# deepqmc/deepqmc

Hardware: NVIDIA H100
Metric: walker.local-energies/sec (higher is better)
Workload: dtype f32

## Files before the change

deepqmc_b200/_lib.py:

```python
from __future__ import annotations

import ctypes as C
import os

MAX_NUC, MAX_T, MAX_L = 32, 4, 4
LIB_NAME = 'libdqmc_b200.so'
LIB_PATH = os.path.join(os.path.dirname(os.path.abspath(__file__)), LIB_NAME)

SYMBOLS = [
    'dqmc_create', 'dqmc_destroy', 'dqmc_last_error', 'dqmc_version', 'dqmc_param_count',
    'dqmc_param_entry', 'dqmc_param_total', 'dqmc_set_params', 'dqmc_workspace_bytes',
    'dqmc_wf_forward', 'dqmc_local_energy', 'dqmc_mcmc_sweep', 'dqmc_launch_count',
    'dqmc_profile_begin', 'dqmc_profile_end', 'dqmc_debug_gemm', 'dqmc_wf_vjp_params', 'dqmc_langevin_sweep',
    'dqmc_set_pseudo_hamiltonian', 'dqmc_wf_orbitals', 'dqmc_mcmc_sweep_exchange',
    'dqmc_workspace_bytes_min', 'dqmc_debug_plan', 'dqmc_stats_pack', 'dqmc_debug_mlp_block', 'dqmc_debug_trunk',
    'dqmc_profile_end_classes', 'dqmc_debug_trunk_phases', 'dqmc_debug_attention', 'dqmc_debug_mlp',
    'dqmc_debug_slater', 'dqmc_debug_det_sum', 'dqmc_spin', 'dqmc_ecp_forward_count', 'dqmc_wf_grad_positions',
    'dqmc_force_terms', 'dqmc_ecp_force', 'dqmc_debug_wgrad', 'dqmc_zv_force',
    'dqmc_debug_attention_bwd',
]


class DqmcConfig(C.Structure):
    _fields_ = [
        ('kind', C.c_int32), ('dtype', C.c_int32), ('gemm_backend', C.c_int32),
        ('n_up', C.c_int32), ('n_down', C.c_int32), ('n_nuc', C.c_int32),
        ('embedding_dim', C.c_int32), ('n_layers', C.c_int32), ('n_heads', C.c_int32),
        ('n_determinants', C.c_int32), ('edge_dim', C.c_int32),
        ('cusp_kind', C.c_int32), ('cusp_same_scale', C.c_double), ('cusp_anti_scale', C.c_double),
        ('z_valence', C.c_double * MAX_NUC), ('ecp_mask', C.c_int32 * MAX_NUC),
        ('ecp_loc_terms', C.c_int32), ('ecp_loc', C.c_double * (MAX_NUC * 3 * 2 * MAX_T)),
        ('ecp_nl_lmax_p1', C.c_int32), ('ecp_nl_terms', C.c_int32),
        ('ecp_nl', C.c_double * (MAX_NUC * MAX_L * 2 * MAX_T)),
        ('n_env_per_nuc', C.c_int32), ('n_nuc_tokens', C.c_int32),
        ('factorized_det', C.c_int32), ('conf_linear', C.c_int32), ('mult_act', C.c_int32),
        ('n_elec_types', C.c_int32), ('jastrow_n', C.c_int32), ('jastrow_dims', C.c_int32 * 8),
        ('backflow_n', C.c_int32), ('backflow_dims', C.c_int32 * 8),
        ('gnn_features', C.c_int32), ('gnn_concat', C.c_int32), ('gnn_conv_ne', C.c_int32), ('gnn_sub_n', C.c_int32),
        ('gnn_deep_edges', C.c_int32), ('gnn_res_norm', C.c_int32), ('gnn_g_bias', C.c_int32), ('gnn_w_bias', C.c_int32),
        ('gnn_w_dims', C.c_int32 * 32), ('gnn_h_dims', C.c_int32 * 32), ('gnn_u_dims', C.c_int32 * 32),
        ('nuc_cusp_kind', C.c_int32), ('z_nuclear', C.c_double * MAX_NUC), ('backflow_add', C.c_int32),
    ]


_cache = {}


def load(path: str | None = None) -> C.CDLL:
    path = path or LIB_PATH
    if path in _cache:
        return _cache[path]
    if not os.path.exists(path):
        raise ImportError(
            f'{path} not found: the CUDA engine is not built. Run `python -c "import __graft_entry__ as g; '
            'g.build()"` (nvcc, sm_90a). There is no CPU fallback.'
        )
    lib = C.CDLL(path)
    for s in SYMBOLS:
        if not hasattr(lib, s):
            raise ImportError(f'{path} does not export {s}')
    vp, i32, i64, u64 = C.c_void_p, C.c_int32, C.c_int64, C.c_uint64
    lib.dqmc_create.argtypes = [C.POINTER(DqmcConfig), C.c_int, C.POINTER(vp)]
    lib.dqmc_destroy.argtypes = [vp]
    lib.dqmc_last_error.argtypes = [vp]
    lib.dqmc_last_error.restype = C.c_char_p
    lib.dqmc_version.restype = C.c_char_p
    lib.dqmc_param_count.argtypes = [vp]
    lib.dqmc_param_entry.argtypes = [vp, C.c_int, C.c_char_p, C.c_int, C.POINTER(i64), C.POINTER(i32), C.POINTER(i32)]
    lib.dqmc_param_total.argtypes = [vp]
    lib.dqmc_param_total.restype = i64
    lib.dqmc_set_params.argtypes = [vp, C.POINTER(C.c_double), i64, vp]
    lib.dqmc_workspace_bytes.argtypes = [vp, i32, i32]
    lib.dqmc_workspace_bytes.restype = i64
    lib.dqmc_workspace_bytes_min.argtypes = [vp, i32, i32]
    lib.dqmc_workspace_bytes_min.restype = i64
    lib.dqmc_debug_plan.argtypes = [vp, i32, i32, i64, C.POINTER(i64), C.POINTER(i64)]
    lib.dqmc_stats_pack.argtypes = [vp, vp, vp, i32, vp, vp]
    lib.dqmc_debug_mlp_block.argtypes = [vp, i32, vp, vp, vp, i32, vp]
    lib.dqmc_debug_trunk.argtypes = [vp, vp, vp, i32, vp]
    lib.dqmc_debug_trunk_phases.argtypes = [vp, C.POINTER(u64), i32]
    lib.dqmc_debug_attention.argtypes = [vp, i32, vp, vp, i32, i32, C.POINTER(i32), vp]
    lib.dqmc_debug_mlp.argtypes = [vp, i32, i32, vp, vp, vp, vp, i32, C.POINTER(i32), vp]
    lib.dqmc_debug_slater.argtypes = [vp, vp, vp, vp, i32, i32, vp, vp, vp, vp, C.POINTER(i32), vp]
    lib.dqmc_debug_det_sum.argtypes = [vp, vp, vp, vp, vp, vp, vp, i32, i32, vp, vp, vp, vp, vp]
    lib.dqmc_debug_wgrad.argtypes = [vp, vp, vp, i32, i32, i32, i32, i32, vp, vp, vp]
    lib.dqmc_debug_attention_bwd.argtypes = [vp, i32, vp, vp, vp, vp, vp, i32, vp]
    lib.dqmc_wf_forward.argtypes = [vp, vp, vp, i32, i32, vp, vp, vp, i64, vp]
    lib.dqmc_wf_orbitals.argtypes = [vp, vp, vp, i32, i32, vp, vp, i64, vp]
    lib.dqmc_local_energy.argtypes = [vp, vp, vp, i32, i32, u64, vp, vp, vp, vp, vp, vp, vp, i64, vp]
    lib.dqmc_mcmc_sweep.argtypes = [vp, vp, vp, vp, vp, vp, vp, i32, i32, i32, C.c_double, i32, u64, u64, u64,
                                    vp, vp, vp, vp, i64, vp]
    lib.dqmc_mcmc_sweep_exchange.argtypes = [vp, vp, vp, vp, vp, vp, vp, i32, i32, i32, C.c_double, i32, u64, u64, u64,
                                             vp, vp, C.c_double, C.POINTER(i32), vp, vp, vp, i64, vp]
    lib.dqmc_langevin_sweep.argtypes = [vp, vp, vp, vp, vp, vp, vp, vp, i32, i32, i32, C.c_double, i32, u64, u64, u64,
                                        vp, vp, vp, vp, i64, vp]
    lib.dqmc_wf_vjp_params.argtypes = [vp, vp, vp, i32, i32, vp, vp, vp, vp, vp, i64, vp]
    lib.dqmc_spin.argtypes = [vp, vp, vp, i32, i32, vp, vp, i32, vp, vp, vp, i64, vp]
    lib.dqmc_wf_grad_positions.argtypes = [vp, vp, vp, i32, i32, vp, vp, vp, vp, vp, i64, vp]
    lib.dqmc_force_terms.argtypes = [vp, vp, vp, i32, i32, vp, vp, vp, vp, vp]
    lib.dqmc_ecp_force.argtypes = [vp, vp, vp, i32, i32, u64, vp, vp, vp, vp, i64, vp]
    lib.dqmc_zv_force.argtypes = [vp, vp, vp, i32, i32, vp, vp, vp, i64, vp]
    lib.dqmc_set_pseudo_hamiltonian.argtypes = [vp, i32, i32, C.c_double, C.POINTER(C.c_double), C.POINTER(i32)]
    lib.dqmc_launch_count.argtypes = [vp]
    lib.dqmc_launch_count.restype = i64
    lib.dqmc_ecp_forward_count.argtypes = [vp]
    lib.dqmc_ecp_forward_count.restype = i64
    lib.dqmc_profile_begin.argtypes = [vp]
    lib.dqmc_debug_gemm.argtypes = [vp, C.c_char_p, C.c_char_p, vp, vp, vp, i32, i32, i32, i32, vp]
    lib.dqmc_profile_end.argtypes = [vp, C.POINTER(C.c_double), C.POINTER(C.c_double), C.POINTER(i64)]
    lib.dqmc_profile_end_classes.argtypes = [vp, C.POINTER(C.c_double), C.POINTER(C.c_double), C.POINTER(i64)]
    _cache[path] = lib
    return lib
```

deepqmc_b200/csrc/engine.cu:

```cuda
#include <algorithm>
#include <array>
#include <cstdio>
#include <cstdlib>
#include <cstring>
#include <limits>
#include <map>
#include <mutex>
#include <optional>
#include <string>
#include <type_traits>
#include <vector>

#include "dqmc_b200.h"
#include "kernels_mcmc.cuh"
#include "kernels_slater.cuh"
#include "kernels_trunk.cuh"
#include "kernels_gnn.cuh"
#include "kernels_bwd.cuh"
#include "kernels_zv.cuh"
#include "attn_mma.cuh"
#if !defined(DQMC_NO_TCGEN05)
#include "gemm_wgmma.cuh"
#include "fused_tc.cuh"
#include "trunk_tc.cuh"
#endif

namespace dq {

struct ParamEntry {
  std::string name;
  int64_t offset;
  int rows, cols;
};

static inline size_t align_up(size_t x, size_t a = 256) { return (x + a - 1) / a * a; }

template <class W>
static double last_above(W w, double lo, double eps) {
  double hi = lo > 0.0 ? 2 * lo : 1.0;
  while (w(hi) >= eps) { lo = hi; hi *= 2; }
  for (;;) {
    const double mid = lo + 0.5 * (hi - lo);
    if (mid <= lo || mid >= hi) break;
    (w(mid) >= eps ? lo : hi) = mid;
  }
  return lo;
}

template <class T>
static double ecp_cutoff_rc2(const T* nl, int L, int Tn, bool on) {
  const double inf = std::numeric_limits<double>::infinity(), eps = std::ldexp(1.0, -100);
  if (!on) return inf;
  for (int l = 0; l < L; ++l)
    for (int t = 0; t < Tn; ++t)
      if ((double)nl[(l * 2 + 1) * Tn + t] != 0.0 && !((double)nl[(l * 2) * Tn + t] > 0.0)) return inf;
  auto w = [&](double d2) {
    double s = 0.0;
    for (int l = 0; l < L; ++l)
      for (int t = 0; t < Tn; ++t)
        s += (2 * l + 1) * std::fabs((double)nl[(l * 2 + 1) * Tn + t]) * std::exp(-(double)nl[(l * 2) * Tn + t] * d2);
    return s;
  };
  if (w(0.0) < eps) return -inf;
  return last_above(w, 0.0, eps);
}

template <class T>
static double ecp_force_cutoff_rc2(const T* nl, int L, int Tn, bool on) {
  const double rc2 = ecp_cutoff_rc2(nl, L, Tn, on), eps = std::ldexp(1.0, -100);
  if (rc2 == std::numeric_limits<double>::infinity()) return rc2;
  double peak = 0.0;
  for (int l = 0; l < L; ++l)
    for (int t = 0; t < Tn; ++t)
      if ((double)nl[(l * 2 + 1) * Tn + t] != 0.0) peak = std::max(peak, 0.5 / (double)nl[(l * 2) * Tn + t]);
  auto wd = [&](double d2) {
    double s = 0.0;
    for (int l = 0; l < L; ++l)
      for (int t = 0; t < Tn; ++t) {
        const double a = (double)nl[(l * 2) * Tn + t];
        s += (2 * l + 1) * 2 * a * std::fabs((double)nl[(l * 2 + 1) * Tn + t]) * std::sqrt(d2) * std::exp(-a * d2);
      }
    return s;
  };
  return std::max(rc2, wd(peak) >= eps ? last_above(wd, peak, eps) : peak);
}

struct Switches {
  bool tc_trunk = true;
  bool tc_f16 = true;
  std::optional<bool> attn_fl_mma;
  std::optional<int> attn_tb, attn_nt;
  bool attn_generic = false;
  bool no_fuse_tanh = false;
  bool slater_generic = false;
  bool slater_fwd1 = false;
  bool ecp_cutoff = true;
  bool ecp_env_table = true;
  bool ecp_emb_table = true;
  int nsms = 0;
  bool trunk_phases = false;
};

inline Switches read_switches() {
  auto env = [](const char* name) { return std::getenv(name); };
  auto num = [&](const char* name) { const char* ev = env(name); return ev ? std::optional<int>(std::atoi(ev)) : std::nullopt; };
  Switches s;
  s.tc_trunk = num("DQMC_TC_TRUNK").value_or(1) != 0;
  s.tc_f16 = num("DQMC_TC_F16").value_or(1) != 0;
  if (auto v = num("DQMC_ATTN_FL_MMA")) s.attn_fl_mma = *v != 0;
  s.attn_tb = num("DQMC_ATTN_TB");
  s.attn_nt = num("DQMC_ATTN_NT");
  s.attn_generic = env("DQMC_ATTN_GENERIC");
  s.no_fuse_tanh = env("DQMC_NO_FUSE_TANH");
  s.slater_generic = env("DQMC_SLATER_GENERIC");
  s.slater_fwd1 = env("DQMC_SLATER_FWD1");
  s.ecp_cutoff = num("DQMC_ECP_CUTOFF").value_or(1) != 0;
  s.ecp_env_table = !env("DQMC_ECP_ENV_TABLE_OFF");
  s.ecp_emb_table = !env("DQMC_ECP_EMB_TABLE_OFF");
  s.nsms = num("DQMC_NSMS").value_or(0);
  s.trunk_phases = num("DQMC_TRUNK_PHASES").value_or(0) != 0;
  return s;
}

struct EngineBase {
  dqmc_config cfg;
  int device = 0;
  std::string err;
  int64_t launches = 0;
  int64_t ecp_forwards = 0;
  std::vector<ParamEntry> entries;
  int64_t total = 0;
  bool dry = false;
  bool plan_only = false;
  mutable const char* dry_hwm = nullptr;
  void note_hwm(const void* q) const { if (dry && (const char*)q > dry_hwm) dry_hwm = (const char*)q; }
  mutable std::vector<unsigned char*> emu_guards;
  bool prof = false;
  double prof_flops = 0;
  int64_t prof_n = 0;
  double prof_cls_flops[3] = {0, 0, 0};
  int64_t prof_cls_n[3] = {0, 0, 0};
  std::vector<int> prof_cls;
#ifndef DQMC_EMU
  std::vector<cudaEvent_t> prof_ev;
  void prof_note(cudaEvent_t e0, cudaEvent_t e1, double flops, int cls) {
    prof_ev.push_back(e0); prof_ev.push_back(e1);
    prof_cls.push_back(cls);
    prof_flops += flops; prof_cls_flops[cls] += flops;
    ++prof_n; ++prof_cls_n[cls];
  }
#endif
  virtual ~EngineBase() {}
  virtual int set_params(const double* host, int64_t n, cudaStream_t st) = 0;
  virtual int64_t ws_bytes(int B, int mode) = 0;
  virtual int64_t ws_bytes_min(int B, int mode) = 0;
  virtual int debug_plan(int B, int mode, int64_t wsb, int64_t* planned, int64_t* carved) = 0;
  virtual int stats_pack(const void* E, const void* stats, int B, double* out, cudaStream_t st) = 0;
  virtual int debug_mlp_block(int layer, const void* O, const void* X, void* Out, int rows, cudaStream_t st) = 0;
  virtual int debug_trunk(const void* X0, void* Out, int rows, cudaStream_t st) = 0;
  virtual int debug_attention(int layer, const void* QKV, void* O, int rows, int S, int32_t* kernel, cudaStream_t st) = 0;
  virtual int debug_mlp(int layer, int S, const void* O, const void* X, void* Out, void* scratch, int rows, int32_t* path,
                        cudaStream_t st) = 0;
  virtual int debug_trunk_phases(uint64_t* out, int n) = 0;
  virtual int debug_slater(const void* r, const void* R, const void* BF, int rows, int S, void* dsign, void* dlog, void* dgrad,
                           void* dlap, int32_t* kernel, cudaStream_t st) = 0;
  virtual int debug_det_sum(const void* r, const void* R, const void* dsign, const void* dlog, const void* dgrad,
                            const void* dlap, int B, int S, void* sign, void* logp, void* grad, void* stats,
                            cudaStream_t st) = 0;
  virtual int debug_wgrad(const void* A, const void* dY, int rows, int Kc, int Nc, int lo, int hi, void* dW, void* db,
                          cudaStream_t st) = 0;
  virtual int debug_attention_bwd(int layer, const void* QKV, const void* dO, void* dQKV, void* dKn, void* dVn, int rows,
                                  cudaStream_t st) = 0;
  virtual int forward(const void* r, const void* R, int Rb, int B, void* sign, void* logp, void* ws, int64_t wsb,
                      cudaStream_t st) = 0;
  virtual int local_energy(const void* r, const void* R, int Rb, int B, uint64_t seed, const void* twist, void* E,
                           void* stats, void* sign, void* logp, void* grad, void* ws, int64_t wsb,
                           cudaStream_t st) = 0;
  virtual int langevin(void* r, void* sign, void* logp, void* force, int32_t* age, void* tau, const void* R, int Rb, int B,
                       int n_sub, double target, int max_age, uint64_t seed, uint64_t step0, uint64_t woff, const void* nn,
                       const void* nu, void* stats, void* ws, int64_t wsb, cudaStream_t st) = 0;
  virtual int vjp_params(const void* r, const void* R, int Rb, int B, const void* weights, void* sign, void* logp,
                         void* grad_params, void* ws, int64_t wsb, cudaStream_t st) = 0;
  virtual int spin(const void* r, const void* R, int Rb, int B, const void* sign, const void* logp, int down_idx, void* s2,
                   void* ratio, void* ws, int64_t wsb, cudaStream_t st) = 0;
  virtual int grad_positions(const void* r, const void* R, int Rb, int B, void* sign, void* logp, void* grad_r, void* grad_R,
                             void* ws, int64_t wsb, cudaStream_t st) = 0;
  virtual int force_terms(const void* r, const void* R, int Rb, int B, const void* grad_r, void* bare, void* zvq, void* Q,
                          cudaStream_t st) = 0;
  virtual int ecp_force(const void* r, const void* R, int Rb, int B, uint64_t seed, const void* twist, void* bare, void* nl,
                        void* ws, int64_t wsb, cudaStream_t st) = 0;
  virtual int zv_force(const void* r, const void* R, int Rb, int B, void* zv, void* grad_R, void* ws, int64_t wsb,
                       cudaStream_t st) = 0;
  virtual int orbitals(const void* r, const void* R, int Rb, int B, void* out, void* ws, int64_t wsb, cudaStream_t st) = 0;
  virtual int set_ph(int n_tab, int n_grid, double r_max, const double* tables, const int32_t* tab_of_nuc) = 0;
  virtual int debug_gemm(const char* wname, const char* bname, const void* A, const void* Res, void* C, int Mr, int S,
                         int sliced, int backend, cudaStream_t st) = 0;
  virtual int mcmc(void* r, void* sign, void* logp, int32_t* age, void* tau, const void* R, int Rb, int B, int n_sub,
                   double target, int max_age, uint64_t seed, uint64_t step0, uint64_t woff, const void* nn,
                   const void* nu, void* stats, void* ws, int64_t wsb, cudaStream_t st, double p_exchange = 0.0,
                   const int32_t* ex_flags = nullptr, const int32_t* ex_idx = nullptr) = 0;

  void add(const std::string& n, int rows, int cols) {
    entries.push_back({n, total, rows, cols});
    total += (int64_t)rows * cols;
  }
  void build_layout() {
    const int N = cfg.n_up + cfg.n_down, M = cfg.n_nuc, d = cfg.embedding_dim, K = cfg.n_determinants;
    const int rep = cfg.n_env_per_nuc > 1 ? cfg.n_env_per_nuc : 1;
    if (cfg.kind == DQMC_PSIFORMER || cfg.kind == DQMC_TRANSPSIFORMER) {
      add("emb.w", 4 * M + 1, d);
      for (int l = 0; l < cfg.n_layers; ++l) {
        std::string p = "L" + std::to_string(l) + ".";
        add(p + "wqkv", d, 3 * d);
        add(p + "wo", d, d);
        add(p + "w1", d, d);
        add(p + "b1", 1, d);
        add(p + "w2", d, d);
        add(p + "b2", 1, d);
        if (cfg.kind == DQMC_TRANSPSIFORMER && cfg.n_nuc_tokens > 0) {
          add(p + "kn", cfg.n_nuc_tokens, d);
          add(p + "vn", cfg.n_nuc_tokens, d);
        }
      }
    }
    int bf_in = d;
    if (cfg.kind == DQMC_PAULINET) {
      const int e = cfg.edge_dim, nl = cfg.gnn_sub_n > 0 ? cfg.gnn_sub_n : 1;
      if (!cfg.gnn_features) add("emb.table", cfg.n_elec_types > 0 ? cfg.n_elec_types : 1, d);
      int dcur = cfg.gnn_features ? 4 * M : d, ecur = 4;
      const int nt = cfg.gnn_conv_ne ? 3 : 2;
      const char* tn[3] = {"same", "anti", "ne"};
      for (int l = 0; l < cfg.n_layers; ++l) {
        std::string p = "G" + std::to_string(l) + ".";
        for (int t = 0; t < nt; ++t) {
          int din = ecur;
          for (int i = 0; i < nl; ++i) {
            const std::string q = p + "w_" + tn[t] + "." + std::to_string(i);
            add(q + ".w", din, cfg.gnn_w_dims[l][i]);
            if (cfg.gnn_w_bias) add(q + ".b", 1, cfg.gnn_w_dims[l][i]);
            din = cfg.gnn_w_dims[l][i];
          }
          if (t < 2) {
            din = dcur;
            for (int i = 0; i < nl; ++i) {
              const std::string q = p + "h_" + tn[t] + "." + std::to_string(i);
              add(q + ".w", din, cfg.gnn_h_dims[l][i]); add(q + ".b", 1, cfg.gnn_h_dims[l][i]);
              din = cfg.gnn_h_dims[l][i];
            }
          } else {
            add(p + "hne", M, e);
          }
          if (!cfg.gnn_concat) { add(p + "g_" + tn[t] + ".w", e, d); add(p + "g_" + tn[t] + ".b", 1, d); }
        }
        if (cfg.gnn_concat) {
          add(p + "g.w", 3 * dcur + nt * e, d);
          if (cfg.gnn_g_bias) add(p + "g.b", 1, d);
        }
        if (cfg.gnn_deep_edges && l < cfg.n_layers - 1) {
          int din = ecur;
          for (int i = 0; i < nl; ++i) {
            const std::string q = p + "u." + std::to_string(i);
            add(q + ".w", din, cfg.gnn_u_dims[l][i]); add(q + ".b", 1, cfg.gnn_u_dims[l][i]);
            din = cfg.gnn_u_dims[l][i];
          }
          ecur = e;
        }
        dcur = d;
      }
      int din = d;
      for (int i = 0; i < cfg.jastrow_n; ++i) {
        add("J" + std::to_string(i) + ".w", din, cfg.jastrow_dims[i]);
        if (i < cfg.jastrow_n - 1) add("J" + std::to_string(i) + ".b", 1, cfg.jastrow_dims[i]);
        din = cfg.jastrow_dims[i];
      }
      din = d;
      for (int i = 0; i < cfg.backflow_n; ++i) {
        const std::string q = std::to_string(i);
        add("bfh" + q + ".up", din, cfg.backflow_dims[i]); add("bfh" + q + ".dn", din, cfg.backflow_dims[i]);
        add("bfb" + q + ".up", 1, cfg.backflow_dims[i]); add("bfb" + q + ".dn", 1, cfg.backflow_dims[i]);
        din = cfg.backflow_dims[i];
      }
      bf_in = din;
      add("bfb.up", 1, K * N); add("bfb.dn", 1, K * N);
      if (cfg.conf_linear) add("conf.w", 1, K);
    }
    if (cfg.kind == DQMC_FERMINET) {
      const int de = cfg.edge_dim;
      int din = 4 * M, ein = 4;
      for (int l = 0; l < cfg.n_layers; ++l) {
        std::string p = "F" + std::to_string(l) + ".";
        add(p + "wg", 3 * din + 2 * ein, d);
        add(p + "bg", 1, d);
        if (l < cfg.n_layers - 1) {
          add(p + "wu", ein, de);
          add(p + "bu", 1, de);
        }
        din = d; ein = de;
      }
    }
    add("bf.up", bf_in, K * N * (cfg.backflow_add == 2 ? 2 : 1));
    add("bf.dn", bf_in, K * N * (cfg.backflow_add == 2 ? 2 : 1));
    add("env.pi_up", K * N, M * rep);
    add("env.pi_dn", K * N, M * rep);
    add("env.zeta_up", K * N, M * rep);
    add("env.zeta_dn", K * N, M * rep);
    add("cusp.alpha", 1, 2);
    if (cfg.nuc_cusp_kind) add("cusp.nuc", 1, 1 + M);
  }
  int64_t off(const std::string& n) const {
    for (auto& e : entries)
      if (e.name == n) return e.offset;
    return -1;
  }
};

struct Arena {
  const EngineBase* e;
  char* base;
  char* top;
  int64_t cap;
  Arena(const EngineBase* e_, void* base_, int64_t cap_ = INT64_MAX) : e(e_), base((char*)base_), top((char*)base_), cap(cap_) {}
  template <class U>
  U* take(size_t n) {
    U* q = (U*)top;
    top += align_up(sizeof(U) * n);
#ifdef DQMC_EMU
    if (!e->dry) { std::memset(top, 0xC3, 256); e->emu_guards.push_back((unsigned char*)top); }
    top += 256;
#endif
    e->note_hwm(top);
    return q;
  }
  int64_t left() const { return cap - (top - base); }
};

static char* plan_base() { return (char*)(uintptr_t)0x100000; }
struct DryPass {
  EngineBase* e;
  bool was;
  const char* hw;
  explicit DryPass(const EngineBase* e_) : e(const_cast<EngineBase*>(e_)), was(e->dry), hw(e->dry_hwm) {
    e->dry = true;
    e->dry_hwm = plan_base();
  }
  ~DryPass() { e->dry = was; e->dry_hwm = hw; }
  int64_t bytes() const { return e->dry_hwm - plan_base(); }
};

template <class F>
static int64_t largest_fit(int64_t hi, int64_t wsb, F bytes) {
  if (hi < 1 || bytes(1) > wsb) return 0;
  if (bytes(hi) <= wsb) return hi;
  int64_t lo = 1;
  while (hi - lo > 1) {
    const int64_t mid = (lo + hi) / 2;
    (bytes(mid) <= wsb ? lo : hi) = mid;
  }
  return lo;
}

static constexpr int64_t kRowCap = 2000000000;

template <class T>
__global__ void convert_kernel(const double* __restrict__ src, T* __restrict__ dst, int64_t n) {
  int64_t i = (int64_t)blockIdx.x * blockDim.x + threadIdx.x;
  if (i < n) dst[i] = (T)src[i];
}

__global__ void split_transpose_kernel(const float* __restrict__ W, int K, int N, float* __restrict__ hi,
                                       float* __restrict__ lo) {
  int idx = blockIdx.x * blockDim.x + threadIdx.x;
  if (idx >= K * N) return;
  int n = idx / K, k = idx % K;
  float w = W[(size_t)k * N + n];
#if !defined(DQMC_NO_TCGEN05)
  float h = tc::tf32_rna(w);
  hi[idx] = h;
  lo[idx] = tc::tf32_rna(w - h);
#else
  float h = __uint_as_float(__float_as_uint(w) & 0xFFFFE000u);
  hi[idx] = h;
  lo[idx] = w - h;
#endif
}

#if !defined(DQMC_NO_TCGEN05)
__global__ void split_transpose_f16_kernel(const float* __restrict__ W, int K, int N, float scale, uint16_t* __restrict__ hi,
                                           uint16_t* __restrict__ lo) {
  int idx = blockIdx.x * blockDim.x + threadIdx.x;
  if (idx >= K * N) return;
  int n = idx / K, k = idx % K;
  const float w = W[(size_t)k * N + n] * scale;
  const uint32_t h = tc::pack_half2_rn(w, 0.f) & 0xFFFFu;
  const uint32_t l = tc::pack_half2_rn(w - tc::half_bits_to_float(h), 0.f) & 0xFFFFu;
  hi[idx] = (uint16_t)h;
  lo[idx] = (uint16_t)l;
}
#endif

#define DQ_CHECK(call)                                                             \
  do {                                                                             \
    if (dry) break;                              \
    cudaError_t e_ = (call);                                                       \
    if (e_ != cudaSuccess) {                                                       \
      err = std::string(#call) + ": " + cudaGetErrorString(e_);                    \
      return 1;                                                                    \
    }                                                                              \
  } while (0)

template <class F>
inline cudaError_t raise_dyn_smem(F fn, int bytes) {
  static std::mutex mu;
  static std::map<std::pair<int, const void*>, int> high;
  int dev = 0;
  cudaError_t e = cudaGetDevice(&dev);
  if (e != cudaSuccess) return e;
  std::lock_guard<std::mutex> lock(mu);
  int& h = high[std::make_pair(dev, (const void*)fn)];
  if (bytes > h) h = bytes;
  return cudaFuncSetAttribute(fn, cudaFuncAttributeMaxDynamicSharedMemorySize, h);
}

#define DQ_LAUNCH(kern, grid, block, smem, stream, ...)          \
  do {                                                           \
    if (dry) break;                           \
    auto kfn_ = kern;                                            \
    DQMC_LAUNCH(kfn_, grid, block, smem, stream, __VA_ARGS__);   \
    ++launches;                                                  \
  } while (0)

template <class T>
struct Engine : EngineBase {
  T* d_params = nullptr;
  T* d_params_t = nullptr;
  double* d_stage = nullptr;
  T* d_zval = nullptr;
  T* d_znuc = nullptr;
  int* d_ecp_mask = nullptr;
  T* d_ecp_loc = nullptr;
  T* d_nl_params = nullptr;
  int* d_nl_nuc = nullptr;
  double* d_nl_rc2 = nullptr;
  double* d_nl_rc2f = nullptr;
  int J = 0;
  T* d_ph_tabs = nullptr;
  int* d_ph_nuc = nullptr;
  int ph_G = 0;
  double ph_rmax = 0;
  int check_guards() {
#ifdef DQMC_EMU
    for (unsigned char* g : emu_guards)
      for (int i = 0; i < 256; ++i)
        if (g[i] != 0xC3) { emu_guards.clear(); err = "emulator: a workspace buffer was overrun (guard zone modified)"; return 4; }
    emu_guards.clear();
#endif
    return 0;
  }
  bool ph_on = false;
  int attn_tb = 1, attn_tb1 = 1;
  bool attn_gen_mma = false;
  bool attn_fl_mma = false;
  int attn_fl_threads = 128;
  bool attn_f32 = false;
  bool embed_fwd_ok = false;
  bool attn_mma_ok = false;
  bool slater_fwd2_ok = false;
  int N, M, d, K, KN, H, dh, T3;
  int BFW = 0;
  int add_off = 0;
  bool gnn = false;
  int bf_in = 0;
  bool trans = false;
  int Mn = 0, env_rep = 1;
  size_t max_smem = 0;
  int n_sms = 132;
  Switches sw;
  struct FwdIn {
    const T* env = nullptr;
    const T* emb = nullptr;
    const int* pairs = nullptr;
    int vper = 0;
    int layout = kVirtEcp;
    T* mos = nullptr;
    bool ph = false;
  };
#if !defined(DQMC_NO_TCGEN05)
  struct TcWeight {
    float* hi = nullptr; float* lo = nullptr; CUtensorMap mh, ml; int N = 0, K = 0;
    uint16_t* h16 = nullptr; CUtensorMap m16h, m16l, m16h_all, m16l_all; float wscale = 1.f; bool f16 = false, f16_all = false;
    CUtensorMap m16h_256, m16l_256; bool f16_256 = false;
  };
  CUtensorMap* d_trunk_maps = nullptr;
  unsigned char* d_trunk_scratch = nullptr;
  unsigned long long* d_trunk_phase = nullptr;
  static constexpr float kActScale = 16.f;
  std::map<std::string, TcWeight> tcw;
  bool use_tc() const { return std::is_same<T, float>::value && cfg.gemm_backend == DQMC_GEMM_TCGEN05; }
  int prepare_tc_weight(const std::string& name, const float* W, int Kc, int Nc, cudaStream_t st, double wmax) {
    TcWeight& w = tcw[name];
    if (!w.hi) {
      DQ_CHECK(cudaMalloc((void**)&w.hi, sizeof(float) * (size_t)Kc * Nc));
      DQ_CHECK(cudaMalloc((void**)&w.lo, sizeof(float) * (size_t)Kc * Nc));
      w.N = Nc; w.K = Kc;
      if (tc::make_weight_map(&w.mh, w.hi, Nc, Kc, tc::kBN) || tc::make_weight_map(&w.ml, w.lo, Nc, Kc, tc::kBN)) {
        err = "cuTensorMapEncodeTiled failed for " + name;
        return 4;
      }
      if (Kc % 64 == 0) {
        DQ_CHECK(cudaMalloc((void**)&w.h16, sizeof(uint16_t) * 2 * (size_t)Kc * Nc));
        const uint16_t* lo16 = w.h16 + (size_t)Kc * Nc;
        if (tc::make_kmajor_map(&w.m16h, w.h16, 2, Nc, Kc, 64, tc::kBN) || tc::make_kmajor_map(&w.m16l, lo16, 2, Nc, Kc, 64, tc::kBN)) {
          err = "cuTensorMapEncodeTiled (half planes) failed for " + name;
          return 4;
        }
        w.f16 = true;
        if (Nc <= 256 && Nc % 16 == 0) {
          if (tc::make_kmajor_map(&w.m16h_all, w.h16, 2, Nc, Kc, 32, Nc) || tc::make_kmajor_map(&w.m16l_all, lo16, 2, Nc, Kc, 32, Nc)) {
            err = "cuTensorMapEncodeTiled (whole-N half planes) failed for " + name;
            return 4;
          }
          w.f16_all = true;
        }
        if (Kc == 256 && Nc % 256 == 0 &&
            !tc::make_kmajor_map(&w.m16h_256, w.h16, 2, Nc, Kc, 32, 256) && !tc::make_kmajor_map(&w.m16l_256, lo16, 2, Nc, Kc, 32, 256))
          w.f16_256 = true;
      }
    }
    DQ_LAUNCH(split_transpose_kernel, dim3((Kc * Nc + 255) / 256), dim3(256), 0, st, W, Kc, Nc, w.hi, w.lo);
    if (w.f16) {
      int e = 0;
      if (wmax > 0) { std::frexp(wmax, &e); e = 10 - e; }
      e = e > 24 ? 24 : (e < -24 ? -24 : e);
      w.wscale = std::ldexp(1.f, e);
      DQ_LAUNCH(split_transpose_f16_kernel, dim3((Kc * Nc + 255) / 256), dim3(256), 0, st, W, Kc, Nc, w.wscale, w.h16,
                w.h16 + (size_t)Kc * Nc);
    }
    return 0;
  }
#else
  bool use_tc() const { return false; }
#endif

  int init() {
    sw = read_switches();
    N = cfg.n_up + cfg.n_down; M = cfg.n_nuc; d = cfg.embedding_dim; K = cfg.n_determinants;
    KN = K * N; H = cfg.n_heads; dh = d / H; T3 = 3 * N;
    BFW = KN * (cfg.backflow_add == 2 ? 2 : 1);
    add_off = cfg.backflow_add == 2 ? KN : 0;
    if (cfg.backflow_add && cfg.kind == DQMC_PAULINET) { err = "additive backflow: linear-head ansatz kinds only"; return 2; }
    if (cfg.kind != DQMC_PSIFORMER && cfg.kind != DQMC_FERMINET && cfg.kind != DQMC_TRANSPSIFORMER &&
        cfg.kind != DQMC_PAULINET) {
      err = "unknown ansatz kind"; return 2;
    }
    trans = cfg.kind == DQMC_TRANSPSIFORMER;
    Mn = trans ? cfg.n_nuc_tokens : 0;
    env_rep = cfg.n_env_per_nuc > 1 ? cfg.n_env_per_nuc : 1;
    if (M * env_rep > 4 * DQMC_MAX_NUC || Mn < 0 || Mn > DQMC_MAX_NUC) { err = "bad config (envelope terms / nuclear tokens)"; return 2; }
    if (H < 1) H = 1;
    if (cfg.kind == DQMC_FERMINET || cfg.kind == DQMC_PAULINET) { H = 1; dh = d; }
    gnn = cfg.kind == DQMC_PAULINET;
    if (gnn && (cfg.jastrow_n > 8 || cfg.backflow_n > 8 || cfg.jastrow_n < 0 || cfg.backflow_n < 0)) { err = "bad MLP depth"; return 2; }
    bf_in = d;
    if (gnn && cfg.backflow_n > 0) bf_in = cfg.backflow_dims[cfg.backflow_n - 1];
    if (M > DQMC_MAX_NUC || d % H != 0 || N < 2) { err = "bad config"; return 2; }
    build_layout();
    DQ_CHECK(cudaSetDevice(device));
    DQ_CHECK(cudaMalloc((void**)&d_params, sizeof(T) * total));
    DQ_CHECK(cudaMalloc((void**)&d_params_t, sizeof(T) * total));
    DQ_CHECK(cudaMalloc((void**)&d_stage, sizeof(double) * total));
    std::vector<T> z(M);
    for (int m = 0; m < M; ++m) z[m] = (T)cfg.z_valence[m];
    DQ_CHECK(cudaMalloc((void**)&d_zval, sizeof(T) * M));
    DQ_CHECK(cudaMemcpy(d_zval, z.data(), sizeof(T) * M, cudaMemcpyHostToDevice));
    {
      std::vector<T> zn(M);
      for (int m = 0; m < M; ++m) zn[m] = (T)cfg.z_nuclear[m];
      DQ_CHECK(cudaMalloc((void**)&d_znuc, sizeof(T) * M));
      DQ_CHECK(cudaMemcpy(d_znuc, zn.data(), sizeof(T) * M, cudaMemcpyHostToDevice));
    }
    DQ_CHECK(cudaMalloc((void**)&d_ecp_mask, sizeof(int) * M));
    DQ_CHECK(cudaMemcpy(d_ecp_mask, cfg.ecp_mask, sizeof(int) * M, cudaMemcpyHostToDevice));
    const int Tm = cfg.ecp_loc_terms;
    if (Tm > 0) {
      std::vector<T> lp((size_t)M * 6 * Tm);
      for (int m = 0; m < M; ++m)
        for (int n = 0; n < 3; ++n)
          for (int ab = 0; ab < 2; ++ab)
            for (int t = 0; t < Tm; ++t) lp[(((size_t)m * 3 + n) * 2 + ab) * Tm + t] = (T)cfg.ecp_loc[m][n][ab][t];
      DQ_CHECK(cudaMalloc((void**)&d_ecp_loc, sizeof(T) * lp.size()));
      DQ_CHECK(cudaMemcpy(d_ecp_loc, lp.data(), sizeof(T) * lp.size(), cudaMemcpyHostToDevice));
    }
    const int L = cfg.ecp_nl_lmax_p1, Tn = cfg.ecp_nl_terms;
    if (L > 0 && Tn > 0) {
      std::vector<T> np((size_t)M * L * 2 * Tn);
      std::vector<int> nuc;
      for (int m = 0; m < M; ++m) {
        bool any = false;
        for (int l = 0; l < L; ++l)
          for (int ab = 0; ab < 2; ++ab)
            for (int t = 0; t < Tn; ++t) {
              double v = cfg.ecp_nl[m][l][ab][t];
              np[(((size_t)m * L + l) * 2 + ab) * Tn + t] = (T)v;
              any = any || v != 0.0;
            }
        if (any) nuc.push_back(m);
      }
      J = (int)nuc.size();
      if (J > 0) {
        DQ_CHECK(cudaMalloc((void**)&d_nl_params, sizeof(T) * np.size()));
        DQ_CHECK(cudaMemcpy(d_nl_params, np.data(), sizeof(T) * np.size(), cudaMemcpyHostToDevice));
        DQ_CHECK(cudaMalloc((void**)&d_nl_nuc, sizeof(int) * J));
        DQ_CHECK(cudaMemcpy(d_nl_nuc, nuc.data(), sizeof(int) * J, cudaMemcpyHostToDevice));
        std::vector<double> rc2(J), rc2f(J);
        for (int j = 0; j < J; ++j) {
          rc2[j] = ecp_cutoff_rc2(np.data() + (size_t)nuc[j] * L * 2 * Tn, L, Tn, sw.ecp_cutoff);
          rc2f[j] = ecp_force_cutoff_rc2(np.data() + (size_t)nuc[j] * L * 2 * Tn, L, Tn, sw.ecp_cutoff);
        }
        DQ_CHECK(cudaMalloc((void**)&d_nl_rc2, sizeof(double) * J));
        DQ_CHECK(cudaMemcpy(d_nl_rc2, rc2.data(), sizeof(double) * J, cudaMemcpyHostToDevice));
        DQ_CHECK(cudaMalloc((void**)&d_nl_rc2f, sizeof(double) * J));
        DQ_CHECK(cudaMemcpy(d_nl_rc2f, rc2f.data(), sizeof(double) * J, cudaMemcpyHostToDevice));
      }
    }
#ifndef DQMC_EMU
    {
      int v = 0;
      DQ_CHECK(cudaDeviceGetAttribute(&v, cudaDevAttrMultiProcessorCount, device));
      if (v > 0) n_sms = v;
    }
#endif
    if (sw.nsms >= 1) n_sms = sw.nsms;
    const bool psif = cfg.kind == DQMC_PSIFORMER || trans;
    attn_f32 = psif && !trans && std::is_same<T, float>::value && dh % 16 == 0 && !sw.attn_generic;
    if (sw.attn_tb && *sw.attn_tb >= 1 && *sw.attn_tb <= T3) attn_tb = *sw.attn_tb;
    else attn_tb = attn_f32 ? attn_f32_pick_tb(N, dh, T3, 32 * 1024) : attn_pick_tb<T>(N, dh, T3, 100 * 1024, Mn);
    size_t s_attn = !psif ? 0 : attn_f32 ? attn_f32_smem_bytes(N, dh, attn_tb) : attn_smem_bytes<T>(N, dh, attn_tb, Mn);
    if (!sw.attn_nt) attn_fl_threads = s_attn > 110 * 1024 ? 512 : (s_attn > 56 * 1024 ? 256 : 128);
    else if (*sw.attn_nt >= 32 && *sw.attn_nt <= 1024 && *sw.attn_nt % 32 == 0) attn_fl_threads = *sw.attn_nt;
    attn_fl_mma = attn_f32 && N <= 32 && dh % 16 == 0 && sw.attn_fl_mma.value_or(N >= 20);
    if (attn_fl_mma && !sw.attn_tb) {
      attn_tb = attn_f32_pick_tb(N, dh, T3, 110 * 1024);
      s_attn = attn_f32_smem_bytes(N, dh, attn_tb);
    }
    attn_gen_mma = psif && !attn_f32 && std::is_same<T, float>::value && dh % 16 == 0 &&
                   sw.attn_fl_mma.value_or(N >= 20 && !sw.attn_generic);
    if (attn_gen_mma) {
      if (!sw.attn_tb) attn_tb = attn_pick_tb<T>(N, dh, T3, 110 * 1024, Mn, 4);
      s_attn = attn_smem_bytes<T>(N, dh, attn_tb, Mn, 4);
    }
    size_t s_sl = slater_smem_bytes<T>(N);
    max_smem = s_attn > s_sl ? s_attn : s_sl;
    if (max_smem > 227 * 1024) { err = "system too large for the shared-memory tiling (N)"; return 2; }
    if (attn_f32) {
      if (launch_attn_f32(nullptr, nullptr, 0, 0, 0, 0.f, 0, (int)s_attn, nullptr, true)) return 1;
    } else if (psif) {
      DQ_CHECK(raise_dyn_smem(attn_fl_kernel<T>, (int)s_attn));
      if constexpr (std::is_same<T, float>::value) DQ_CHECK(raise_dyn_smem((attn_fl_kernel<T, true>), (int)s_attn));
    }
    DQ_CHECK(raise_dyn_smem(slater_kernel<T>, (int)s_sl));
    slater_fwd2_ok = N <= 32 && slater_fwd2_smem_bytes<T>(N, M, K) <= 110 * 1024 && !sw.slater_generic && !sw.slater_fwd1;
    if (slater_fwd2_ok) {
      DQ_CHECK(raise_dyn_smem(slater_fwd2_kernel<T, 14>, (int)slater_fwd2_smem_bytes<T>(N, M, K)));
      DQ_CHECK(raise_dyn_smem(slater_fwd2_kernel<T, 16>, (int)slater_fwd2_smem_bytes<T>(N, M, K)));
      DQ_CHECK(raise_dyn_smem(slater_fwd2_kernel<T, 28>, (int)slater_fwd2_smem_bytes<T>(N, M, K)));
      DQ_CHECK(raise_dyn_smem(slater_fwd2_kernel<T, 30>, (int)slater_fwd2_smem_bytes<T>(N, M, K)));
      DQ_CHECK(raise_dyn_smem(slater_fwd2_kernel<T, 32>, (int)slater_fwd2_smem_bytes<T>(N, M, K)));
    }
    attn_mma_ok = psif && std::is_same<T, float>::value && dh == 64 && N + Mn <= 48 && d % 4 == 0 && !sw.attn_generic;
    embed_fwd_ok = psif && d % 4 == 0 && embed_fwd_smem_bytes<T>(M, d) <= 200 * 1024;
    if (embed_fwd_ok)
      DQ_CHECK(raise_dyn_smem(embed_fwd_kernel<T>, (int)embed_fwd_smem_bytes<T>(M, d)));
    if (cfg.gemm_backend == DQMC_GEMM_TCGEN05) {
#if !defined(DQMC_NO_TCGEN05)
      if (!std::is_same<T, float>::value) { err = "DQMC_GEMM_TCGEN05 needs dtype DQMC_F32"; return 2; }
      if (d % 32 != 0) { err = "DQMC_GEMM_TCGEN05 needs embedding_dim % 32 == 0"; return 2; }
      DQ_CHECK(raise_dyn_smem(tc::gemm3x_kernel<false>, tc::SmemLayout::total()));
      DQ_CHECK(raise_dyn_smem(tc::gemm3x_kernel<true>, tc::SmemLayout::total()));
      DQ_CHECK(raise_dyn_smem(tc::mlp_block_f16_kernel<128>, tc::MlpSmem::total()));
      DQ_CHECK(raise_dyn_smem(tc::mlp_block_f16_kernel<256>, tc::MlpSmem::total()));
      DQ_CHECK(raise_dyn_smem(tc::trunk_f16_kernel<1>, tc::TrSmem::total()));
      DQ_CHECK(raise_dyn_smem(tc::trunk_f16_kernel<2>, tc::TrSmem::total()));
      DQ_CHECK(raise_dyn_smem(tc::trunk_f16_kernel<4>, tc::TrSmem::total()));
      DQ_CHECK(raise_dyn_smem(tc::trunk_f16_kernel<8>, tc::TrSmem::total()));
      DQ_CHECK(raise_dyn_smem(tc::trunk_f16_kernel<16>, tc::TrSmem::total()));
      DQ_CHECK(raise_dyn_smem(tc::trunk_f16_kernel<32>, tc::TrSmem::total()));
      if (psif && !trans && d == 256 && H == 4 && N <= 32 && cfg.n_layers <= tc::kTrMaxLayers) {
        DQ_CHECK(cudaMalloc((void**)&d_trunk_maps, sizeof(CUtensorMap) * 8 * cfg.n_layers));
        DQ_CHECK(cudaMalloc((void**)&d_trunk_scratch, (size_t)n_sms * tc::kTrScratchPerCta));
        if (sw.trunk_phases) {
          DQ_CHECK(cudaMalloc((void**)&d_trunk_phase, sizeof(unsigned long long) * tc::kPhases));
          DQ_CHECK(cudaMemset(d_trunk_phase, 0, sizeof(unsigned long long) * tc::kPhases));
        }
      }
#else
      err = "this build has no tensor-core backend"; return 2;
#endif
    }
    return 0;
  }
  ~Engine() override {
    if (plan_only) return;
    cudaFree(d_params); cudaFree(d_params_t); cudaFree(d_stage); cudaFree(d_znuc); cudaFree(d_zval); cudaFree(d_ecp_mask);
    if (d_ecp_loc) cudaFree(d_ecp_loc);
    if (d_nl_params) cudaFree(d_nl_params);
    if (d_nl_nuc) cudaFree(d_nl_nuc);
    if (d_nl_rc2) cudaFree(d_nl_rc2);
    if (d_nl_rc2f) cudaFree(d_nl_rc2f);
    if (d_ph_tabs) cudaFree(d_ph_tabs);
    if (d_ph_nuc) cudaFree(d_ph_nuc);
#if !defined(DQMC_NO_TCGEN05)
    for (auto& kv : tcw) {
      if (kv.second.hi) cudaFree(kv.second.hi);
      if (kv.second.lo) cudaFree(kv.second.lo);
      if (kv.second.h16) cudaFree(kv.second.h16);
    }
    if (d_trunk_maps) cudaFree(d_trunk_maps);
    if (d_trunk_scratch) cudaFree(d_trunk_scratch);
    if (d_trunk_phase) cudaFree(d_trunk_phase);
#endif
  }
  const T* P(const std::string& n) const { return d_params + off(n); }

  int set_ph(int n_tab, int n_grid, double r_max, const double* tables, const int32_t* tab_of_nuc) override {
    if (J > 0 || cfg.ecp_loc_terms > 0) { err = "pseudo-Hamiltonian and Gaussian-type ECP are mutually exclusive"; return 2; }
    if (n_tab < 1 || n_grid < 2 || !(r_max > 0) || !tables || !tab_of_nuc) { err = "bad pseudo-Hamiltonian tables"; return 2; }
    for (int m = 0; m < M; ++m)
      if (tab_of_nuc[m] >= n_tab) { err = "pseudo-Hamiltonian table index out of range"; return 2; }
    std::vector<T> h((size_t)n_tab * 2 * n_grid);
    for (size_t i = 0; i < h.size(); ++i) h[i] = (T)tables[i];
    if (d_ph_tabs) cudaFree(d_ph_tabs);
    if (d_ph_nuc) cudaFree(d_ph_nuc);
    DQ_CHECK(cudaMalloc((void**)&d_ph_tabs, sizeof(T) * h.size()));
    DQ_CHECK(cudaMemcpy(d_ph_tabs, h.data(), sizeof(T) * h.size(), cudaMemcpyHostToDevice));
    DQ_CHECK(cudaMalloc((void**)&d_ph_nuc, sizeof(int) * M));
    DQ_CHECK(cudaMemcpy(d_ph_nuc, tab_of_nuc, sizeof(int) * M, cudaMemcpyHostToDevice));
    ph_G = n_grid; ph_rmax = r_max; ph_on = true;
    return 0;
  }
  PhArgs<T> ph_args(const T* QA) const {
    PhArgs<T> a;
    a.QA = QA; a.tabs = d_ph_tabs; a.tab_of_nuc = d_ph_nuc; a.G = ph_G; a.rmax = (T)ph_rmax;
    return a;
  }

  int set_params(const double* host, int64_t n, cudaStream_t st) override {
    if (n != total) { err = "parameter count mismatch"; return 2; }
    DQ_CHECK(cudaMemcpyAsync(d_stage, host, sizeof(double) * n, cudaMemcpyHostToDevice, st));
    DQ_LAUNCH(convert_kernel<T>, dim3((unsigned)((n + 255) / 256)), dim3(256), 0, st, (const double*)d_stage, d_params, n);
    for (auto& e : entries)
      if (e.rows >= 1 && e.cols >= 1)
        DQ_LAUNCH(transpose_kernel<T>, dim3((e.rows * e.cols + 255) / 256), dim3(256), 0, st, (const T*)(d_params + e.offset),
                  e.rows, e.cols, d_params_t + e.offset);
#if !defined(DQMC_NO_TCGEN05)
    if (use_tc()) {
      std::map<std::string, double> wmax;
      auto group = [](const std::string& n) {
        const size_t k = n.size();
        return (k > 3 && (n.compare(k - 3, 3, ".up") == 0 || n.compare(k - 3, 3, ".dn") == 0)) ? n.substr(0, k - 3) : n;
      };
      for (auto& e : entries) {
        double m = 0;
        for (int64_t i = 0; i < (int64_t)e.rows * e.cols; ++i) m = std::max(m, std::fabs(host[e.offset + i]));
        double& g = wmax[group(e.name)];
        g = std::max(g, m);
      }
      for (auto& e : entries) {
        bool is_w = e.name.find(".w") != std::string::npos || e.name.rfind("bf.", 0) == 0;
        if (!is_w || e.name == "emb.w" || e.rows % 32 != 0 || e.cols < 64) continue;
        int rc = prepare_tc_weight(e.name, (const float*)(d_params + e.offset), e.rows, e.cols, st, wmax[group(e.name)]);
        if (rc) return rc;
      }
      if (d_trunk_maps && trunk_weights_ok()) {
        std::vector<CUtensorMap> hm((size_t)8 * cfg.n_layers);
        for (int l = 0; l < cfg.n_layers; ++l) {
          const std::string pfx = "L" + std::to_string(l) + ".";
          int g = 0;
          for (const char* n : {"wqkv", "wo", "w1", "w2"}) {
            const TcWeight& w = tcw.at(pfx + n);
            hm[(size_t)8 * l + 2 * g] = w.m16h_256;
            hm[(size_t)8 * l + 2 * g + 1] = w.m16l_256;
            ++g;
          }
        }
        DQ_CHECK(cudaMemcpy(d_trunk_maps, hm.data(), sizeof(CUtensorMap) * hm.size(), cudaMemcpyHostToDevice));
      }
    }
#endif
    DQ_CHECK(cudaGetLastError());
    return 0;
  }

  struct Ws {
    T *X, *O, *A, *M1, *QKV, *BF, *dsign, *dlog, *dlap, *dgrad;
    T* QA = nullptr;
    T* Gadd = nullptr;
    T *G0 = nullptr, *G1 = nullptr, *G2 = nullptr, *Hs = nullptr, *Ha = nullptr, *C = nullptr, *Fc = nullptr, *HT = nullptr,
      *E0 = nullptr, *E1 = nullptr, *ET0 = nullptr, *ET1 = nullptr, *W3 = nullptr,
      *Y0 = nullptr, *Y1 = nullptr, *Jb = nullptr;
  };
  int gnn_hmax() const {
    int h = 1;
    for (int i = 0; i < cfg.backflow_n; ++i) h = cfg.backflow_dims[i] > h ? cfg.backflow_dims[i] : h;
    return h;
  }
  size_t fermi_dmax() const { return (size_t)(4 * M > d ? 4 * M : d); }
  size_t fermi_emax() const { return (size_t)(cfg.edge_dim > 4 ? cfg.edge_dim : 4); }
  int gnn_dmax() const { return cfg.gnn_features && 4 * M > d ? 4 * M : d; }
  int gnn_emax() const {
    int m = cfg.edge_dim > 4 ? cfg.edge_dim : 4;
    for (int l = 0; l < cfg.n_layers && l < 8; ++l)
      for (int i = 0; i < cfg.gnn_sub_n && i < 4; ++i) {
        m = cfg.gnn_w_dims[l][i] > m ? cfg.gnn_w_dims[l][i] : m;
        m = cfg.gnn_u_dims[l][i] > m ? cfg.gnn_u_dims[l][i] : m;
      }
    return m;
  }
  int gnn_hnode_max() const {
    int m = cfg.edge_dim;
    for (int l = 0; l < cfg.n_layers && l < 8; ++l)
      for (int i = 0; i < cfg.gnn_sub_n && i < 4; ++i) m = cfg.gnn_h_dims[l][i] > m ? cfg.gnn_h_dims[l][i] : m;
    return m;
  }
  int gnn_jsum() const {
    int j = d;
    for (int i = 0; i < cfg.jastrow_n; ++i) j += cfg.jastrow_dims[i];
    return j;
  }
  int64_t chunk_bytes(int Bc, int S) const {
    DryPass dp(this);
    carve(plan_base(), Bc, S);
    return dp.bytes();
  }
  Ws carve(void* base, int Bc, int S) const {
    Ws w;
    size_t rows = (size_t)Bc * N * S;
    Arena a(this, base);
    if (gnn) {
      const size_t e = cfg.edge_dim, hm = gnn_hmax(), dm = gnn_dmax(), em = gnn_emax(), hn = gnn_hnode_max();
      const size_t pairs8 = (size_t)Bc * N * (N + (cfg.gnn_conv_ne ? M : 0)) * 8;
      w.X = a.take<T>(rows * dm); w.O = a.take<T>(rows * dm); w.G0 = a.take<T>(rows * d); w.G1 = a.take<T>(rows * d);
      w.G2 = a.take<T>(rows * d); w.Fc = a.take<T>(rows * (3 * dm + 3 * e)); w.Hs = a.take<T>(rows * e);
      w.Ha = a.take<T>(rows * e); w.HT = a.take<T>(rows * hn); w.C = a.take<T>(rows * 3 * e);
      w.E0 = a.take<T>(pairs8 * em); w.E1 = a.take<T>(pairs8 * em); w.ET0 = a.take<T>(pairs8 * em); w.ET1 = a.take<T>(pairs8 * em);
      w.W3 = a.take<T>(pairs8 * 3 * e);
      w.Y0 = a.take<T>(rows * hm); w.Y1 = a.take<T>(rows * hm); w.Jb = a.take<T>((size_t)Bc * S * gnn_jsum());
      w.A = w.M1 = w.QKV = nullptr;
      w.BF = a.take<T>(rows * KN);
    } else if (cfg.kind == DQMC_FERMINET) {
      const size_t dm = fermi_dmax(), em = fermi_emax(), fin = 3 * dm + 2 * em;
      w.X = a.take<T>(rows * dm); w.O = a.take<T>(rows * dm); w.QKV = a.take<T>(rows * fin);
      w.A = a.take<T>(rows * N * em); w.M1 = a.take<T>(rows * N * em);
      w.BF = a.take<T>(rows * BFW);
    } else {
      w.X = a.take<T>(rows * d); w.O = a.take<T>(rows * d); w.A = a.take<T>(rows * d); w.M1 = a.take<T>(rows * d);
      w.QKV = a.take<T>(rows * 3 * d); w.BF = a.take<T>(rows * BFW);
    }
    w.dsign = a.take<T>((size_t)Bc * K); w.dlog = a.take<T>((size_t)Bc * K); w.dlap = a.take<T>((size_t)Bc * K);
    w.dgrad = a.take<T>((size_t)Bc * K * (S > 1 ? T3 : 1));
    if (ph_on && S > 1) w.QA = a.take<T>((size_t)Bc * N * PH_STRIDE);
    if (cfg.backflow_add) w.Gadd = a.take<T>((size_t)Bc * N * 5);
    return w;
  }
  template <class Prefix>
  int64_t prefixed_bytes(Prefix prefix, int64_t Bc, int S) const {
    DryPass dp(this);
    Arena a(this, plan_base());
    prefix(a);
    carve(a.top, (int)Bc, S);
    return dp.bytes();
  }
  int max_chunk(int64_t wsb, int S, int B) const {
    int64_t row_cap = kRowCap / ((int64_t)N * S * 3 * d);
    if (cfg.kind == DQMC_FERMINET) row_cap = kRowCap / ((int64_t)N * N * S * (3 * (int64_t)fermi_dmax() + 64));
    if (gnn) row_cap = kRowCap / ((int64_t)N * (N + M + S) * (8 * gnn_emax() + 3 * gnn_dmax() + 3 * cfg.edge_dim + KN));
    return (int)largest_fit(std::min<int64_t>(B, row_cap), wsb, [&](int64_t n) { return chunk_bytes((int)n, S); });
  }
  struct VirtGroup {
    T *r, *sign, *logp, *env = nullptr, *emb = nullptr, *sign0 = nullptr, *logp0 = nullptr;
    int *pairs = nullptr, *offs = nullptr;
    T *gr = nullptr, *gR = nullptr, *gR0 = nullptr;
  };
  VirtGroup carve_virt_group(Arena& a, int64_t nb, int64_t V) const {
    VirtGroup g;
    g.r = a.take<T>(V * 3 * N); g.sign = a.take<T>(V); g.logp = a.take<T>(V);
    g.env = a.take<T>(nb * N * K * N); g.emb = a.take<T>(nb * N * d);
    return g;
  }
  VirtGroup carve_ecp_group(Arena& a, int64_t nb) const {
    VirtGroup g = carve_virt_group(a, nb, nb * J * N * 12);
    g.pairs = a.take<int>(nb * J * N); g.offs = a.take<int>(nb + 1);
    return g;
  }
  VirtGroup carve_ecp_force_group(Arena& a, int64_t nb) const {
    const int64_t V = nb * J * N * 12;
    VirtGroup g;
    g.r = a.take<T>(V * 3 * N); g.sign = a.take<T>(V); g.logp = a.take<T>(V);
    g.gr = a.take<T>(V * 3 * N); g.gR = a.take<T>(V * 3 * M);
    g.pairs = a.take<int>(nb * J * N); g.offs = a.take<int>(nb + 1);
    g.sign0 = a.take<T>(nb); g.logp0 = a.take<T>(nb); g.gR0 = a.take<T>(nb * 3 * M);
    return g;
  }
  VirtGroup carve_spin_group(Arena& a, int64_t nb, int64_t P) const {
    VirtGroup g = carve_virt_group(a, nb, nb * P);
    g.sign0 = a.take<T>(nb); g.logp0 = a.take<T>(nb);
    return g;
  }
  int64_t group_cap(int64_t vper) const { return std::max<int64_t>(1, kRowCap / ((int64_t)N * 3 * d) / vper); }
  int64_t ecp_bytes(int64_t nb, int64_t Vc) const { return prefixed_bytes([&](Arena& a) { carve_ecp_group(a, nb); }, Vc, 1); }
  void fwd_chunk_carve(Arena& a, int64_t Vc) const { carve(a.top, (int)Vc, 1); }
  void pos_chunk_carve(Arena& a, int64_t Vc) {
    const PosOut none{nullptr, nullptr};
    reverse_chunk(nullptr, nullptr, 0, (int)Vc, nullptr, nullptr, nullptr, nullptr, Arena(this, a.top), nullptr, &none);
  }
  int64_t ecp_force_bytes(int64_t nb, int64_t Vc) {
    DryPass dp(this);
    Arena a(this, plan_base());
    carve_ecp_force_group(a, nb);
    pos_chunk_carve(a, Vc);
    return dp.bytes();
  }
  bool has_nl_force() const { return has_pos_pass() && !trans; }
  int64_t spin_bytes(int64_t nb, int64_t P, int64_t Vc) const {
    return prefixed_bytes([&](Arena& a) { carve_spin_group(a, nb, P); }, Vc, 1);
  }
  struct Proposals { T *r, *force, *sign, *logp; int* cnt; };
  Proposals carve_proposals(Arena& a, int B, bool with_force) const {
    Proposals q;
    q.r = a.take<T>((size_t)B * 3 * N); q.force = with_force ? a.take<T>((size_t)B * 3 * N) : nullptr;
    q.sign = a.take<T>(B); q.logp = a.take<T>(B); q.cnt = a.take<int>(1);
    return q;
  }
  struct ForceBufs { T *E, *stats, *grad; };
  ForceBufs carve_force(Arena& a, int B) const {
    ForceBufs f;
    f.E = a.take<T>(B); f.stats = a.take<T>((size_t)6 * B); f.grad = a.take<T>((size_t)B * T3);
    return f;
  }
  int64_t sweep_bytes(int B, bool langevin, int Bc) const {
    auto prefix = [&](Arena& a) { carve_proposals(a, B, langevin); if (langevin) carve_force(a, B); };
    return prefixed_bytes(prefix, Bc, langevin ? T3 + 2 : 1);
  }
  int64_t vjp_chunk_bytes(int Bc, bool pos = false) {
    DryPass dp(this);
    const PosOut none{nullptr, nullptr};
    reverse_chunk(nullptr, nullptr, 0, Bc, nullptr, nullptr, nullptr, nullptr, Arena(this, plan_base()), nullptr,
                  pos ? &none : nullptr);
    return dp.bytes();
  }
  bool has_pos_pass() const { return !gnn && !cfg.backflow_add; }
  int64_t ws_bytes(int B, int mode) override {
    if (B < 1) B = 1;
    if (mode == DQMC_MODE_VJP) return vjp_chunk_bytes(B);
    if (mode == DQMC_MODE_GRAD_POS) return has_pos_pass() ? vjp_chunk_bytes(B, true) : 0;
    if (mode == DQMC_MODE_MCMC) return sweep_bytes(B, false, B);
    if (mode == DQMC_MODE_LANGEVIN) return sweep_bytes(B, true, B);
    if (mode == DQMC_MODE_ECP_FORCE) {
      if (!J || !has_nl_force()) return 0;
      const int64_t vper = (int64_t)J * N * 12, nb = std::min<int64_t>(B, group_cap(vper));
      return ecp_force_bytes(nb, nb * vper);
    }
    if (mode == DQMC_MODE_ZV_FORCE) return zv_refusal() ? 0 : zv_chunk_bytes(B);
    if (mode == DQMC_MODE_SPIN) {
      const int64_t P = (int64_t)cfg.n_up * cfg.n_down;
      if (!P) return 0;
      const int64_t nb = std::min<int64_t>(B, group_cap(P));
      return spin_bytes(nb, P, nb * P);
    }
    int S = mode == DQMC_MODE_FORWARD ? 1 : T3 + 2;
    int64_t need = chunk_bytes(B, S);
    if (mode == DQMC_MODE_LOCAL_ENERGY && J > 0) {
      const int64_t vper = (int64_t)J * N * 12, nb = std::min<int64_t>(B, group_cap(vper));
      need = std::max(need, ecp_bytes(nb, nb * vper));
    }
    return need;
  }
  int64_t ws_bytes_min(int B, int mode) override {
    if (B < 1) B = 1;
    const int S = T3 + 2;
    switch (mode) {
      case DQMC_MODE_VJP: return vjp_chunk_bytes(1);
      case DQMC_MODE_GRAD_POS: return has_pos_pass() ? vjp_chunk_bytes(1, true) : 0;
      case DQMC_MODE_MCMC: return sweep_bytes(B, false, 1);
      case DQMC_MODE_LANGEVIN: return sweep_bytes(B, true, 1);
      case DQMC_MODE_LOCAL_ENERGY: return std::max<int64_t>(chunk_bytes(1, S), J > 0 ? ecp_bytes(1, 1) : 0);
      case DQMC_MODE_ECP_FORCE: return J > 0 && has_nl_force() ? ecp_force_bytes(1, 1) : 0;
      case DQMC_MODE_ZV_FORCE: return zv_refusal() ? 0 : zv_chunk_bytes(1);
      case DQMC_MODE_SPIN: {
        const int64_t P = (int64_t)cfg.n_up * cfg.n_down;
        return P ? spin_bytes(1, P, 1) : 0;
      }
      default: return chunk_bytes(1, 1);
    }
  }
  int debug_plan(int B, int mode, int64_t wsb, int64_t* planned, int64_t* carved) override {
    const int64_t pl = ws_bytes(B, mode);
    if (planned) *planned = pl;
    if (wsb <= 0) wsb = pl;
    DryPass dp(this);
    void* ws = plan_base();
    int rc = 0;
    switch (mode) {
      case DQMC_MODE_FORWARD: rc = forward(nullptr, nullptr, 0, B, nullptr, nullptr, ws, wsb, nullptr); break;
      case DQMC_MODE_LOCAL_ENERGY:
        rc = local_energy(nullptr, nullptr, 0, B, 0, nullptr, nullptr, nullptr, nullptr, nullptr, nullptr, ws, wsb, nullptr);
        break;
      case DQMC_MODE_VJP: rc = vjp_params(nullptr, nullptr, 0, B, nullptr, nullptr, nullptr, nullptr, ws, wsb, nullptr); break;
      case DQMC_MODE_MCMC:
        rc = mcmc(nullptr, nullptr, nullptr, nullptr, nullptr, nullptr, 0, B, 1, 0.5, -1, 0, 0, 0, nullptr, nullptr, nullptr, ws, wsb,
                  nullptr, 0.0, nullptr, nullptr);
        break;
      case DQMC_MODE_LANGEVIN:
        rc = langevin(nullptr, nullptr, nullptr, nullptr, nullptr, nullptr, nullptr, 0, B, 1, 0.5, -1, 0, 0, 0, nullptr, nullptr,
                      nullptr, ws, wsb, nullptr);
        break;
      case DQMC_MODE_SPIN: rc = spin(nullptr, nullptr, 0, B, nullptr, nullptr, -1, nullptr, nullptr, ws, wsb, nullptr); break;
      case DQMC_MODE_GRAD_POS:
        rc = grad_positions(nullptr, nullptr, 0, B, nullptr, nullptr, nullptr, nullptr, ws, wsb, nullptr);
        break;
      case DQMC_MODE_ECP_FORCE:
        rc = ecp_force(nullptr, nullptr, 0, B, 0, nullptr, nullptr, has_nl_force() ? ws : nullptr, ws, wsb, nullptr);
        break;
      case DQMC_MODE_ZV_FORCE: rc = zv_force(nullptr, nullptr, 0, B, nullptr, nullptr, ws, wsb, nullptr); break;
      default: err = "unknown mode"; rc = 2;
    }
    if (carved) *carved = dp.bytes();
    return rc;
  }

  bool can_fuse_act(int S) const {
    if (!use_tc() || sw.no_fuse_tanh) return false;
    if (S == 1) return true;
    return S <= 128 && (128 / S) * S >= 112;
  }
  bool gemm_on_tc(const char* w0, const char* w1, int lda, int ldc, int Kc, const T* bias1) const {
#if !defined(DQMC_NO_TCGEN05)
    return use_tc() && !bias1 && Kc % 32 == 0 && lda % 4 == 0 && ldc % 4 == 0 && tcw.count(w0) && (!w1 || tcw.count(w1));
#else
    return false;
#endif
  }
  int gemm(const T* A, int lda, const char* w0, const char* w1, int zsplit, int ldw, const T* bias, const T* Res,
           int ldr, T* C, int ldc, int Mr, int Nc, int Kc, int S, int sliced, int Nel, cudaStream_t st, int act = 0,
           const T* bias1 = nullptr) {
    if (dry) return 0;
    const T* W0 = P(w0);
    const T* W1 = w1 ? P(w1) : nullptr;
#if !defined(DQMC_NO_TCGEN05)
    if constexpr (std::is_same<T, float>::value) {
      if (gemm_on_tc(w0, w1, lda, ldc, Kc, bias1)) {
        const TcWeight& t0 = tcw.at(w0);
        const TcWeight& t1 = w1 ? tcw.at(w1) : t0;
        tc::Params p;
        p.A = A; p.lda = lda; p.bias = bias; p.Res = Res; p.ldr = ldr; p.C = C; p.ldc = ldc; p.M = Mr; p.N = Nc;
        p.K = Kc; p.S = S; p.sliced = sliced; p.Nel = Nel; p.z_split = zsplit; p.err_flag = nullptr;
        p.act = act;
        p.rpt = (act && S > 1) ? (128 / S) * S : tc::kBM;
        p.a_scale = 1.f; p.unscale = 1.f;
        const bool f16 = S == 1 && sw.tc_f16 && Kc % 64 == 0 && t0.f16 && t1.f16 && t0.wscale == t1.wscale;
        if (f16) { p.a_scale = kActScale; p.unscale = 1.f / (kActScale * t0.wscale); }
        const int MT = (Mr + p.rpt - 1) / p.rpt, NT = (Nc + tc::kBN - 1) / tc::kBN;
        const int n_tiles = (sliced ? Nel : 1) * MT * NT;
#ifndef DQMC_EMU
        cudaEvent_t e0 = nullptr, e1 = nullptr;
        if (prof) { cudaEventCreate(&e0); cudaEventCreate(&e1); cudaEventRecord(e0, st); }
#endif
        if (f16)
          DQ_LAUNCH(tc::gemm3x_kernel<true>, dim3(n_tiles), dim3(tc::kThreads), tc::SmemLayout::total(), st, t0.m16h, t0.m16l,
                    t1.m16h, t1.m16l, p);
        else
          DQ_LAUNCH(tc::gemm3x_kernel<false>, dim3(n_tiles), dim3(tc::kThreads), tc::SmemLayout::total(), st, t0.mh, t0.ml,
                    t1.mh, t1.ml, p);
#ifndef DQMC_EMU
        if (prof) {
          cudaEventRecord(e1, st);
          prof_note(e0, e1, 2.0 * (double)Mr * (sliced ? Nel : 1) * (double)Nc * (double)Kc, 0);
        }
#endif
        return 0;
      }
    }
#endif
    if (act) { err = "internal: fused activation requested on the CUDA-core GEMM"; return 5; }
    GemmArgs<T> g;
    g.A = A; g.lda = lda; g.W0 = W0; g.W1 = W1; g.z_split = zsplit; g.ldw = ldw; g.bias = bias; g.Res = Res;
    g.ldr = ldr; g.C = C; g.ldc = ldc; g.M = Mr; g.N = Nc; g.K = Kc; g.S = S; g.sliced = sliced; g.Nel = Nel;
    g.bias1 = bias1;
    constexpr int BM = 64, BN = 64, BK = 16, TM = 4, TN = 4;
    dim3 grid((Nc + BN - 1) / BN, (Mr + BM - 1) / BM, sliced ? Nel : 1);
#ifndef DQMC_EMU
    cudaEvent_t e0 = nullptr, e1 = nullptr;
    if (prof) { cudaEventCreate(&e0); cudaEventCreate(&e1); cudaEventRecord(e0, st); }
#endif
    DQ_LAUNCH((gemm_kernel<T, BM, BN, BK, TM, TN>), grid, dim3(256), 0, st, g);
#ifndef DQMC_EMU
    if (prof) {
      cudaEventRecord(e1, st);
      prof_note(e0, e1, 2.0 * (double)Mr * (sliced ? Nel : 1) * (double)Nc * (double)Kc, 0);
    }
#endif
    return 0;
  }

  bool can_fuse_mlp(int S, const std::string& pfx) const {
#if !defined(DQMC_NO_TCGEN05)
    if (S != 1 || !use_tc() || !sw.tc_f16 || (d != 128 && d != 256)) return false;
    for (const char* n : {"wo", "w1", "w2"}) {
      auto it = tcw.find(pfx + n);
      if (it == tcw.end() || !it->second.f16_all) return false;
    }
    return true;
#else
    return false;
#endif
  }
  int mlp_block(const std::string& pfx, const T* O, const T* X, T* Out, int rows, cudaStream_t st) {
    if (dry) return 0;
#if !defined(DQMC_NO_TCGEN05)
    if constexpr (std::is_same<T, float>::value) {
      const TcWeight& wo = tcw.at(pfx + "wo");
      const TcWeight& w1 = tcw.at(pfx + "w1");
      const TcWeight& w2 = tcw.at(pfx + "w2");
      tc::MlpParams p;
      p.O = O; p.ldo = d; p.X = X; p.ldx = d; p.Out = Out; p.ldout = d; p.b1 = P(pfx + "b1"); p.b2 = P(pfx + "b2");
      p.M = rows; p.d = d; p.a_scale = kActScale;
      p.us0 = 1.f / (kActScale * wo.wscale); p.us1 = 1.f / (kActScale * w1.wscale); p.us2 = 1.f / (kActScale * w2.wscale);
      p.err_flag = nullptr;
      const int MT = (rows + 127) / 128;
      const int grid = MT < n_sms ? MT : n_sms;
#ifndef DQMC_EMU
      cudaEvent_t e0 = nullptr, e1 = nullptr;
      if (prof) { cudaEventCreate(&e0); cudaEventCreate(&e1); cudaEventRecord(e0, st); }
#endif
      if (d == 256)
        DQ_LAUNCH(tc::mlp_block_f16_kernel<256>, dim3(grid), dim3(tc::kMlpThreads), tc::MlpSmem::total(), st, wo.m16h_all,
                  wo.m16l_all, w1.m16h_all, w1.m16l_all, w2.m16h_all, w2.m16l_all, p);
      else
        DQ_LAUNCH(tc::mlp_block_f16_kernel<128>, dim3(grid), dim3(tc::kMlpThreads), tc::MlpSmem::total(), st, wo.m16h_all,
                  wo.m16l_all, w1.m16h_all, w1.m16l_all, w2.m16h_all, w2.m16l_all, p);
#ifndef DQMC_EMU
      if (prof) {
        cudaEventRecord(e1, st);
        prof_note(e0, e1, 3 * 2.0 * (double)rows * (double)d * (double)d, 1);
      }
#endif
      return 0;
    }
#endif
    err = "internal: fused MLP block without the tensor-core backend";
    return 5;
  }

  int debug_mlp_block(int layer, const void* O, const void* X, void* Out, int rows, cudaStream_t st) override {
    const std::string pfx = "L" + std::to_string(layer) + ".";
    if (!can_fuse_mlp(1, pfx)) { err = "fused MLP block not available for this configuration"; return 2; }
    int rc = mlp_block(pfx, (const T*)O, (const T*)X, (T*)Out, rows, st);
    if (rc) return rc;
    DQ_CHECK(cudaGetLastError());
    return 0;
  }

  bool trunk_weights_ok() const {
#if !defined(DQMC_NO_TCGEN05)
    for (int l = 0; l < cfg.n_layers; ++l)
      for (const char* n : {"wqkv", "wo", "w1", "w2"}) {
        auto it = tcw.find("L" + std::to_string(l) + "." + n);
        if (it == tcw.end() || !it->second.f16_256) return false;
      }
    return true;
#else
    return false;
#endif
  }
  bool can_trunk(int S) const {
#if !defined(DQMC_NO_TCGEN05)
    return S == 1 && use_tc() && sw.tc_f16 && sw.tc_trunk && d_trunk_maps && d_trunk_scratch && cfg.n_layers >= 1 && trunk_weights_ok();
#else
    return false;
#endif
  }
  int trunk_block(const T* X0, T* Out, int rows, cudaStream_t st, const FwdIn& in, int64_t v0) {
    if (dry) return 0;
#if !defined(DQMC_NO_TCGEN05)
    if constexpr (std::is_same<T, float>::value) {
      tc::TrunkParams p;
      p.X0 = X0; p.ldx = d; p.Out = Out; p.ldout = d; p.maps = d_trunk_maps; p.scratch = d_trunk_scratch;
      p.Xbase = in.emb; p.v0 = in.emb ? (long long)v0 : 0; p.vper = in.emb ? in.vper : 0;
      p.n_up = cfg.n_up; p.vlayout = in.layout; p.pairs = in.pairs; p.wspin = P("emb.w") + (size_t)(4 * M) * d;
      int np2 = 1;
      while (np2 < N) np2 *= 2;
      p.walkers = rows / N; p.N = N; p.L = cfg.n_layers; p.a_scale = kActScale;
      p.attn_scale = (float)(1.0 / std::sqrt((double)dh)); p.err_flag = nullptr; p.phase = d_trunk_phase;
      for (int l = 0; l < cfg.n_layers; ++l) {
        const std::string pfx = "L" + std::to_string(l) + ".";
        p.b1[l] = P(pfx + "b1"); p.b2[l] = P(pfx + "b2");
        int g = 0;
        for (const char* n : {"wqkv", "wo", "w1", "w2"}) p.us[l][g++] = 1.f / (kActScale * tcw.at(pfx + n).wscale);
      }
      const int G = 128 / np2, MT = (p.walkers + G - 1) / G;
      const int grid = MT < n_sms ? MT : n_sms;
#ifndef DQMC_EMU
      cudaEvent_t e0 = nullptr, e1 = nullptr;
      if (prof) { cudaEventCreate(&e0); cudaEventCreate(&e1); cudaEventRecord(e0, st); }
#endif
      switch (np2) {
        case 1: DQ_LAUNCH(tc::trunk_f16_kernel<1>, dim3(grid), dim3(tc::kTrThreads), tc::TrSmem::total(), st, p); break;
        case 2: DQ_LAUNCH(tc::trunk_f16_kernel<2>, dim3(grid), dim3(tc::kTrThreads), tc::TrSmem::total(), st, p); break;
        case 4: DQ_LAUNCH(tc::trunk_f16_kernel<4>, dim3(grid), dim3(tc::kTrThreads), tc::TrSmem::total(), st, p); break;
        case 8: DQ_LAUNCH(tc::trunk_f16_kernel<8>, dim3(grid), dim3(tc::kTrThreads), tc::TrSmem::total(), st, p); break;
        case 16: DQ_LAUNCH(tc::trunk_f16_kernel<16>, dim3(grid), dim3(tc::kTrThreads), tc::TrSmem::total(), st, p); break;
        case 32: DQ_LAUNCH(tc::trunk_f16_kernel<32>, dim3(grid), dim3(tc::kTrThreads), tc::TrSmem::total(), st, p); break;
        default: err = "internal: fused trunk walker slot above 32"; return 5;
      }
#ifndef DQMC_EMU
      if (prof) {
        cudaEventRecord(e1, st);
        prof_note(e0, e1, (double)cfg.n_layers * 2.0 * (double)rows * (6.0 * d * d + 2.0 * N * d), 2);
      }
#endif
      return 0;
    }
#endif
    err = "internal: fused trunk without the tensor-core backend";
    return 5;
  }
  int debug_trunk_phases(uint64_t* out, int n) override {
#if !defined(DQMC_NO_TCGEN05)
    if (!d_trunk_phase) { err = "trunk phase timers are off (set DQMC_TRUNK_PHASES=1 before creating the engine)"; return 2; }
    if (n < tc::kPhases) { err = "dqmc_debug_trunk_phases: the output holds fewer than the kernel's counters"; return 2; }
    DQ_CHECK(cudaMemcpy(out, d_trunk_phase, sizeof(unsigned long long) * tc::kPhases, cudaMemcpyDeviceToHost));
    DQ_CHECK(cudaMemset(d_trunk_phase, 0, sizeof(unsigned long long) * tc::kPhases));
    return 0;
#else
    err = "this build has no tensor-core backend"; return 2;
#endif
  }
  int debug_trunk(const void* X0, void* Out, int rows, cudaStream_t st) override {
    if (!can_trunk(1)) { err = "fused trunk not available for this configuration"; return 2; }
    if (rows % N != 0) { err = "debug_trunk: rows must be a multiple of the electron count"; return 2; }
    int rc = trunk_block((const T*)X0, (T*)Out, rows, st, FwdIn{}, 0);
    if (rc) return rc;
    DQ_CHECK(cudaGetLastError());
    return 0;
  }

  int debug_attention(int layer, const void* QKV, void* O, int rows, int S, int32_t* kernel, cudaStream_t st) override {
    if (!(cfg.kind == DQMC_PSIFORMER || trans)) { err = "debug_attention: the configuration has no softmax attention layers"; return 2; }
    if (layer < 0 || layer >= cfg.n_layers) { err = "debug_attention: layer out of range"; return 2; }
    if (S != 1 && S != T3 + 2) { err = "debug_attention: S must be 1 or 3N + 2"; return 2; }
    if (rows < 1 || rows % (N * S) != 0) { err = "debug_attention: rows must be a positive multiple of N S"; return 2; }
    int rc = attention((const T*)QKV, (T*)O, rows / (N * S), S, layer, st, kernel);
    if (rc) return rc;
    DQ_CHECK(cudaGetLastError());
    return 0;
  }

  int debug_mlp(int layer, int S, const void* O, const void* X, void* Out, void* scratch, int rows, int32_t* path,
                cudaStream_t st) override {
    if (!(cfg.kind == DQMC_PSIFORMER || trans)) { err = "debug_mlp: the configuration has no attention layers"; return 2; }
    if (layer < 0 || layer >= cfg.n_layers) { err = "debug_mlp: layer out of range"; return 2; }
    if (S != 1 && S != T3 + 2) { err = "debug_mlp: S must be 1 or 3N + 2"; return 2; }
    if (rows < 1 || rows % (N * S) != 0) { err = "debug_mlp: rows must be a positive multiple of N S"; return 2; }
    T* A = (T*)scratch;
    int rc = mlp("L" + std::to_string(layer) + ".", (const T*)O, (const T*)X, (T*)Out, A, A + (size_t)rows * d, rows / (N * S), S,
                 st, path);
    if (rc) return rc;
    DQ_CHECK(cudaGetLastError());
    return 0;
  }

  int debug_slater(const void* r, const void* R, const void* BF, int rows, int S, void* dsign, void* dlog, void* dgrad,
                   void* dlap, int32_t* kernel, cudaStream_t st) override {
    if (S != 1 && S != T3 + 2) { err = "debug_slater: S must be 1 or 3N + 2"; return 2; }
    if (rows < 1 || rows % (N * S) != 0) { err = "debug_slater: rows must be a positive multiple of N S"; return 2; }
    if (S > 1 && (!dgrad || !dlap)) { err = "debug_slater: S = 3N + 2 needs the gradient and Laplacian outputs"; return 2; }
    const int Bc = rows / (N * S);
    T* bf = nullptr;
    T* gadd = nullptr;
    DQ_CHECK(cudaMalloc((void**)&bf, sizeof(T) * (size_t)rows * BFW));
    if (cfg.backflow_add && cudaMalloc((void**)&gadd, sizeof(T) * (size_t)Bc * N * 5) != cudaSuccess) {
      cudaFree(bf);
      err = "debug_slater: out of device memory";
      return 1;
    }
    int rc = 0;
    if (cudaMemcpyAsync(bf, BF, sizeof(T) * (size_t)rows * BFW, cudaMemcpyDeviceToDevice, st) != cudaSuccess) {
      err = "debug_slater: copy of the backflow rows failed";
      rc = 1;
    }
    if (!rc) rc = slater((const T*)r, (const T*)R, 0, Bc, S, bf, gadd, (T*)dsign, (T*)dlog, (T*)dgrad, (T*)dlap, st, nullptr,
                         FwdIn{}, 0, kernel);
    if (!rc && cudaStreamSynchronize(st) != cudaSuccess) { err = "debug_slater: kernel failed"; rc = 1; }
    cudaFree(bf);
    cudaFree(gadd);
    if (rc) return rc;
    DQ_CHECK(cudaGetLastError());
    return 0;
  }

  int debug_det_sum(const void* r, const void* R, const void* dsign, const void* dlog, const void* dgrad, const void* dlap,
                    int B, int S, void* sign, void* logp, void* grad, void* stats, cudaStream_t st) override {
    if (S != 1 && S != T3 + 2) { err = "debug_det_sum: S must be 1 or 3N + 2"; return 2; }
    if (B < 1) { err = "debug_det_sum: needs at least one walker"; return 2; }
    if (S > 1 && (!dgrad || !dlap || !grad || !stats)) { err = "debug_det_sum: S = 3N + 2 needs every jet array"; return 2; }
    T* E = nullptr;
    DQ_CHECK(cudaMalloc((void**)&E, sizeof(T) * (size_t)B));
    const FinalizeCfg fc = finalize_cfg(S);
    DQ_LAUNCH(finalize_kernel<T>, dim3(B), dim3(128), finalize_smem_bytes<T>(N, K), st, fc, (const T*)r, (const T*)R, 0,
              (const T*)dsign, (const T*)dlog, (const T*)dgrad, (const T*)dlap, P("cusp.alpha"), (const T*)d_zval,
              (const T*)d_ecp_loc, (const int*)d_ecp_mask, B, (T*)sign, (T*)logp, E, (T*)stats, (T*)grad,
              cfg.conf_linear ? P("conf.w") : (const T*)nullptr, (const T*)nullptr,
              cfg.nuc_cusp_kind ? P("cusp.nuc") : (const T*)nullptr, PhArgs<T>());
    const bool ok = cudaStreamSynchronize(st) == cudaSuccess;
    cudaFree(E);
    if (!ok) { err = "debug_det_sum: kernel failed"; return 1; }
    DQ_CHECK(cudaGetLastError());
    return 0;
  }

  int debug_attention_bwd(int layer, const void* QKV, const void* dO, void* dQKV, void* dKn, void* dVn, int rows,
                          cudaStream_t st) override {
    if (!(cfg.kind == DQMC_PSIFORMER || trans)) { err = "debug_attention_bwd: the configuration has no softmax attention layers"; return 2; }
    if (layer < 0 || layer >= cfg.n_layers) { err = "debug_attention_bwd: layer out of range"; return 2; }
    if (rows < 1 || rows % N != 0) { err = "debug_attention_bwd: rows must be a positive multiple of N"; return 2; }
    if (Mn > 0 && (!dKn || !dVn)) { err = "debug_attention_bwd: nuclear tokens need the dKn / dVn outputs"; return 2; }
    int rc = attention_bwd(layer, (const T*)QKV, (const T*)dO, (T*)dQKV, rows / N, Mn > 0 ? (T*)dKn : nullptr,
                           Mn > 0 ? (T*)dVn : nullptr, st);
    if (rc) return rc;
    DQ_CHECK(cudaGetLastError());
    return 0;
  }

  int debug_wgrad(const void* A, const void* dY, int rows, int Kc, int Nc, int lo, int hi, void* dW, void* db,
                  cudaStream_t st) override {
    if (rows < 1 || Kc < 1 || Nc < 1) { err = "debug_wgrad: rows, K and Nc must be positive"; return 2; }
    if (hi != ALL_ROWS && (lo < 0 || hi < lo || hi > N)) { err = "debug_wgrad: the electron range must lie in [0, N]"; return 2; }
    wgrad((const T*)A, Kc, (const T*)dY, Nc, rows, Kc, Nc, (T*)dW, lo, hi, st);
    bgrad((const T*)dY, Nc, rows, Nc, (T*)db, st, lo, hi);
    DQ_CHECK(cudaGetLastError());
    return 0;
  }

  int debug_gemm(const char* wname, const char* bname, const void* A, const void* Res, void* C, int Mr, int S,
                 int sliced, int backend, cudaStream_t st) override {
    int64_t o = off(wname);
    if (o < 0) { err = "unknown weight"; return 2; }
    int rows = 0, cols = 0;
    for (auto& e : entries) if (e.name == wname) { rows = e.rows; cols = e.cols; }
    int saved = cfg.gemm_backend;
    cfg.gemm_backend = backend;
    int rc = gemm((const T*)A, rows, wname, sliced ? "bf.dn" : nullptr, cfg.n_up, cols, bname ? P(bname) : nullptr,
                  (const T*)Res, cols, (T*)C, cols, Mr, cols, rows, S, sliced, N, st);
    cfg.gemm_backend = saved;
    if (rc) return rc;
    DQ_CHECK(cudaGetLastError());
    return 0;
  }

  template <int NE, int DH>
  int attn_f32_go(const float* QKV, float* O, int Bc, int S, int tb, float scale, int smem, cudaStream_t st, bool setup) {
    if (setup) {
      DQ_CHECK(raise_dyn_smem((attn_fl_f32_kernel<NE, DH, false>), smem));
      DQ_CHECK(raise_dyn_smem((attn_fl_f32_kernel<NE, DH, true>), smem));
      return 0;
    }
    if (attn_fl_mma && S > 1)
      DQ_LAUNCH((attn_fl_f32_kernel<NE, DH, true>), dim3(Bc, H), dim3(256), smem, st, QKV, 3 * d, O, d, N, S, dh, d, scale, tb);
    else
      DQ_LAUNCH((attn_fl_f32_kernel<NE, DH, false>), dim3(Bc, H), dim3(attn_fl_threads), smem, st, QKV, 3 * d, O, d, N, S, dh, d, scale, tb);
    return 0;
  }
  int launch_attn_generic(const T* QKV, T* O, int Bc, int S, int tb, T scale, const T* kn, const T* vn, cudaStream_t st) {
    if constexpr (std::is_same<T, float>::value) {
      if (attn_gen_mma && S > 1) {
        DQ_LAUNCH((attn_fl_kernel<T, true>), dim3(Bc, H), dim3(256), attn_smem_bytes<T>(N, dh, tb, Mn, 4), st, QKV, 3 * d, O, d, N, S,
                  dh, d, scale, tb, kn, vn, Mn);
        return 0;
      }
    }
    DQ_LAUNCH(attn_fl_kernel<T>, dim3(Bc, H), dim3(S > 1 ? attn_fl_threads : 128), attn_smem_bytes<T>(N, dh, tb, Mn), st, QKV, 3 * d,
              O, d, N, S, dh, d, scale, tb, kn, vn, Mn);
    return 0;
  }
  int launch_attn_f32(const float* QKV, float* O, int Bc, int S, int tb, float scale, int, int smem, cudaStream_t st,
                      bool setup) {
    if (dh == 64) {
      switch (N) {
        case 4: return attn_f32_go<4, 64>(QKV, O, Bc, S, tb, scale, smem, st, setup);
        case 10: return attn_f32_go<10, 64>(QKV, O, Bc, S, tb, scale, smem, st, setup);
        case 14: return attn_f32_go<14, 64>(QKV, O, Bc, S, tb, scale, smem, st, setup);
        case 28: return attn_f32_go<28, 64>(QKV, O, Bc, S, tb, scale, smem, st, setup);
        case 30: return attn_f32_go<30, 64>(QKV, O, Bc, S, tb, scale, smem, st, setup);
        default: return attn_f32_go<0, 64>(QKV, O, Bc, S, tb, scale, smem, st, setup);
      }
    }
    return attn_f32_go<0, 0>(QKV, O, Bc, S, tb, scale, smem, st, setup);
  }

  int ferminet_trunk(const T* r, const T* R, int Rb, int Bc, int S, Ws& w, T** Xout, cudaStream_t st, const T* qa = nullptr) {
    const int rows = Bc * N * S, rowsE = Bc * N * N * S, de = cfg.edge_dim, d0 = 4 * M;
    const T isq2 = (T)0.70710678118654752440;
    DQ_LAUNCH(embed_kernel<T>, dim3(Bc * N), dim3(128), sizeof(T) * 5 * d0, st, r, R, Rb, N, M, cfg.n_up, S, 0, 0,
              (const T*)nullptr, d0, w.X, Bc * N, 1, qa);
    DQ_LAUNCH(edge_feat_kernel<T>, dim3((Bc * N * N + 127) / 128), dim3(128), 0, st, r, N, S, w.A, Bc * N * N, qa);
    T* Hc = w.X; T* Hn = w.O; T* Ec = w.A; T* En = w.M1;
    int dcur = d0, ecur = 4;
    for (int l = 0; l < cfg.n_layers; ++l) {
      std::string p = "F" + std::to_string(l) + ".";
      const int fin = 3 * dcur + 2 * ecur;
      DQ_LAUNCH(fermi_agg_kernel<T>, dim3(Bc * S, N), dim3(128), 0, st, (const T*)Hc, dcur, (const T*)Ec, ecur, N, cfg.n_up,
                S, w.QKV);
      int rc = gemm(w.QKV, fin, (p + "wg").c_str(), nullptr, 0, d, P(p + "bg"), nullptr, 0, Hn, d, rows, d, fin, S, 0, N, st);
      if (rc) return rc;
      DQ_LAUNCH(tanh_fl_kernel<T>, dim3(Bc * N, (d + 127) / 128), dim3(128), 0, st, Hn, d,
                (const T*)(dcur == d ? Hc : nullptr), dcur, S, d, dcur == d ? isq2 : T(1));
      if (l < cfg.n_layers - 1) {
        rc = gemm(Ec, ecur, (p + "wu").c_str(), nullptr, 0, de, P(p + "bu"), nullptr, 0, En, de, rowsE, de, ecur, S, 0, N, st);
        if (rc) return rc;
        DQ_LAUNCH(tanh_fl_kernel<T>, dim3(Bc * N * N, 1), dim3(32), 0, st, En, de, (const T*)(ecur == de ? Ec : nullptr),
                  ecur, S, de, ecur == de ? isq2 : T(1));
        T* t2 = Ec; Ec = En; En = t2;
        ecur = de;
      }
      T* t1 = Hc; Hc = Hn; Hn = t1;
      dcur = d;
    }
    *Xout = Hc;
    return 0;
  }

  int gnn_mlp(const T* in, int din, const std::string& base, const int* dims, int nl, bool bias, T* tmp, T* out, int rows_,
              int Sg, cudaStream_t st) {
    const T* cur = in;
    int dc = din;
    for (int i = 0; i < nl; ++i) {
      T* dst = (i == nl - 1) ? out : tmp;
      const std::string q = base + "." + std::to_string(i);
      int rc = gemm(cur, dc, (q + ".w").c_str(), nullptr, 0, dims[i], bias ? P(q + ".b") : nullptr, nullptr, 0, dst, dims[i], rows_,
                    dims[i], dc, Sg, 0, 1, st);
      if (rc) return rc;
      DQ_LAUNCH(act_fl_kernel<T>, dim3(rows_ / Sg, (dims[i] + 63) / 64), dim3(64), 0, st, dst, dims[i], (const T*)nullptr, 0, Sg,
                dims[i], T(1), 0);
      cur = dst; dc = dims[i];
    }
    return 0;
  }

  int paulinet_trunk(const T* r, const T* R, int Rb, int Bc, int S, Ws& w, T** Xbf, const T** jastrow, cudaStream_t st,
                     const T* qa = nullptr) {
    const int rows = Bc * N * S, e = cfg.edge_dim, groups = Bc * N, nl = cfg.gnn_sub_n > 0 ? cfg.gnn_sub_n : 1;
    const int Mne = cfg.gnn_conv_ne ? M : 0, NS = N + Mne, nt = cfg.gnn_conv_ne ? 3 : 2;
    const int pairs = Bc * N * NS, prow = pairs * 8;
    const T isq2 = (T)0.70710678118654752440;
    int dcur = d, ecur = 4;
    if (cfg.gnn_features) {
      dcur = 4 * M;
      DQ_LAUNCH(embed_kernel<T>, dim3(Bc * N), dim3(128), sizeof(T) * 5 * dcur, st, r, R, Rb, N, M, cfg.n_up, S, 0, 0,
                (const T*)nullptr, dcur, w.X, Bc * N, 1, qa);
    } else {
      DQ_LAUNCH(gnn_embed_kernel<T>, dim3((Bc * N * d + 127) / 128), dim3(128), 0, st, P("emb.table"),
                cfg.n_elec_types > 0 ? cfg.n_elec_types : 1, N, cfg.n_up, S, d, w.X, Bc * N);
    }
    DQ_LAUNCH(gnn_edge_feat_kernel<T>, dim3((pairs + 63) / 64), dim3(64), 0, st, r, R, Rb, N, M, Mne, w.E0, pairs, S > 1 ? qa : (const T*)nullptr);
    T* X = w.X;
    T* Xn = w.O;
    T* E = w.E0;
    T* En = w.E1;
    const char* tn[3] = {"same", "anti", "ne"};
    for (int l = 0; l < cfg.n_layers; ++l) {
      const std::string p = "G" + std::to_string(l) + ".";
      for (int t = 0; t < nt; ++t) {
        int rc = gnn_mlp(E, ecur, p + "w_" + tn[t], cfg.gnn_w_dims[l], nl, cfg.gnn_w_bias != 0, w.ET0, w.W3 + (size_t)t * prow * e,
                         prow, 8, st);
        if (rc) return rc;
      }
      int rc = gnn_mlp(X, dcur, p + "h_same", cfg.gnn_h_dims[l], nl, true, w.HT, w.Hs, rows, S, st);
      if (rc) return rc;
      rc = gnn_mlp(X, dcur, p + "h_anti", cfg.gnn_h_dims[l], nl, true, w.HT, w.Ha, rows, S, st);
      if (rc) return rc;
      DQ_LAUNCH(gnn_conv_kernel<T>, dim3(groups), dim3(128), 0, st, (const T*)w.W3, (const T*)(w.W3 + (size_t)prow * e),
                (const T*)(w.W3 + (size_t)2 * prow * e), (const T*)w.Hs, (const T*)w.Ha,
                cfg.gnn_conv_ne ? P(p + "hne") : (const T*)nullptr, N, Mne, cfg.n_up, S, e, w.C);
      T* Xout;
      if (cfg.gnn_concat) {
        const int fin = 3 * dcur + nt * e;
        DQ_LAUNCH(gnn_concat_kernel<T>, dim3(Bc * S, N), dim3(128), 0, st, (const T*)X, dcur, (const T*)w.C, nt * e, N, cfg.n_up,
                  S, w.Fc);
        rc = gemm(w.Fc, fin, (p + "g.w").c_str(), nullptr, 0, d, cfg.gnn_g_bias ? P(p + "g.b") : nullptr, nullptr, 0, Xn, d, rows,
                  d, fin, S, 0, N, st);
        if (rc) return rc;
        const bool res = dcur == d;
        DQ_LAUNCH(act_fl_kernel<T>, dim3(groups, (d + 63) / 64), dim3(64), 0, st, Xn, d, res ? (const T*)X : (const T*)nullptr,
                  d, S, d, (res && cfg.gnn_res_norm) ? isq2 : T(1), 0);
        Xout = Xn; Xn = X;
      } else {
        T* G[3] = {w.G0, w.G1, w.G2};
        const T* res = dcur == d ? X : nullptr;
        for (int t = 0; t < nt; ++t) {
          rc = gemm(w.C + t * e, nt * e, (p + "g_" + tn[t] + ".w").c_str(), nullptr, 0, d, P(p + "g_" + tn[t] + ".b"), nullptr,
                    0, G[t], d, rows, d, e, S, 0, N, st);
          if (rc) return rc;
          const bool last = t == nt - 1;
          DQ_LAUNCH(act_fl_kernel<T>, dim3(groups, (d + 63) / 64), dim3(64), 0, st, G[t], d, res, d, S, d,
                    (last && res && cfg.gnn_res_norm) ? isq2 : T(1), 0);
          res = G[t];
        }
        Xout = G[nt - 1];
        T* old = X;
        if (nt == 3) w.G2 = old; else w.G1 = old;
      }
      X = Xout;
      dcur = d;
      if (cfg.gnn_deep_edges && l < cfg.n_layers - 1) {
        rc = gnn_mlp(E, ecur, p + "u", cfg.gnn_u_dims[l], nl, true, w.ET0, w.ET1, prow, 8, st);
        if (rc) return rc;
        if (ecur == e) {
          DQ_LAUNCH((axpby_kernel<T>), dim3((unsigned)(((size_t)prow * e + 255) / 256)), dim3(256), 0, st, (const T*)E,
                    (const T*)w.ET1, isq2, En, (size_t)prow * e);
          T* tmp = E; E = En; En = tmp;
        } else {
          T* tmp = E; E = w.ET1; w.ET1 = tmp;
        }
        ecur = e;
      }
    }
    *jastrow = nullptr;
    if (cfg.jastrow_n > 0) {
      const int jr = Bc * S;
      T* cur = w.Jb;
      int din = d;
      DQ_LAUNCH(sum_electrons_kernel<T>, dim3((jr * d + 127) / 128), dim3(128), 0, st, (const T*)X, N, S, d, cur, jr * d);
      for (int i = 0; i < cfg.jastrow_n; ++i) {
        const int dout = cfg.jastrow_dims[i];
        T* nxt = cur + (size_t)jr * din;
// ... 1283 lines not shown
    const int ne = B * 3 * N;
    for (int s = 0; s < n_sub; ++s) {
      const T* nns = nn ? (const T*)nn + (size_t)s * ne : nullptr;
      const T* nus = nu ? (const T*)nu + (size_t)s * B : nullptr;
      bool exchange = false;
      if (ex_flags) exchange = ex_flags[s] != 0;
      else if (p_exchange > 0.0) {
        uint32_t w4[4];
        Philox::gen(seed ^ 0xA0761D6478BD642Full, 0, step0 + (uint64_t)s, w4);
        exchange = Philox::u01(w4[0], w4[1]) < p_exchange;
      }
      if (exchange)
        DQ_LAUNCH(exchange_propose_kernel<T>, dim3((B + 127) / 128), dim3(128), 0, st, (const T*)r, q.r,
                  ex_idx ? ex_idx + (size_t)s * 2 * B : (const int32_t*)nullptr, seed, step0 + (uint64_t)s, woff, cfg.n_up, N, B);
      else
      DQ_LAUNCH(propose_kernel<T>, dim3((ne / 2 + 1 + 127) / 128), dim3(128), 0, st, (const T*)r, q.r, (const T*)tau, nns,
                seed, step0 + (uint64_t)s, woff * (uint64_t)(3 * N), ne);
      int rc = run_batched(q.r, R, Rb, B, 1, q.sign, q.logp, nullptr, nullptr, nullptr, a.top, a.left(), st);
      if (rc) return rc;
      DQ_LAUNCH(accept_kernel<T>, dim3((B + 127) / 128), dim3(128), 0, st, r, (const T*)q.r, sign, (const T*)q.sign, logp,
                (const T*)q.logp, age, nus, seed, step0 + (uint64_t)s, woff, exchange ? -1 : max_age, B, N, q.cnt);
      DQ_LAUNCH(tau_kernel<T>, dim3(1), dim3(32), 0, st, tau, q.cnt, B, exchange ? T(0) : (T)target, stats);
    }
    DQ_LAUNCH(sampler_stats_kernel<T>, dim3(1), dim3(256), 0, st, (const T*)r, (const T*)logp, (const int*)age,
              (const T*)tau, B, N, stats);
    DQ_CHECK(cudaGetLastError());
    return check_guards();
  }
};

}

struct dqmc_engine {
  dq::EngineBase* e;
};

#define DQ_NEED_DEVICE(h)                                                                        \
  do {                                                                                            \
    if ((h)->e->plan_only) {                                                                      \
      (h)->e->err = "plan-only engine (created with device < 0): no compute entry points";        \
      return 2;                                                                                   \
    }                                                                                             \
  } while (0)

extern "C" {

const char* dqmc_version(void) { return "dqmc_b200 0.1 (sm_90a)"; }

int dqmc_create(const dqmc_config* cfg, int device, dqmc_handle* out) {
  if (!cfg || !out) return 2;
  dq::EngineBase* e = nullptr;
  int rc = 0;
  const bool plan = device < 0;
  if (cfg->dtype == DQMC_F64) {
    auto* x = new dq::Engine<double>();
    x->cfg = *cfg; x->device = device; x->dry = x->plan_only = plan; rc = x->init(); e = x;
  } else if (cfg->dtype == DQMC_F32) {
    auto* x = new dq::Engine<float>();
    x->cfg = *cfg; x->device = device; x->dry = x->plan_only = plan; rc = x->init(); e = x;
  } else {
    return 2;
  }
  if (rc) {
    std::fprintf(stderr, "dqmc_create failed: %s\n", e->err.c_str());
    delete e;
    return rc;
  }
  *out = new dqmc_engine{e};
  return 0;
}
int dqmc_destroy(dqmc_handle h) {
  if (!h) return 2;
  delete h->e;
  delete h;
  return 0;
}
const char* dqmc_last_error(dqmc_handle h) { return h ? h->e->err.c_str() : "null handle"; }
int dqmc_param_count(dqmc_handle h) { return h ? (int)h->e->entries.size() : -1; }
int64_t dqmc_param_total(dqmc_handle h) { return h ? h->e->total : -1; }
int dqmc_param_entry(dqmc_handle h, int idx, char* name, int name_len, int64_t* offset, int32_t* rows, int32_t* cols) {
  if (!h || idx < 0 || idx >= (int)h->e->entries.size()) return 2;
  auto& en = h->e->entries[idx];
  if (name && name_len > 0) {
    std::strncpy(name, en.name.c_str(), name_len - 1);
    name[name_len - 1] = 0;
  }
  if (offset) *offset = en.offset;
  if (rows) *rows = en.rows;
  if (cols) *cols = en.cols;
  return 0;
}
int dqmc_set_params(dqmc_handle h, const double* host_params, int64_t n, void* stream) {
  if (!h) return 2;
  DQ_NEED_DEVICE(h);
  return h->e->set_params(host_params, n, (cudaStream_t)stream);
}
int64_t dqmc_workspace_bytes(dqmc_handle h, int32_t n_walkers, int32_t mode) {
  return h ? h->e->ws_bytes(n_walkers, mode) : -1;
}
int64_t dqmc_workspace_bytes_min(dqmc_handle h, int32_t n_walkers, int32_t mode) {
  return h ? h->e->ws_bytes_min(n_walkers, mode) : -1;
}
int dqmc_wf_forward(dqmc_handle h, const void* r, const void* R, int32_t R_batched, int32_t n_walkers, void* out_sign,
                    void* out_log, void* workspace, int64_t workspace_bytes, void* stream) {
  if (!h) return 2;
  DQ_NEED_DEVICE(h);
  if (n_walkers < 0) { h->e->err = "negative walker count"; return 2; }
  if (n_walkers == 0) return 0;
  return h->e->forward(r, R, R_batched, n_walkers, out_sign, out_log, workspace, workspace_bytes, (cudaStream_t)stream);
}
int dqmc_wf_orbitals(dqmc_handle h, const void* r, const void* R, int32_t R_batched, int32_t n_walkers, void* out_orbitals,
                     void* workspace, int64_t workspace_bytes, void* stream) {
  if (!h) return 2;
  DQ_NEED_DEVICE(h);
  if (n_walkers < 0) { h->e->err = "negative walker count"; return 2; }
  if (n_walkers == 0) return 0;
  return h->e->orbitals(r, R, R_batched, n_walkers, out_orbitals, workspace, workspace_bytes, (cudaStream_t)stream);
}
int dqmc_local_energy(dqmc_handle h, const void* r, const void* R, int32_t R_batched, int32_t n_walkers, uint64_t seed,
                      const void* ecp_twist, void* out_E, void* out_stats, void* out_sign, void* out_log,
                      void* out_grad, void* workspace, int64_t workspace_bytes, void* stream) {
  if (!h) return 2;
  DQ_NEED_DEVICE(h);
  if (n_walkers < 0) { h->e->err = "negative walker count"; return 2; }
  if (n_walkers == 0) return 0;
  return h->e->local_energy(r, R, R_batched, n_walkers, seed, ecp_twist, out_E, out_stats, out_sign, out_log, out_grad,
                            workspace, workspace_bytes, (cudaStream_t)stream);
}
int dqmc_mcmc_sweep(dqmc_handle h, void* r, void* sign, void* log, int32_t* age, void* tau, const void* R,
                    int32_t R_batched, int32_t n_walkers, int32_t n_sub, double target_acceptance, int32_t max_age,
                    uint64_t seed, uint64_t step0, uint64_t walker_offset, const void* noise_normal,
                    const void* noise_uniform, void* out_stats, void* workspace, int64_t workspace_bytes, void* stream) {
  if (!h) return 2;
  DQ_NEED_DEVICE(h);
  if (n_walkers < 1) { h->e->err = "the sampler needs at least one walker"; return 2; }
  return h->e->mcmc(r, sign, log, age, tau, R, R_batched, n_walkers, n_sub, target_acceptance, max_age, seed, step0,
                    walker_offset, noise_normal, noise_uniform, out_stats, workspace, workspace_bytes,
                    (cudaStream_t)stream);
}
int dqmc_mcmc_sweep_exchange(dqmc_handle h, void* r, void* sign, void* log, int32_t* age, void* tau, const void* R,
                             int32_t R_batched, int32_t n_walkers, int32_t n_sub, double target_acceptance, int32_t max_age,
                             uint64_t seed, uint64_t step0, uint64_t walker_offset, const void* noise_normal,
                             const void* noise_uniform, double exchange_step_probability, const int32_t* exchange_flags,
                             const int32_t* exchange_idx, void* out_stats, void* workspace, int64_t workspace_bytes,
                             void* stream) {
  if (!h) return 2;
  DQ_NEED_DEVICE(h);
  if (n_walkers < 1) { h->e->err = "the sampler needs at least one walker"; return 2; }
  if (h->e->cfg.n_up < 1 || h->e->cfg.n_down < 1) { h->e->err = "spin exchange needs electrons of both spins"; return 2; }
  return h->e->mcmc(r, sign, log, age, tau, R, R_batched, n_walkers, n_sub, target_acceptance, max_age, seed, step0,
                    walker_offset, noise_normal, noise_uniform, out_stats, workspace, workspace_bytes, (cudaStream_t)stream,
                    exchange_step_probability, exchange_flags, exchange_idx);
}
int dqmc_langevin_sweep(dqmc_handle h, void* r, void* sign, void* log, void* force, int32_t* age, void* tau, const void* R,
                        int32_t R_batched, int32_t n_walkers, int32_t n_sub, double target_acceptance, int32_t max_age,
                        uint64_t seed, uint64_t step0, uint64_t walker_offset, const void* noise_normal,
                        const void* noise_uniform, void* out_stats, void* workspace, int64_t workspace_bytes, void* stream) {
  if (!h) return 2;
  DQ_NEED_DEVICE(h);
  if (n_walkers < 1) { h->e->err = "the sampler needs at least one walker"; return 2; }
  return h->e->langevin(r, sign, log, force, age, tau, R, R_batched, n_walkers, n_sub, target_acceptance, max_age, seed, step0,
                        walker_offset, noise_normal, noise_uniform, out_stats, workspace, workspace_bytes, (cudaStream_t)stream);
}
int dqmc_wf_vjp_params(dqmc_handle h, const void* r, const void* R, int32_t R_batched, int32_t n_walkers, const void* weights,
                       void* out_sign, void* out_log, void* out_grad_params, void* workspace, int64_t workspace_bytes,
                       void* stream) {
  if (!h) return 2;
  DQ_NEED_DEVICE(h);
  if (n_walkers < 0) { h->e->err = "negative walker count"; return 2; }
  return h->e->vjp_params(r, R, R_batched, n_walkers, weights, out_sign, out_log, out_grad_params, workspace, workspace_bytes,
                          (cudaStream_t)stream);
}
int dqmc_spin(dqmc_handle h, const void* r, const void* R, int32_t R_batched, int32_t n_walkers, const void* sign,
              const void* log, int32_t down_idx, void* out_s2, void* out_ratio, void* workspace, int64_t workspace_bytes,
              void* stream) {
  if (!h) return 2;
  DQ_NEED_DEVICE(h);
  if (n_walkers < 0) { h->e->err = "negative walker count"; return 2; }
  return h->e->spin(r, R, R_batched, n_walkers, sign, log, down_idx, out_s2, out_ratio, workspace, workspace_bytes,
                    (cudaStream_t)stream);
}
int dqmc_wf_grad_positions(dqmc_handle h, const void* r, const void* R, int32_t R_batched, int32_t n_walkers, void* out_sign,
                           void* out_log, void* out_grad_r, void* out_grad_R, void* workspace, int64_t workspace_bytes,
                           void* stream) {
  if (!h) return 2;
  DQ_NEED_DEVICE(h);
  if (n_walkers < 0) { h->e->err = "negative walker count"; return 2; }
  if (n_walkers > 0 && (!r || !R || !out_sign || !out_log)) { h->e->err = "dqmc_wf_grad_positions: null array"; return 2; }
  return h->e->grad_positions(r, R, R_batched, n_walkers, out_sign, out_log, out_grad_r, out_grad_R, workspace, workspace_bytes,
                              (cudaStream_t)stream);
}
int dqmc_force_terms(dqmc_handle h, const void* r, const void* R, int32_t R_batched, int32_t n_walkers, const void* grad_r,
                     void* out_bare, void* out_zvq, void* out_Q, void* stream) {
  if (!h) return 2;
  DQ_NEED_DEVICE(h);
  if (n_walkers < 0) { h->e->err = "negative walker count"; return 2; }
  if (n_walkers > 0 && (!r || !R)) { h->e->err = "dqmc_force_terms: null array"; return 2; }
  return h->e->force_terms(r, R, R_batched, n_walkers, grad_r, out_bare, out_zvq, out_Q, (cudaStream_t)stream);
}
int dqmc_ecp_force(dqmc_handle h, const void* r, const void* R, int32_t R_batched, int32_t n_walkers, uint64_t seed,
                   const void* ecp_twist, void* out_bare, void* out_nl, void* workspace, int64_t workspace_bytes, void* stream) {
  if (!h) return 2;
  DQ_NEED_DEVICE(h);
  if (n_walkers < 0) { h->e->err = "negative walker count"; return 2; }
  if (n_walkers > 0 && (!r || !R)) { h->e->err = "dqmc_ecp_force: null array"; return 2; }
  return h->e->ecp_force(r, R, R_batched, n_walkers, seed, ecp_twist, out_bare, out_nl, workspace, workspace_bytes,
                         (cudaStream_t)stream);
}
int dqmc_zv_force(dqmc_handle h, const void* r, const void* R, int32_t R_batched, int32_t n_walkers, void* out_zv,
                  void* out_grad_R, void* workspace, int64_t workspace_bytes, void* stream) {
  if (!h) return 2;
  DQ_NEED_DEVICE(h);
  if (n_walkers < 0) { h->e->err = "negative walker count"; return 2; }
  if (n_walkers > 0 && (!r || !R || !out_zv)) { h->e->err = "dqmc_zv_force: null array"; return 2; }
  return h->e->zv_force(r, R, R_batched, n_walkers, out_zv, out_grad_R, workspace, workspace_bytes, (cudaStream_t)stream);
}
int dqmc_set_pseudo_hamiltonian(dqmc_handle h, int32_t n_tab, int32_t n_grid, double r_max, const double* tables,
                                const int32_t* tab_of_nuc) {
  if (!h) return 2;
  if (!h->e->plan_only) cudaSetDevice(h->e->device);
  return h->e->set_ph(n_tab, n_grid, r_max, tables, tab_of_nuc);
}
int dqmc_debug_plan(dqmc_handle h, int32_t n_walkers, int32_t mode, int64_t workspace_bytes, int64_t* planned_bytes,
                    int64_t* carved_bytes) {
  if (!h) return 2;
  if (n_walkers < 1) { h->e->err = "dqmc_debug_plan needs at least one walker"; return 2; }
  return h->e->debug_plan(n_walkers, mode, workspace_bytes, planned_bytes, carved_bytes);
}
int dqmc_stats_pack(dqmc_handle h, const void* E_loc, const void* stats, int32_t n_walkers, double* out11, void* stream) {
  if (!h) return 2;
  DQ_NEED_DEVICE(h);
  if (n_walkers < 1 || !E_loc || !out11) { h->e->err = "dqmc_stats_pack: bad arguments"; return 2; }
  return h->e->stats_pack(E_loc, stats, n_walkers, out11, (cudaStream_t)stream);
}
int64_t dqmc_launch_count(dqmc_handle h) { return h ? h->e->launches : -1; }
int64_t dqmc_ecp_forward_count(dqmc_handle h) { return h ? h->e->ecp_forwards : -1; }

int dqmc_debug_gemm(dqmc_handle h, const char* weight, const char* bias, const void* A, const void* Res, void* C,
                    int32_t rows, int32_t S, int32_t sliced, int32_t backend, void* stream) {
  if (!h) return 2;
  DQ_NEED_DEVICE(h);
  return h->e->debug_gemm(weight, bias, A, Res, C, rows, S, sliced, backend, (cudaStream_t)stream);
}

int dqmc_debug_mlp_block(dqmc_handle h, int32_t layer, const void* O, const void* X, void* Out, int32_t rows, void* stream) {
  if (!h) return 2;
  DQ_NEED_DEVICE(h);
  return h->e->debug_mlp_block(layer, O, X, Out, rows, (cudaStream_t)stream);
}
int dqmc_debug_trunk(dqmc_handle h, const void* X0, void* Out, int32_t rows, void* stream) {
  if (!h) return 2;
  DQ_NEED_DEVICE(h);
  return h->e->debug_trunk(X0, Out, rows, (cudaStream_t)stream);
}
int dqmc_debug_attention(dqmc_handle h, int32_t layer, const void* QKV, void* O, int32_t rows, int32_t S, int32_t* kernel,
                         void* stream) {
  if (!h) return 2;
  DQ_NEED_DEVICE(h);
  if (!QKV || !O) { h->e->err = "dqmc_debug_attention: null array"; return 2; }
  return h->e->debug_attention(layer, QKV, O, rows, S, kernel, (cudaStream_t)stream);
}
int dqmc_debug_mlp(dqmc_handle h, int32_t layer, int32_t S, const void* O, const void* X, void* Out, void* scratch, int32_t rows,
                   int32_t* path, void* stream) {
  if (!h) return 2;
  DQ_NEED_DEVICE(h);
  if (!O || !X || !Out || !scratch) { h->e->err = "dqmc_debug_mlp: null array"; return 2; }
  return h->e->debug_mlp(layer, S, O, X, Out, scratch, rows, path, (cudaStream_t)stream);
}
int dqmc_debug_slater(dqmc_handle h, const void* r, const void* R, const void* BF, int32_t rows, int32_t S, void* det_sign,
                      void* det_log, void* det_grad, void* det_lap, int32_t* kernel, void* stream) {
  if (!h) return 2;
  DQ_NEED_DEVICE(h);
  if (!r || !R || !BF || !det_sign || !det_log) { h->e->err = "dqmc_debug_slater: null array"; return 2; }
  return h->e->debug_slater(r, R, BF, rows, S, det_sign, det_log, det_grad, det_lap, kernel, (cudaStream_t)stream);
}
int dqmc_debug_det_sum(dqmc_handle h, const void* r, const void* R, const void* det_sign, const void* det_log,
                       const void* det_grad, const void* det_lap, int32_t B, int32_t S, void* sign, void* logp, void* grad,
                       void* stats, void* stream) {
  if (!h) return 2;
  DQ_NEED_DEVICE(h);
  if (!r || !R || !det_sign || !det_log || !sign || !logp) { h->e->err = "dqmc_debug_det_sum: null array"; return 2; }
  return h->e->debug_det_sum(r, R, det_sign, det_log, det_grad, det_lap, B, S, sign, logp, grad, stats, (cudaStream_t)stream);
}
int dqmc_debug_attention_bwd(dqmc_handle h, int32_t layer, const void* QKV, const void* dO, void* dQKV, void* dKn, void* dVn,
                             int32_t rows, void* stream) {
  if (!h) return 2;
  DQ_NEED_DEVICE(h);
  if (!QKV || !dO || !dQKV) { h->e->err = "dqmc_debug_attention_bwd: null array"; return 2; }
  return h->e->debug_attention_bwd(layer, QKV, dO, dQKV, dKn, dVn, rows, (cudaStream_t)stream);
}
int dqmc_debug_wgrad(dqmc_handle h, const void* A, const void* dY, int32_t rows, int32_t K, int32_t Nc, int32_t lo, int32_t hi,
                     void* dW, void* db, void* stream) {
  if (!h) return 2;
  DQ_NEED_DEVICE(h);
  if (!A || !dY || !dW || !db) { h->e->err = "dqmc_debug_wgrad: null array"; return 2; }
  return h->e->debug_wgrad(A, dY, rows, K, Nc, lo, hi, dW, db, (cudaStream_t)stream);
}
int dqmc_debug_trunk_phases(dqmc_handle h, uint64_t* out, int32_t n) {
  if (!h) return 2;
  DQ_NEED_DEVICE(h);
  if (!out) { h->e->err = "dqmc_debug_trunk_phases: null output"; return 2; }
  return h->e->debug_trunk_phases(out, n);
}

int dqmc_profile_begin(dqmc_handle h) {
  if (!h) return 2;
  h->e->prof = true; h->e->prof_flops = 0; h->e->prof_n = 0;
  for (int c = 0; c < 3; ++c) { h->e->prof_cls_flops[c] = 0; h->e->prof_cls_n[c] = 0; }
  h->e->prof_cls.clear();
  return 0;
}
int dqmc_profile_end_classes(dqmc_handle h, double* ms3, double* flops3, int64_t* n3) {
  if (!h) return 2;
  double ms[3] = {0, 0, 0};
#ifndef DQMC_EMU
  for (size_t i = 0; i + 1 < h->e->prof_ev.size(); i += 2) {
    cudaEventSynchronize(h->e->prof_ev[i + 1]);
    float t = 0;
    cudaEventElapsedTime(&t, h->e->prof_ev[i], h->e->prof_ev[i + 1]);
    ms[h->e->prof_cls[i / 2]] += t;
    cudaEventDestroy(h->e->prof_ev[i]); cudaEventDestroy(h->e->prof_ev[i + 1]);
  }
  h->e->prof_ev.clear();
#endif
  h->e->prof_cls.clear();
  h->e->prof = false;
  for (int c = 0; c < 3; ++c) {
    if (ms3) ms3[c] = ms[c];
    if (flops3) flops3[c] = h->e->prof_cls_flops[c];
    if (n3) n3[c] = h->e->prof_cls_n[c];
  }
  return 0;
}
int dqmc_profile_end(dqmc_handle h, double* gemm_ms, double* gemm_flops, int64_t* n_gemm) {
  double ms[3], fl[3];
  int64_t n[3];
  const int rc = dqmc_profile_end_classes(h, ms, fl, n);
  if (rc) return rc;
  if (gemm_ms) *gemm_ms = ms[0] + ms[1] + ms[2];
  if (gemm_flops) *gemm_flops = fl[0] + fl[1] + fl[2];
  if (n_gemm) *n_gemm = n[0] + n[1] + n[2];
  return 0;
}

}
```

deepqmc_b200/csrc/fused_tc.cuh:

```cuda
#pragma once
#include <cstdint>

#include "tc_ptx.cuh"

namespace dq {
namespace tc {

constexpr int kMlpThreads = 256;
constexpr int kMlpSlots = 3;

struct MlpParams {
  const float* O; int ldo;
  const float* X; int ldx;
  float* Out; int ldout;
  const float* b1; const float* b2;
  int M, d;
  float a_scale;
  float us0, us1, us2;
  int* err_flag;
};

struct MlpSmem {
  static __host__ __device__ int abuf(int kb, int plane) { return (kb * 2 + plane) * 16384; }
  static __host__ __device__ int wring(int wg, int s) { return 131072 + (wg * kMlpSlots + s) * 16384; }
  static __host__ __device__ int bars() { return 131072 + 2 * kMlpSlots * 16384; }
  static __host__ __device__ int phases() { return bars() + 64; }
  static __host__ __device__ int total() { return phases() + 2 * 8 * 16; }
};
__device__ __forceinline__ uint64_t* ring_full(unsigned char* smem, int wg) {
  return (uint64_t*)(smem + MlpSmem::bars()) + wg * kMlpSlots;
}
__device__ __forceinline__ uint64_t* mma_token(unsigned char* smem, int wg) {
  return (uint64_t*)(smem + MlpSmem::bars()) + 2 * kMlpSlots + wg;
}
__device__ __forceinline__ void init_rings(unsigned char* smem) {
  for (int i = 0; i < 2 * kMlpSlots + 2; ++i) mbar_init((uint64_t*)(smem + MlpSmem::bars()) + i, 1);
  fence_barrier_init();
}
__device__ __forceinline__ void start_pingpong(unsigned char* smem) {
  if (threadIdx.x == 128) mbar_arrive(mma_token(smem, 0));
}

enum Phase {
  kPhLoad, kPhQkv, kPhQkvEpi, kPhAttn, kPhWo, kPhWoEpi, kPhW1, kPhW1Epi, kPhW2, kPhW2Epi, kPhWait, kPhTurn, kPhPairs, kPhases
};
static_assert(kPhases <= 16, "MlpSmem::phases() holds 16 counters per warpgroup");
struct PhaseClock {
  unsigned long long* acc;
  long long t;
  __device__ __forceinline__ explicit PhaseClock(unsigned long long* a) : acc(a), t(0) {
    if (a) t = clock64();
  }
  __device__ __forceinline__ void mark(int k) {
    if (acc) {
      const long long n = clock64();
      acc[k] += (unsigned long long)(n - t);
      t = n;
    }
  }
  __device__ __forceinline__ void count(int k) { if (acc) acc[k] += 1; }
  __device__ __forceinline__ void waited(long long w, int k) {
    acc[k] += (unsigned long long)w;
    t += w;
  }
};

__device__ __forceinline__ float mlp_tanh(float x) {
  const float x2 = x * x;
  const float poly = x + x * x2 * (-0.33333333333f + x2 * (0.13333333333f + x2 * (-0.05396825397f)));
  const float e = ex2_approx(x * 2.8853900817779268f);
  const float big = 1.f - fast_div(2.f, 1.f + e);
  return fabsf(x) < 0.15f ? poly : big;
}

__device__ __forceinline__ void split_half2(float x0, float x1, uint32_t& hi, uint32_t& lo) {
  const float c0 = __fmul_rn(x0, 8193.f), c1 = __fmul_rn(x1, 8193.f);
  const float h0 = __fsub_rn(c0, __fsub_rn(c0, x0)), h1 = __fsub_rn(c1, __fsub_rn(c1, x1));
  hi = pack_half2_rn(h0, h1);
  lo = pack_half2_rn(__fsub_rn(x0, h0), __fsub_rn(x1, h1));
}

__device__ __forceinline__ int operand_off(int row, int col) {
  const int cc = col & 63;
  return (row >> 3) * 1024 + (row & 7) * 128 + ((((cc >> 3) ^ row) & 7) << 4) + (cc & 7) * 2;
}
__device__ __forceinline__ void store_operand_pair(unsigned char* smem, int row, int col, float a0, float a1) {
  uint32_t h, l;
  split_half2(a0, a1, h, l);
  const int off = operand_off(row, col), kb = col >> 6;
  *(uint32_t*)(smem + MlpSmem::abuf(kb, 0) + off) = h;
  *(uint32_t*)(smem + MlpSmem::abuf(kb, 1) + off) = l;
}
__device__ __forceinline__ void store_operand_quad(unsigned char* smem, int row, int col, float4 a) {
  uint32_t h01, l01, h23, l23;
  split_half2(a.x, a.y, h01, l01);
  split_half2(a.z, a.w, h23, l23);
  const int off = operand_off(row, col), kb = col >> 6;
  *(uint2*)(smem + MlpSmem::abuf(kb, 0) + off) = make_uint2(h01, h23);
  *(uint2*)(smem + MlpSmem::abuf(kb, 1) + off) = make_uint2(l01, l23);
}

struct Ring {
  uint32_t nslot = 0, nturn = 0;
};
enum Turn { kTurnTake = 1, kTurnPass = 2, kTurnOwn = kTurnTake | kTurnPass, kTurnKeep = 0 };

template <int D>
__device__ __forceinline__ void gemm_abuf(float (&acc)[D / 2], unsigned char* smem, Ring& ring, const CUtensorMap* mh,
                                          const CUtensorMap* ml, int y0, int turn, int* err, PhaseClock& pc) {
  uint32_t& nslot = ring.nslot;
  constexpr int KB = D / 64;
  constexpr int NS = 4 * KB;
  static_assert(NS >= kMlpSlots, "the ring is filled at the start of a GEMM");
  constexpr uint32_t kSlot = D * 64u;
  const int wg = threadIdx.x >> 7;
  const bool leader = (threadIdx.x & 127) == 0;
  uint64_t* full = ring_full(smem, wg);
#pragma unroll
  for (int i = 0; i < D / 2; ++i) acc[i] = 0.f;
  auto stage = [&](int i) { return (int)((nslot + (uint32_t)i) % (uint32_t)kMlpSlots); };
  auto load = [&](int i) {
    const int st = stage(i);
    mbar_expect_tx(&full[st], kSlot);
    tma_load_2d(((i >> 1) & 1) ? ml : mh, &full[st], smem + MlpSmem::wring(wg, st), (i >> 2) * 64 + (i & 1) * 32, y0);
  };
  if (leader)
    for (int i = 0; i < kMlpSlots; ++i) load(i);
  if (turn & kTurnTake) {
    const long long t0 = pc.acc ? clock64() : 0;
    mbar_wait(mma_token(smem, wg), ring.nturn & 1u, err);
    ++ring.nturn;
    if (pc.acc) pc.waited(clock64() - t0, kPhTurn);
  }
  auto acquire = [&](int i) {
    const int st = stage(i);
    const long long t0 = pc.acc ? clock64() : 0;
    mbar_wait(&full[st], ((nslot + (uint32_t)i) / (uint32_t)kMlpSlots) & 1u, err);
    if (pc.acc) pc.waited(clock64() - t0, kPhWait);
    return smem_u32(smem + MlpSmem::wring(wg, st));
  };
  auto retire = [&](int i) {
    wgmma_wait1();
    if (i == 0) return;
    wg_sync(wg);
    if (leader && i + kMlpSlots - 1 < NS) load(i + kMlpSlots - 1);
  };
  auto mma = [&](float (&d)[D / 2], uint32_t a, uint32_t w, int accumulate) {
    if constexpr (D == 256) wgmma_f16_n256(d, make_desc(a), make_desc64(w), accumulate);
    else wgmma_f16_n128(d, make_desc(a), make_desc64(w), accumulate);
  };
#pragma unroll 1
  for (int kb = 0; kb < KB; ++kb) {
    const uint32_t ah = smem_u32(smem + MlpSmem::abuf(kb, 0)) + wg * 8192, al = smem_u32(smem + MlpSmem::abuf(kb, 1)) + wg * 8192;
#pragma unroll
    for (int q = 0; q < 2; ++q) {
      const uint32_t w = acquire(4 * kb + q);
      wgmma_fence();
#pragma unroll
      for (int kk = 0; kk < 2; ++kk) {
        const int k = 2 * q + kk;
        mma(acc, al + 32 * k, w + 32 * kk, (kb | k) ? 1 : 0);
        mma(acc, ah + 32 * k, w + 32 * kk, 1);
      }
      wgmma_commit();
      retire(4 * kb + q);
    }
#pragma unroll
    for (int q = 0; q < 2; ++q) {
      const uint32_t w = acquire(4 * kb + 2 + q);
      wgmma_fence();
#pragma unroll
      for (int kk = 0; kk < 2; ++kk) mma(acc, ah + 32 * (2 * q + kk), w + 32 * kk, 1);
      wgmma_commit();
      retire(4 * kb + 2 + q);
    }
  }
  if ((turn & kTurnPass) && leader) mbar_arrive(mma_token(smem, wg ^ 1));
  wgmma_wait0();
  fence_acc(acc);
  wg_sync(wg);
  nslot += NS;
}

struct Frag {
  int fr, fc;
  __device__ __forceinline__ Frag() {
    const int tid = threadIdx.x, lane = tid & 31;
    fr = 64 * (tid >> 7) + 16 * ((tid >> 5) & 3) + (lane >> 2);
    fc = 2 * (lane & 3);
  }
};

enum MlpEpi { kEpiWo, kEpiW1, kEpiW2 };
template <int E>
__device__ __forceinline__ void mlp_epi_pair(unsigned char* smem, int row, int c, float acc0, float acc1, float2 r, float us,
                                             const float* bias, float a_scale, float* gout, bool operand) {
  float v0, v1;
  if constexpr (E == kEpiWo) {
    v0 = r.x + acc0 * us;
    v1 = r.y + acc1 * us;
  } else {
    const float2 b = make_float2(__ldg(bias + c), __ldg(bias + c + 1));
    if constexpr (E == kEpiW1) {
      v0 = mlp_tanh(acc0 * us + b.x);
      v1 = mlp_tanh(acc1 * us + b.y);
    } else {
      v0 = r.x + mlp_tanh(acc0 * us + b.x);
      v1 = r.y + mlp_tanh(acc1 * us + b.y);
    }
  }
  if (E != kEpiW1 && gout) *(float2*)(gout + c) = make_float2(v0, v1);
  if (operand) store_operand_pair(smem, row, c, v0 * a_scale, v1 * a_scale);
}

template <int D, int E>
__device__ __forceinline__ void mlp_epilogue(float (&acc)[D / 2], unsigned char* smem, float us, const float* bias,
                                             float a_scale, const float* const (&rin)[2], float* const (&gout)[2], bool operand) {
  const Frag f;
  constexpr int QJ = D / 32;
  constexpr int kJ = 4;
#pragma unroll 1
  for (int q = 0; q < 4; ++q) {
#pragma unroll
    for (int jb = 0; jb < QJ; jb += kJ) {
      float2 r[kJ][2];
#pragma unroll
      for (int j = 0; j < kJ; ++j)
#pragma unroll
        for (int h = 0; h < 2; ++h)
          r[j][h] = E != kEpiW1 && rin[h] ? *(const float2*)(rin[h] + 8 * (QJ * q + jb + j) + f.fc) : make_float2(0.f, 0.f);
#pragma unroll
      for (int j = 0; j < kJ; ++j)
#pragma unroll
        for (int h = 0; h < 2; ++h) {
          if (E == kEpiW2 && !rin[h]) continue;
          mlp_epi_pair<E>(smem, f.fr + 8 * h, 8 * (QJ * q + jb + j) + f.fc, acc[4 * (jb + j) + 2 * h],
                          acc[4 * (jb + j) + 2 * h + 1], r[j][h], us, bias, a_scale, gout[h], E != kEpiW2 || operand);
        }
    }
#pragma unroll
    for (int i = 0; i < D / 2 - D / 8; ++i) acc[i] = acc[i + D / 8];
  }
}

template <int D>
__device__ __forceinline__ void mlp3(float (&acc)[D / 2], unsigned char* smem, Ring& ring, const CUtensorMap* const (&wmaps)[6],
                                     float us0, float us1, float us2, float a_scale, const float* b1, const float* b2,
                                     const float* const (&xin)[2], float* const (&aout)[2], float* const (&xout)[2],
                                     bool operand_out, int* err, PhaseClock& pc) {
  const int wg = threadIdx.x >> 7;
#pragma unroll 1
  for (int g = 0; g < 3; ++g) {
    const CUtensorMap* mh = g == 0 ? wmaps[0] : (g == 1 ? wmaps[2] : wmaps[4]);
    const CUtensorMap* ml = g == 0 ? wmaps[1] : (g == 1 ? wmaps[3] : wmaps[5]);
    gemm_abuf<D>(acc, smem, ring, mh, ml, 0, kTurnOwn, err, pc);
    pc.mark(kPhWo + 2 * g);
    if (g == 0) {
      mlp_epilogue<D, kEpiWo>(acc, smem, us0, nullptr, a_scale, xin, aout, true);
      fence_proxy_async();
      wg_sync(wg);
      pc.mark(kPhWoEpi);
    } else if (g == 1) {
      mlp_epilogue<D, kEpiW1>(acc, smem, us1, b1, a_scale, xin, aout, true);
      fence_proxy_async();
      wg_sync(wg);
      pc.mark(kPhW1Epi);
    } else {
      const float* const ain[2] = {aout[0], aout[1]};
      mlp_epilogue<D, kEpiW2>(acc, smem, us2, b2, a_scale, ain, xout, operand_out);
      pc.mark(kPhW2Epi);
    }
  }
}

template <int D>
__global__ void __launch_bounds__(kMlpThreads, 1)
mlp_block_f16_kernel(const __grid_constant__ CUtensorMap wo_hi, const __grid_constant__ CUtensorMap wo_lo,
                     const __grid_constant__ CUtensorMap w1_hi, const __grid_constant__ CUtensorMap w1_lo,
                     const __grid_constant__ CUtensorMap w2_hi, const __grid_constant__ CUtensorMap w2_lo, MlpParams p) {
  DQMC_TC_SMEM(smem);
  if ((smem_u32(smem) & 1023u) != 0u) tc_trap();
  const int tid = threadIdx.x, wg = tid >> 7;
  const int MT = (p.M + 127) / 128;

  if (tid == 0) {
    init_rings(smem);
    tma_prefetch_desc(&wo_hi); tma_prefetch_desc(&wo_lo); tma_prefetch_desc(&w1_hi);
    tma_prefetch_desc(&w1_lo); tma_prefetch_desc(&w2_hi); tma_prefetch_desc(&w2_lo);
  }
  __syncthreads();
  start_pingpong(smem);
  const Frag f;
  Ring ring;
  float acc[D / 2];
  PhaseClock pc(nullptr);
  for (int tile = blockIdx.x; tile < MT; tile += gridDim.x) {
    for (int idx = tid & 127; idx < 64 * (D / 4); idx += 128) {
      const int r = 64 * wg + idx / (D / 4), c = 4 * (idx % (D / 4));
      const int grow = tile * 128 + r;
      float4 v = make_float4(0.f, 0.f, 0.f, 0.f);
      if (grow < p.M) v = __ldg((const float4*)(p.O + (size_t)grow * p.ldo + c));
      const float sc = p.a_scale;
      store_operand_quad(smem, r, c, make_float4(v.x * sc, v.y * sc, v.z * sc, v.w * sc));
    }
    fence_proxy_async();
    wg_sync(wg);
    const float* xin[2];
    float* aout[2];
#pragma unroll
    for (int h = 0; h < 2; ++h) {
      const int grow = tile * 128 + f.fr + 8 * h;
      const bool valid = grow < p.M;
      xin[h] = valid ? p.X + (size_t)grow * p.ldx : nullptr;
      aout[h] = valid ? p.Out + (size_t)grow * p.ldout : nullptr;
    }
    const CUtensorMap* const wmaps[6] = {&wo_hi, &wo_lo, &w1_hi, &w1_lo, &w2_hi, &w2_lo};
    mlp3<D>(acc, smem, ring, wmaps, p.us0, p.us1, p.us2, p.a_scale, p.b1, p.b2, xin, aout, aout, false, p.err_flag, pc);
  }
}

}
}
```

deepqmc_b200/csrc/tc_ptx.cuh:

```cuda
#pragma once
#include <cuda.h>
#include <cuda_runtime.h>

#include <cstdint>

#define DQMC_TC_SMEM(name) extern __shared__ __align__(1024) unsigned char name[]

namespace dq {
namespace tc {

__device__ __forceinline__ uint32_t smem_u32(const void* p) { return (uint32_t)__cvta_generic_to_shared(p); }

__device__ __forceinline__ void mbar_init(uint64_t* bar, uint32_t count) {
  asm volatile("mbarrier.init.shared::cta.b64 [%0], %1;" ::"r"(smem_u32(bar)), "r"(count));
}
__device__ __forceinline__ void mbar_expect_tx(uint64_t* bar, uint32_t bytes) {
  asm volatile("mbarrier.arrive.expect_tx.shared::cta.b64 _, [%0], %1;" ::"r"(smem_u32(bar)), "r"(bytes) : "memory");
}
__device__ __forceinline__ void mbar_wait(uint64_t* bar, uint32_t parity, int* err_flag) {
  uint32_t done = 0;
  const long long t0 = clock64();
  while (true) {
    asm volatile(
        "{\n\t.reg .pred p;\n\t"
        "mbarrier.try_wait.parity.shared::cta.b64 p, [%1], %2;\n\t"
        "selp.u32 %0, 1, 0, p;\n\t}"
        : "=r"(done)
        : "r"(smem_u32(bar)), "r"(parity)
        : "memory");
    if (done) break;
    if (clock64() - t0 > 4000000000LL) {
      if (err_flag) atomicExch(err_flag, 1);
      __trap();
    }
  }
}
__device__ __forceinline__ void mbar_arrive(uint64_t* bar) {
  asm volatile("mbarrier.arrive.shared::cta.b64 _, [%0];" ::"r"(smem_u32(bar)) : "memory");
}
__device__ __forceinline__ void wg_sync(int wg) { asm volatile("bar.sync %0, 128;" ::"r"(1 + wg) : "memory"); }
__device__ __forceinline__ void fence_proxy_async() { asm volatile("fence.proxy.async.shared::cta;" ::: "memory"); }
__device__ __forceinline__ void ldsm_x4(uint32_t saddr, uint32_t (&r)[4]) {
  asm volatile("ldmatrix.sync.aligned.m8n8.x4.shared.b16 {%0,%1,%2,%3}, [%4];"
               : "=r"(r[0]), "=r"(r[1]), "=r"(r[2]), "=r"(r[3]) : "r"(saddr) : "memory");
}
__device__ __forceinline__ void fence_barrier_init() { asm volatile("fence.mbarrier_init.release.cluster;" ::: "memory"); }

__device__ __forceinline__ void tma_load_2d(const CUtensorMap* map, uint64_t* bar, void* dst, int x, int y) {
  asm volatile(
      "cp.async.bulk.tensor.2d.shared::cluster.global.mbarrier::complete_tx::bytes [%0], [%1, {%3, %4}], [%2];"
      ::"r"(smem_u32(dst)), "l"(map), "r"(smem_u32(bar)), "r"(x), "r"(y)
      : "memory");
}
__device__ __forceinline__ void tma_prefetch_desc(const CUtensorMap* map) {
  asm volatile("prefetch.tensormap [%0];" ::"l"(map) : "memory");
}

__device__ __forceinline__ uint64_t make_desc(uint32_t saddr) {
  uint64_t d = 0;
  d |= (uint64_t)((saddr >> 4) & 0x3FFF);
  d |= (uint64_t)1 << 16;
  d |= (uint64_t)(1024 >> 4) << 32;
  d |= (uint64_t)1 << 62;
  return d;
}
__device__ __forceinline__ uint64_t make_desc64(uint32_t saddr) {
  uint64_t d = 0;
  d |= (uint64_t)((saddr >> 4) & 0x3FFF);
  d |= (uint64_t)1 << 16;
  d |= (uint64_t)(512 >> 4) << 32;
  d |= (uint64_t)2 << 62;
  return d;
}

__device__ __forceinline__ void wgmma_fence() { asm volatile("wgmma.fence.sync.aligned;" ::: "memory"); }
__device__ __forceinline__ void wgmma_commit() { asm volatile("wgmma.commit_group.sync.aligned;" ::: "memory"); }
__device__ __forceinline__ void wgmma_wait0() { asm volatile("wgmma.wait_group.sync.aligned 0;" ::: "memory"); }
__device__ __forceinline__ void wgmma_wait1() { asm volatile("wgmma.wait_group.sync.aligned 1;" ::: "memory"); }
template <int R>
__device__ __forceinline__ void fence_acc(float (&d)[R]) {
#pragma unroll
  for (int i = 0; i < R; ++i) asm volatile("" : "+f"(d[i])::"memory");
}

__device__ __forceinline__ void wgmma_tf32_n128(float* d, uint64_t da, uint64_t db, int acc) {
  asm volatile(
      "{\n\t.reg .pred p;\n\tsetp.ne.b32 p, %66, 0;\n\t"
      "wgmma.mma_async.sync.aligned.m64n128k8.f32.tf32.tf32 "
      "{"
      "%0, %1, %2, %3, %4, %5, %6, %7, %8, %9, %10, %11, %12, %13, %14, %15,"
      "%16, %17, %18, %19, %20, %21, %22, %23, %24, %25, %26, %27, %28, %29, %30, %31,"
      "%32, %33, %34, %35, %36, %37, %38, %39, %40, %41, %42, %43, %44, %45, %46, %47,"
      "%48, %49, %50, %51, %52, %53, %54, %55, %56, %57, %58, %59, %60, %61, %62, %63"
      "}, %64, %65, p, 1, 1;\n\t}"
      : "+f"(d[0]), "+f"(d[1]), "+f"(d[2]), "+f"(d[3]), "+f"(d[4]), "+f"(d[5]), "+f"(d[6]), "+f"(d[7]),
        "+f"(d[8]), "+f"(d[9]), "+f"(d[10]), "+f"(d[11]), "+f"(d[12]), "+f"(d[13]), "+f"(d[14]), "+f"(d[15]),
        "+f"(d[16]), "+f"(d[17]), "+f"(d[18]), "+f"(d[19]), "+f"(d[20]), "+f"(d[21]), "+f"(d[22]), "+f"(d[23]),
        "+f"(d[24]), "+f"(d[25]), "+f"(d[26]), "+f"(d[27]), "+f"(d[28]), "+f"(d[29]), "+f"(d[30]), "+f"(d[31]),
        "+f"(d[32]), "+f"(d[33]), "+f"(d[34]), "+f"(d[35]), "+f"(d[36]), "+f"(d[37]), "+f"(d[38]), "+f"(d[39]),
        "+f"(d[40]), "+f"(d[41]), "+f"(d[42]), "+f"(d[43]), "+f"(d[44]), "+f"(d[45]), "+f"(d[46]), "+f"(d[47]),
        "+f"(d[48]), "+f"(d[49]), "+f"(d[50]), "+f"(d[51]), "+f"(d[52]), "+f"(d[53]), "+f"(d[54]), "+f"(d[55]),
        "+f"(d[56]), "+f"(d[57]), "+f"(d[58]), "+f"(d[59]), "+f"(d[60]), "+f"(d[61]), "+f"(d[62]), "+f"(d[63])
      : "l"(da), "l"(db), "r"(acc));
}
__device__ __forceinline__ void wgmma_f16_n128(float* d, uint64_t da, uint64_t db, int acc) {
  asm volatile(
      "{\n\t.reg .pred p;\n\tsetp.ne.b32 p, %66, 0;\n\t"
      "wgmma.mma_async.sync.aligned.m64n128k16.f32.f16.f16 "
      "{"
      "%0, %1, %2, %3, %4, %5, %6, %7, %8, %9, %10, %11, %12, %13, %14, %15,"
      "%16, %17, %18, %19, %20, %21, %22, %23, %24, %25, %26, %27, %28, %29, %30, %31,"
      "%32, %33, %34, %35, %36, %37, %38, %39, %40, %41, %42, %43, %44, %45, %46, %47,"
      "%48, %49, %50, %51, %52, %53, %54, %55, %56, %57, %58, %59, %60, %61, %62, %63"
      "}, %64, %65, p, 1, 1, 0, 0;\n\t}"
      : "+f"(d[0]), "+f"(d[1]), "+f"(d[2]), "+f"(d[3]), "+f"(d[4]), "+f"(d[5]), "+f"(d[6]), "+f"(d[7]),
        "+f"(d[8]), "+f"(d[9]), "+f"(d[10]), "+f"(d[11]), "+f"(d[12]), "+f"(d[13]), "+f"(d[14]), "+f"(d[15]),
        "+f"(d[16]), "+f"(d[17]), "+f"(d[18]), "+f"(d[19]), "+f"(d[20]), "+f"(d[21]), "+f"(d[22]), "+f"(d[23]),
        "+f"(d[24]), "+f"(d[25]), "+f"(d[26]), "+f"(d[27]), "+f"(d[28]), "+f"(d[29]), "+f"(d[30]), "+f"(d[31]),
        "+f"(d[32]), "+f"(d[33]), "+f"(d[34]), "+f"(d[35]), "+f"(d[36]), "+f"(d[37]), "+f"(d[38]), "+f"(d[39]),
        "+f"(d[40]), "+f"(d[41]), "+f"(d[42]), "+f"(d[43]), "+f"(d[44]), "+f"(d[45]), "+f"(d[46]), "+f"(d[47]),
        "+f"(d[48]), "+f"(d[49]), "+f"(d[50]), "+f"(d[51]), "+f"(d[52]), "+f"(d[53]), "+f"(d[54]), "+f"(d[55]),
        "+f"(d[56]), "+f"(d[57]), "+f"(d[58]), "+f"(d[59]), "+f"(d[60]), "+f"(d[61]), "+f"(d[62]), "+f"(d[63])
      : "l"(da), "l"(db), "r"(acc));
}
__device__ __forceinline__ void wgmma_f16_n256(float* d, uint64_t da, uint64_t db, int acc) {
  asm volatile(
      "{\n\t.reg .pred p;\n\tsetp.ne.b32 p, %130, 0;\n\t"
      "wgmma.mma_async.sync.aligned.m64n256k16.f32.f16.f16 "
      "{"
      "%0, %1, %2, %3, %4, %5, %6, %7, %8, %9, %10, %11, %12, %13, %14, %15,"
      "%16, %17, %18, %19, %20, %21, %22, %23, %24, %25, %26, %27, %28, %29, %30, %31,"
      "%32, %33, %34, %35, %36, %37, %38, %39, %40, %41, %42, %43, %44, %45, %46, %47,"
      "%48, %49, %50, %51, %52, %53, %54, %55, %56, %57, %58, %59, %60, %61, %62, %63,"
      "%64, %65, %66, %67, %68, %69, %70, %71, %72, %73, %74, %75, %76, %77, %78, %79,"
      "%80, %81, %82, %83, %84, %85, %86, %87, %88, %89, %90, %91, %92, %93, %94, %95,"
      "%96, %97, %98, %99, %100, %101, %102, %103, %104, %105, %106, %107, %108, %109, %110, %111,"
      "%112, %113, %114, %115, %116, %117, %118, %119, %120, %121, %122, %123, %124, %125, %126, %127"
      "}, %128, %129, p, 1, 1, 0, 0;\n\t}"
      : "+f"(d[0]), "+f"(d[1]), "+f"(d[2]), "+f"(d[3]), "+f"(d[4]), "+f"(d[5]), "+f"(d[6]), "+f"(d[7]),
        "+f"(d[8]), "+f"(d[9]), "+f"(d[10]), "+f"(d[11]), "+f"(d[12]), "+f"(d[13]), "+f"(d[14]), "+f"(d[15]),
        "+f"(d[16]), "+f"(d[17]), "+f"(d[18]), "+f"(d[19]), "+f"(d[20]), "+f"(d[21]), "+f"(d[22]), "+f"(d[23]),
        "+f"(d[24]), "+f"(d[25]), "+f"(d[26]), "+f"(d[27]), "+f"(d[28]), "+f"(d[29]), "+f"(d[30]), "+f"(d[31]),
        "+f"(d[32]), "+f"(d[33]), "+f"(d[34]), "+f"(d[35]), "+f"(d[36]), "+f"(d[37]), "+f"(d[38]), "+f"(d[39]),
        "+f"(d[40]), "+f"(d[41]), "+f"(d[42]), "+f"(d[43]), "+f"(d[44]), "+f"(d[45]), "+f"(d[46]), "+f"(d[47]),
        "+f"(d[48]), "+f"(d[49]), "+f"(d[50]), "+f"(d[51]), "+f"(d[52]), "+f"(d[53]), "+f"(d[54]), "+f"(d[55]),
        "+f"(d[56]), "+f"(d[57]), "+f"(d[58]), "+f"(d[59]), "+f"(d[60]), "+f"(d[61]), "+f"(d[62]), "+f"(d[63]),
        "+f"(d[64]), "+f"(d[65]), "+f"(d[66]), "+f"(d[67]), "+f"(d[68]), "+f"(d[69]), "+f"(d[70]), "+f"(d[71]),
        "+f"(d[72]), "+f"(d[73]), "+f"(d[74]), "+f"(d[75]), "+f"(d[76]), "+f"(d[77]), "+f"(d[78]), "+f"(d[79]),
        "+f"(d[80]), "+f"(d[81]), "+f"(d[82]), "+f"(d[83]), "+f"(d[84]), "+f"(d[85]), "+f"(d[86]), "+f"(d[87]),
        "+f"(d[88]), "+f"(d[89]), "+f"(d[90]), "+f"(d[91]), "+f"(d[92]), "+f"(d[93]), "+f"(d[94]), "+f"(d[95]),
        "+f"(d[96]), "+f"(d[97]), "+f"(d[98]), "+f"(d[99]), "+f"(d[100]), "+f"(d[101]), "+f"(d[102]), "+f"(d[103]),
        "+f"(d[104]), "+f"(d[105]), "+f"(d[106]), "+f"(d[107]), "+f"(d[108]), "+f"(d[109]), "+f"(d[110]), "+f"(d[111]),
        "+f"(d[112]), "+f"(d[113]), "+f"(d[114]), "+f"(d[115]), "+f"(d[116]), "+f"(d[117]), "+f"(d[118]), "+f"(d[119]),
        "+f"(d[120]), "+f"(d[121]), "+f"(d[122]), "+f"(d[123]), "+f"(d[124]), "+f"(d[125]), "+f"(d[126]), "+f"(d[127])
      : "l"(da), "l"(db), "r"(acc));
}

__device__ __forceinline__ float ex2_approx(float x) {
  float e;
  asm("ex2.approx.ftz.f32 %0, %1;" : "=f"(e) : "f"(x));
  return e;
}
__device__ __forceinline__ float fast_div(float a, float b) { return __fdividef(a, b); }
__device__ __forceinline__ uint32_t pack_half2_rn(float lo, float hi) {
  uint32_t r;
  asm("cvt.rn.f16x2.f32 %0, %1, %2;" : "=r"(r) : "f"(hi), "f"(lo));
  return r;
}
__device__ __forceinline__ float half_bits_to_float(uint32_t h16) {
  float f;
  asm("{\n\t.reg .b16 h;\n\tcvt.u16.u32 h, %1;\n\tcvt.f32.f16 %0, h;\n\t}" : "=f"(f) : "r"(h16));
  return f;
}
__device__ __forceinline__ void tc_trap() { __trap(); }
__device__ __forceinline__ float tf32_rna(float x) {
  uint32_t r;
  asm("cvt.rna.tf32.f32 %0, %1;" : "=r"(r) : "f"(x));
  return __uint_as_float(r);
}

typedef CUresult (*EncodeTiledFn)(CUtensorMap*, CUtensorMapDataType, cuuint32_t, void*, const cuuint64_t*,
                                  const cuuint64_t*, const cuuint32_t*, const cuuint32_t*, CUtensorMapInterleave,
                                  CUtensorMapSwizzle, CUtensorMapL2promotion, CUtensorMapFloatOOBfill);

inline EncodeTiledFn get_encode_fn() {
  static EncodeTiledFn fn = nullptr;
  if (!fn) {
    void* ptr = nullptr;
    cudaDriverEntryPointQueryResult q;
    if (cudaGetDriverEntryPoint("cuTensorMapEncodeTiled", &ptr, cudaEnableDefault, &q) == cudaSuccess && ptr)
      fn = (EncodeTiledFn)ptr;
  }
  return fn;
}
inline int make_kmajor_map(CUtensorMap* map, const void* base, int elem_bytes, int rows, int K, int box_k, int box_rows) {
  EncodeTiledFn fn = get_encode_fn();
  if (!fn) return 1;
  const int inner = box_k * elem_bytes;
  if ((inner != 128 && inner != 64) || (elem_bytes != 4 && elem_bytes != 2)) return 3;
  cuuint64_t gdim[2] = {(cuuint64_t)K, (cuuint64_t)rows};
  cuuint64_t gstr[1] = {(cuuint64_t)K * (cuuint64_t)elem_bytes};
  cuuint32_t box[2] = {(cuuint32_t)box_k, (cuuint32_t)box_rows};
  cuuint32_t estr[2] = {1, 1};
  CUresult r = fn(map, elem_bytes == 4 ? CU_TENSOR_MAP_DATA_TYPE_FLOAT32 : CU_TENSOR_MAP_DATA_TYPE_FLOAT16, 2, (void*)base, gdim,
                  gstr, box, estr, CU_TENSOR_MAP_INTERLEAVE_NONE,
                  inner == 128 ? CU_TENSOR_MAP_SWIZZLE_128B : CU_TENSOR_MAP_SWIZZLE_64B, CU_TENSOR_MAP_L2_PROMOTION_L2_256B,
                  CU_TENSOR_MAP_FLOAT_OOB_FILL_NONE);
  return r == CUDA_SUCCESS ? 0 : 2;
}

}
}
```

deepqmc_b200/csrc/trunk_tc.cuh:

```cuda
#pragma once
#include <cstdint>

#include "attn_mma.cuh"
#include "common.cuh"
#include "fused_tc.cuh"
#include "tc_ptx.cuh"

namespace dq {
namespace tc {

constexpr int kTrThreads = 256;
constexpr int kTrMaxLayers = 8;
constexpr int kTrKvBytes = 128 * 512 * 4;
constexpr int kTrScratchPerCta = kTrKvBytes + 128 * 256 * 4;
using TrSmem = MlpSmem;

struct TrunkParams {
  const float* X0; int ldx;
  const float* Xbase;
  long long v0; int vper;
  int n_up, vlayout;
  const int* pairs;
  const float* wspin;
  float* Out; int ldout;
  const CUtensorMap* maps;
  const float* b1[kTrMaxLayers];
  const float* b2[kTrMaxLayers];
  float us[kTrMaxLayers][4];
  unsigned char* scratch;
  int walkers, N, L;
  float a_scale;
  float attn_scale;
  int* err_flag;
  unsigned long long* phase;
};

template <int NP>
__global__ void __launch_bounds__(kTrThreads, 1)
trunk_f16_kernel(TrunkParams p) {
  static_assert(NP >= 1 && NP <= 32 && (NP & (NP - 1)) == 0, "walker slot: a power of two <= 32");
  DQMC_TC_SMEM(smem);
  if ((smem_u32(smem) & 1023u) != 0u) tc_trap();

  const int tid = threadIdx.x, wg = tid >> 7;
  const int N = p.N, L = p.L;
  constexpr int lnp = NP == 1 ? 0 : NP == 2 ? 1 : NP == 4 ? 2 : NP == 8 ? 3 : NP == 16 ? 4 : 5;
  constexpr int G = 128 / NP;
  const int MT = (p.walkers + G - 1) / G;
  uint2* kbuf = (uint2*)(p.scratch + (size_t)blockIdx.x * kTrScratchPerCta);
  uint2* vbuf = kbuf + 128 * 128;
  float* resid = (float*)(vbuf + 64 * 256);

  if (tid == 0) {
    init_rings(smem);
    for (int i = 0; i < 8 * L; ++i) tma_prefetch_desc(p.maps + i);
  }
  unsigned long long* ph = (unsigned long long*)(smem + TrSmem::phases());
  if (tid < 32) ph[tid] = 0ull;
  __syncthreads();
  start_pingpong(smem);
  PhaseClock pc(p.phase && (tid & 127) == 0 ? ph + 16 * wg : nullptr);
  const Frag f;
  Ring ring;
  float acc[128];
  const int lane = tid & 31, r0 = 16 * (tid >> 5), ag = lane >> 2;
  const int k0 = r0 & ~((NP > 16 ? NP : 16) - 1);
  for (int tile = blockIdx.x; tile < MT; tile += gridDim.x) {
    auto grow_of = [&](int r) -> long long {
      const int walker = tile * G + (r >> lnp), el = r & (NP - 1);
      return (el < N && walker < p.walkers) ? (long long)walker * N + el : -1;
    };
#pragma unroll 1
    for (int i0 = 0; i0 < 64 * 64 / 128; i0 += 8) {
      float4 x[8];
#pragma unroll
      for (int i = 0; i < 8; ++i) {
        const int idx = (tid & 127) + 128 * (i0 + i), r = 64 * wg + (idx >> 6), c = 4 * (idx & 63);
        const long long row = grow_of(r);
        x[i] = make_float4(0.f, 0.f, 0.f, 0.f);
        if (row >= 0) {
          const float* xrow = p.X0 + (size_t)row * p.ldx;
          float sw = 0.f;
          if (p.vper > 0) {
            const int walker = tile * G + (r >> lnp), el = r & (NP - 1);
            const VirtualMove mv = virtual_move((int)p.v0 + walker, p.vper, N, p.n_up, p.vlayout, p.pairs);
            if (mv.e1 < 0) {
              xrow = el == mv.e0 ? p.X0 + (size_t)walker * p.ldx : p.Xbase + ((size_t)mv.base * N + el) * p.ldx;
            } else {
              const int src = el == mv.e0 ? mv.e1 : (el == mv.e1 ? mv.e0 : el);
              xrow = p.Xbase + ((size_t)mv.base * N + src) * p.ldx;
              sw = el == mv.e0 ? 2.f : (el == mv.e1 ? -2.f : 0.f);
            }
          }
          x[i] = __ldg((const float4*)(xrow + c));
          if (sw != 0.f) {
            const float4 ws = __ldg((const float4*)(p.wspin + c));
            x[i].x += sw * ws.x; x[i].y += sw * ws.y; x[i].z += sw * ws.z; x[i].w += sw * ws.w;
          }
        }
      }
#pragma unroll
      for (int i = 0; i < 8; ++i) {
        const int idx = (tid & 127) + 128 * (i0 + i), r = 64 * wg + (idx >> 6), c = 4 * (idx & 63);
        *(float4*)(resid + r * 256 + c) = x[i];
        const float sc = p.a_scale;
        store_operand_quad(smem, r, c, make_float4(x[i].x * sc, x[i].y * sc, x[i].z * sc, x[i].w * sc));
      }
    }
    fence_proxy_async();
    wg_sync(wg);
    pc.mark(kPhLoad);
    for (int l = 0; l < L; ++l) {
      const bool last = l == L - 1;
      const CUtensorMap* lm = p.maps + 8 * l;
#pragma unroll 1
      for (int j = 0; j < 3; ++j) {
        const int blk = j == 2 ? 0 : j + 1;
        const int turn = j == 0 ? kTurnTake : (j == 2 ? kTurnPass : kTurnKeep);
        gemm_abuf<256>(acc, smem, ring, lm, lm + 1, 256 * blk, turn, p.err_flag, pc);
        pc.mark(kPhQkv);
        const float us = p.us[l][0];
        const int odd = ag & 1;
        uint2* gdst[2];
#pragma unroll
        for (int h = 0; h < 2; ++h) {
          const int r = f.fr + 8 * h;
          gdst[h] = blk == 1 ? kbuf + r * 128 + (f.fc >> 1) : vbuf + (r >> 1) * 256 + f.fc + odd;
        }
        const int gq = blk == 1 ? 32 : 64;
#pragma unroll 1
        for (int q = 0; q < 4; ++q) {
#pragma unroll
          for (int jj = 0; jj < 8; ++jj)
#pragma unroll
            for (int h = 0; h < 2; ++h) {
              const int r = f.fr + 8 * h, c = 64 * q + 8 * jj + f.fc;
              float x0 = acc[4 * jj + 2 * h] * us * kAmQS, x1 = acc[4 * jj + 2 * h + 1] * us * kAmQS;
              if (blk == 2) {
                const float y = __shfl_xor_sync(0xffffffffu, odd ? x0 : x1, 4);
                x0 = odd ? y : x0;
                x1 = odd ? x1 : y;
              }
              uint2 v;
              am_split2(x0, x1, v.x, v.y);
              if (blk != 0) {
                gdst[h][gq * q + (gq >> 3) * jj] = v;
              } else if ((r & (NP - 1)) < N) {
                const int off = operand_off(r, c);
                *(uint32_t*)(smem + MlpSmem::abuf(q, 0) + off) = v.x;
                *(uint32_t*)(smem + MlpSmem::abuf(q, 1) + off) = v.y;
              }
            }
#pragma unroll
          for (int i = 0; i < 96; ++i) acc[i] = acc[i + 32];
        }
        pc.mark(kPhQkvEpi);
      }
      wg_sync(wg);
      for (int h = 0; h < 4; ++h) {
        const uint32_t qhi = smem_u32(smem + MlpSmem::abuf(h, 0)), qlo = smem_u32(smem + MlpSmem::abuf(h, 1));
        auto ldq = [&](int kt, uint32_t (&qh)[4], uint32_t (&ql)[4]) {
          const int off = operand_off(r0 + (lane & 15), 16 * kt + 8 * (lane >> 4));
          ldsm_x4(qhi + off, qh);
          ldsm_x4(qlo + off, ql);
        };
        auto ldk = [&](int nt, int kt, uint32_t (&kh)[2], uint32_t (&kl)[2]) {
          const uint2* kp = kbuf + (k0 + nt * 8 + ag) * 128 + 32 * h + 8 * kt + (lane & 3);
          const uint2 a = kp[0], b = kp[4];
          kh[0] = a.x; kl[0] = a.y; kh[1] = b.x; kl[1] = b.y;
        };
        auto ldv = [&](int kk, int nt, auto keep, uint32_t (&vh)[2], uint32_t (&vl)[2]) {
          const int j = 16 * kk + 2 * (lane & 3);
          const uint2* vp = vbuf + ((k0 + j) >> 1) * 256 + 64 * h + 8 * nt + ag;
          const uint2 a = vp[0], b = vp[4 * 256];
          auto sel = [](uint32_t x, bool lo, bool hi) { return (lo ? x & 0xFFFFu : 0u) | (hi ? x & 0xFFFF0000u : 0u); };
          vh[0] = sel(a.x, keep(j), keep(j + 1)); vl[0] = sel(a.y, keep(j), keep(j + 1));
          vh[1] = sel(b.x, keep(j + 8), keep(j + 9)); vl[1] = sel(b.y, keep(j + 8), keep(j + 9));
        };
        auto valid = [&](int i, int j) {
          const int r = r0 + ag + 8 * i, k = k0 + j;
          return (k >> lnp) == (r >> lnp) && (k & (NP - 1)) < N;
        };
        auto store = [&](int i, int c, float o0, float o1) {
          const int r = r0 + ag + 8 * i;
          if ((r & (NP - 1)) < N) store_operand_pair(smem, r, 64 * h + c, o0 * p.a_scale, o1 * p.a_scale);
        };
        attn_task_frag<(NP > 16 ? 4 : 2)>(p.attn_scale, ldq, ldk, ldv, valid, store, NP < 16 ? NP : 0);
      }
      fence_proxy_async();
      wg_sync(wg);
      pc.mark(kPhAttn);
      const float* xin[2];
      float* aout[2];
      float* xout[2];
#pragma unroll
      for (int h = 0; h < 2; ++h) {
        const int r = f.fr + 8 * h;
        xin[h] = resid + r * 256;
        aout[h] = resid + r * 256;
        const long long row = grow_of(r);
        xout[h] = !last ? resid + r * 256 : (row >= 0 ? p.Out + (size_t)row * p.ldout : nullptr);
      }
      const CUtensorMap* const wmaps[6] = {lm + 2, lm + 3, lm + 4, lm + 5, lm + 6, lm + 7};
      mlp3<256>(acc, smem, ring, wmaps, p.us[l][1], p.us[l][2], p.us[l][3], p.a_scale, p.b1[l], p.b2[l], xin, aout, xout,
                !last, p.err_flag, pc);
      fence_proxy_async();
      wg_sync(wg);
      pc.mark(kPhW2Epi);
      if (tid < 128) pc.count(kPhPairs);
    }
  }
  if (pc.acc)
    for (int k = 0; k < kPhases; ++k) atomicAdd(p.phase + k, pc.acc[k]);
}

}
}
```

deepqmc_b200/engine.py:

```python
from __future__ import annotations

import ctypes as C

import numpy as np
import torch

from . import _lib
from . import params as PN
from .spec import AnsatzSpec

MODE_FORWARD, MODE_LOCAL_ENERGY, MODE_VJP, MODE_MCMC, MODE_LANGEVIN, MODE_SPIN, MODE_GRAD_POS, MODE_ECP_FORCE = 0, 1, 2, 3, 4, 5, 6, 7
MODE_ZV_FORCE = 8
_TORCH_DTYPE = {0: torch.float64, 1: torch.float32}


def paulinet_backflow_hidden(spec: AnsatzSpec) -> list[int]:
    du, dd = PN.backflow_dims(spec, spec.n_up)[:-1], PN.backflow_dims(spec, spec.n_down)[:-1]
    return [max(a, b) for a, b in zip(du, dd)]


def paulinet_env_rep(spec: AnsatzSpec) -> int:
    return max(max((spec.env_centers.count(c) for c in set(spec.env_centers)), default=1), 1)


# ... 502 lines not shown
            from .nuclear import nuclear_stream_vjp

            def e(name):
                off, rows, cols = self.entries[name]
                return flat[off:off + rows * cols].reshape(rows, cols).detach().cpu().double().numpy()

            N, K, M, E = self.spec.n_elec, self.spec.n_determinants, self.spec.n_nuc, self.spec.n_env_per_nuc
            cot = {'kn': [e(f'L{l}.kn') for l in range(self.spec.n_layers)],
                   'vn': [e(f'L{l}.vn') for l in range(self.spec.n_layers)]}
            for s_, t in (('up', 'up'), ('down', 'dn')):
                cot[f'zetas_{s_}'] = e(f'env.zeta_{t}').reshape(K, N, M, E).sum(1).transpose(1, 0, 2)
            host = nuclear_stream_vjp(self.spec, self._params, self._nuc_R, cot)
            for k, v in host.items():
                v = v.to(device=self.device, dtype=self.dtype)
                grads[k] = grads[k] + v.reshape(grads[k].shape) if k in grads else v
        return sign, log, grads

    def spin(self, r, R, sign=None, log=None, down_idx=-1, want_ratios=False, max_ws_bytes=None):
        r = self._prep(r)
        B = r.shape[0]
        R, Rb = self._R(R, B)
        n_up, n_down = self.spec.n_up, self.spec.n_down
        P = n_up * n_down if down_idx < 0 else n_up
        s2 = torch.empty(B, dtype=self.dtype, device=self.device)
        ratio = torch.empty(B, P, dtype=self.dtype, device=self.device) if want_ratios else None
        sg = self._prep(sign) if sign is not None else None
        lg = self._prep(log) if log is not None else None
        ptr = lambda t: t.data_ptr() if t is not None else None
        ws = self.workspace(B, MODE_SPIN, max_ws_bytes)
        rc = self.lib.dqmc_spin(self.h, r.data_ptr(), R.data_ptr(), Rb, B, ptr(sg), ptr(lg), int(down_idx), s2.data_ptr(),
                                ptr(ratio), ws.data_ptr(), ws.numel(), self._stream())
        self._check(rc, 'dqmc_spin')
        return s2, ratio

    def grad_positions(self, r, R, want_r=True, want_R=True, max_ws_bytes=None):
        r = self._prep(r)
        B, N = r.shape[0], r.shape[1]
        R, Rb = self._R(R, B)
        mk = lambda *s: torch.empty(*s, dtype=self.dtype, device=self.device)
        sign, log = mk(B), mk(B)
        gr = mk(B, N, 3) if want_r else None
        gR = mk(B, self.spec.n_nuc, 3) if want_R else None
        ptr = lambda t: t.data_ptr() if t is not None else None
        ws = self.workspace(B, MODE_GRAD_POS, max_ws_bytes)
        rc = self.lib.dqmc_wf_grad_positions(self.h, r.data_ptr(), R.data_ptr(), Rb, B, sign.data_ptr(), log.data_ptr(), ptr(gr),
                                             ptr(gR), ws.data_ptr(), ws.numel(), self._stream())
        self._check(rc, 'dqmc_wf_grad_positions')
        return sign, log, gr, gR

    def force_terms(self, r, R, grad_r=None):
        r = self._prep(r)
        B = r.shape[0]
        R, Rb = self._R(R, B)
        mk = lambda *s: torch.empty(*s, dtype=self.dtype, device=self.device)
        M = self.spec.n_nuc
        bare, Q = mk(B, M, 3), mk(B, M, 3)
        g = self._prep(grad_r).reshape(B, -1) if grad_r is not None else None
        zvq = mk(B, M, 3) if g is not None else None
        ptr = lambda t: t.data_ptr() if t is not None else None
        rc = self.lib.dqmc_force_terms(self.h, r.data_ptr(), R.data_ptr(), Rb, B, ptr(g), bare.data_ptr(), ptr(zvq), Q.data_ptr(),
                                       self._stream())
        self._check(rc, 'dqmc_force_terms')
        return bare, zvq, Q

    def ecp_force(self, r, R, seed=0, ecp_twist=None, want_nl=True, max_ws_bytes=None):
        r = self._prep(r)
        B = r.shape[0]
        R, Rb = self._R(R, B)
        mk = lambda *s: torch.empty(*s, dtype=self.dtype, device=self.device)
        M = self.spec.n_nuc
        bare = mk(B, M, 3)
        nl = mk(B, M, 3) if want_nl else None
        tw = self._prep(ecp_twist) if ecp_twist is not None else None
        ptr = lambda t: t.data_ptr() if t is not None else None
        ws = self.workspace(B, MODE_ECP_FORCE, max_ws_bytes) if want_nl else None
        rc = self.lib.dqmc_ecp_force(self.h, r.data_ptr(), R.data_ptr(), Rb, B, seed, ptr(tw), bare.data_ptr(), ptr(nl), ptr(ws),
                                     ws.numel() if ws is not None else 0, self._stream())
        self._check(rc, 'dqmc_ecp_force')
        return bare, nl

    def zv_force(self, r, R, want_grad_R=False, max_ws_bytes=None):
        r = self._prep(r)
        B = r.shape[0]
        R, Rb = self._R(R, B)
        mk = lambda *s: torch.empty(*s, dtype=self.dtype, device=self.device)
        M = self.spec.n_nuc
        zv = mk(B, M, 3)
        gR = mk(B, M, 3) if want_grad_R else None
        ws = self.workspace(B, MODE_ZV_FORCE, max_ws_bytes)
        rc = self.lib.dqmc_zv_force(self.h, r.data_ptr(), R.data_ptr(), Rb, B, zv.data_ptr(),
                                    gR.data_ptr() if gR is not None else None, ws.data_ptr(), ws.numel(), self._stream())
        self._check(rc, 'dqmc_zv_force')
        return zv, gR

    def mcmc_sweep(self, state, R, n_sub, target_acceptance=0.57, max_age=None, seed=0, step0=0, walker_offset=0,
                   noise_normal=None, noise_uniform=None, max_ws_bytes=None, exchange_probability=0.0, exchange_flags=None,
                   exchange_idx=None):
        r = state['r']
        B = r.shape[0]
        for k in ('r', 'sign', 'log', 'tau'):
            assert state[k].dtype == self.dtype and state[k].is_contiguous() and state[k].device == self.device, k
        assert state['age'].dtype == torch.int32
        R, Rb = self._R(R, B)
        nn = self._prep(noise_normal) if noise_normal is not None else None
        nu = self._prep(noise_uniform) if noise_uniform is not None else None
        stats = torch.zeros(7, dtype=self.dtype, device=self.device)
        ws = self.workspace(B, MODE_MCMC, max_ws_bytes)
        if exchange_probability > 0.0 or exchange_flags is not None:
            flags = None
            if exchange_flags is not None:
                flags = (C.c_int32 * n_sub)(*[int(f) for f in exchange_flags])
            xi = None
            if exchange_idx is not None:
                xi = exchange_idx.to(device=self.device, dtype=torch.int32).contiguous()
                assert xi.shape == (n_sub, B, 2)
            rc = self.lib.dqmc_mcmc_sweep_exchange(
                self.h, r.data_ptr(), state['sign'].data_ptr(), state['log'].data_ptr(), state['age'].data_ptr(),
                state['tau'].data_ptr(), R.data_ptr(), Rb, B, n_sub, float(target_acceptance if target_acceptance else 0.0),
                -1 if max_age is None else int(max_age), seed, step0, walker_offset,
                nn.data_ptr() if nn is not None else None, nu.data_ptr() if nu is not None else None,
                float(exchange_probability), flags, xi.data_ptr() if xi is not None else None,
                stats.data_ptr(), ws.data_ptr(), ws.numel(), self._stream())
            self._check(rc, 'dqmc_mcmc_sweep_exchange')
            return stats
        rc = self.lib.dqmc_mcmc_sweep(
            self.h, r.data_ptr(), state['sign'].data_ptr(), state['log'].data_ptr(), state['age'].data_ptr(),
            state['tau'].data_ptr(), R.data_ptr(), Rb, B, n_sub, float(target_acceptance if target_acceptance else 0.0),
            -1 if max_age is None else int(max_age), seed, step0, walker_offset,
            nn.data_ptr() if nn is not None else None, nu.data_ptr() if nu is not None else None,
            stats.data_ptr(), ws.data_ptr(), ws.numel(), self._stream())
        self._check(rc, 'dqmc_mcmc_sweep')
        return stats

    def langevin_sweep(self, state, R, n_sub, target_acceptance=0.57, max_age=None, seed=0, step0=0, walker_offset=0,
                       noise_normal=None, noise_uniform=None):
        r = state['r']
        B, N = r.shape[0], r.shape[1]
        for k in ('r', 'sign', 'log', 'force', 'tau'):
            assert state[k].dtype == self.dtype and state[k].is_contiguous() and state[k].device == self.device, k
        assert state['age'].dtype == torch.int32
        R, Rb = self._R(R, B)
        nn = self._prep(noise_normal) if noise_normal is not None else None
        nu = self._prep(noise_uniform) if noise_uniform is not None else None
        stats = torch.zeros(7, dtype=self.dtype, device=self.device)
        ws = self.workspace(B, MODE_LANGEVIN)
        rc = self.lib.dqmc_langevin_sweep(
            self.h, r.data_ptr(), state['sign'].data_ptr(), state['log'].data_ptr(), state['force'].data_ptr(),
            state['age'].data_ptr(), state['tau'].data_ptr(), R.data_ptr(), Rb, B, n_sub,
            float(target_acceptance if target_acceptance else 0.0), -1 if max_age is None else int(max_age), seed, step0,
            walker_offset, nn.data_ptr() if nn is not None else None, nu.data_ptr() if nu is not None else None,
            stats.data_ptr(), ws.data_ptr(), ws.numel(), self._stream())
        self._check(rc, 'dqmc_langevin_sweep')
        return stats

    def debug_gemm(self, weight, A, bias=None, Res=None, S=1, sliced=False, backend=0):
        off, K, Nc = self.entries[weight]
        A = self._prep(A)
        rows = A.shape[0]
        out_rows = rows
        Cout = torch.zeros(out_rows, Nc, dtype=self.dtype, device=self.device)
        Res = self._prep(Res) if Res is not None else None
        rc = self.lib.dqmc_debug_gemm(self.h, weight.encode(), bias.encode() if bias else None, A.data_ptr(),
                                      Res.data_ptr() if Res is not None else None, Cout.data_ptr(),
                                      rows // self.spec.n_elec if sliced else rows, S, int(sliced),
                                      backend, self._stream())
        self._check(rc, 'dqmc_debug_gemm')
        return Cout

    def stats_pack(self, E, stats=None):
        out = torch.empty(11, dtype=torch.float64, device=self.device)
        assert E.dtype == self.dtype and E.is_contiguous() and (stats is None or (stats.is_contiguous() and stats.shape == (6, E.shape[0])))
        rc = self.lib.dqmc_stats_pack(self.h, E.data_ptr(), stats.data_ptr() if stats is not None else None, E.shape[0],
                                      out.data_ptr(), self._stream())
        self._check(rc, 'dqmc_stats_pack')
        return out

    def debug_plan(self, n_walkers: int, mode: int, workspace_bytes: int = 0):
        pl, cv = C.c_int64(), C.c_int64()
        rc = self.lib.dqmc_debug_plan(self.h, n_walkers, mode, workspace_bytes, C.byref(pl), C.byref(cv))
        self._check(rc, 'dqmc_debug_plan')
        return pl.value, cv.value

    def workspace_bytes(self, n_walkers: int, mode: int) -> int:
        return self.lib.dqmc_workspace_bytes(self.h, n_walkers, mode)

    def workspace_bytes_min(self, n_walkers: int, mode: int) -> int:
        return self.lib.dqmc_workspace_bytes_min(self.h, n_walkers, mode)

    def debug_mlp_block(self, layer, O, X):
        O, X = self._prep(O), self._prep(X)
        out = torch.empty_like(O)
        rc = self.lib.dqmc_debug_mlp_block(self.h, layer, O.data_ptr(), X.data_ptr(), out.data_ptr(), O.shape[0], self._stream())
        self._check(rc, 'dqmc_debug_mlp_block')
        return out

    def debug_trunk(self, X0):
        X0 = self._prep(X0)
        assert X0.dim() == 2 and X0.shape[1] == self.spec.embedding_dim and X0.shape[0] % self.spec.n_elec == 0, tuple(X0.shape)
        out = torch.empty_like(X0)
        rc = self.lib.dqmc_debug_trunk(self.h, X0.data_ptr(), out.data_ptr(), X0.shape[0], self._stream())
        self._check(rc, 'dqmc_debug_trunk')
        return out

    ATTN_KERNELS = ('attn_fwd_mma_kernel', 'attn_fl_f32_kernel', 'attn_fl_kernel', 'attn_fl_f32_kernel_mma', 'attn_fl_kernel_mma')

    def debug_attention(self, layer, QKV, S=1):
        QKV = self._prep(QKV)
        d = self.spec.embedding_dim
        assert QKV.dim() == 2 and QKV.shape[1] == 3 * d and QKV.shape[0] % (self.spec.n_elec * S) == 0, tuple(QKV.shape)
        out = torch.empty(QKV.shape[0], d, dtype=self.dtype, device=self.device)
        kernel = C.c_int32(-1)
        rc = self.lib.dqmc_debug_attention(self.h, layer, QKV.data_ptr(), out.data_ptr(), QKV.shape[0], S, C.byref(kernel),
                                           self._stream())
        self._check(rc, 'dqmc_debug_attention')
        return out, self.ATTN_KERNELS[kernel.value]

    MLP_PATHS = ('mlp_block', 'gemm_fused_tanh', 'gemm_tanh_fl_kernel', 'simt_gemm_tanh_fl_kernel')

    def debug_mlp(self, layer, O, X, S=1):
        O, X = self._prep(O), self._prep(X)
        d = self.spec.embedding_dim
        assert O.shape == X.shape and O.dim() == 2 and O.shape[1] == d and O.shape[0] % (self.spec.n_elec * S) == 0, tuple(O.shape)
        out = torch.empty_like(O)
        scratch = torch.empty(2 * O.shape[0], d, dtype=self.dtype, device=self.device)
        path = C.c_int32(-1)
        rc = self.lib.dqmc_debug_mlp(self.h, layer, S, O.data_ptr(), X.data_ptr(), out.data_ptr(), scratch.data_ptr(), O.shape[0],
                                     C.byref(path), self._stream())
        self._check(rc, 'dqmc_debug_mlp')
        return out, self.MLP_PATHS[path.value]

    SLATER_KERNELS = ('slater_small_kernel', 'slater_fwd2_kernel', 'slater_fwd_reg_kernel', 'slater_kernel')

    def _nuclei(self):
        return self._prep(self.hamil.mol.coords)

    def debug_slater(self, r, BF, S=1):
        r, BF = self._prep(r), self._prep(BF)
        N, K = self.spec.n_elec, self.spec.n_determinants
        B = r.shape[0]
        assert r.shape == (B, N, 3) and BF.dim() == 2 and BF.shape[0] == B * N * S, (tuple(r.shape), tuple(BF.shape))
        mk = lambda *s: torch.empty(*s, dtype=self.dtype, device=self.device)
        sign, log = mk(B, K), mk(B, K)
        grad, lap = (mk(B, K, 3 * N), mk(B, K)) if S > 1 else (None, None)
        kernel = (C.c_int32 * 2)(-1, -1)
        ptr = lambda t: t.data_ptr() if t is not None else None
        R = self._nuclei()
        rc = self.lib.dqmc_debug_slater(self.h, r.data_ptr(), R.data_ptr(), BF.data_ptr(), BF.shape[0], S,
                                        sign.data_ptr(), log.data_ptr(), ptr(grad), ptr(lap), kernel, self._stream())
        self._check(rc, 'dqmc_debug_slater')
        name = self.SLATER_KERNELS[kernel[0]] + (f'<{kernel[1]}>' if kernel[1] else '')
        return sign, log, grad, lap, name

    def debug_det_sum(self, r, det_sign, det_log, det_grad=None, det_lap=None):
        r, det_sign, det_log = self._prep(r), self._prep(det_sign), self._prep(det_log)
        N = self.spec.n_elec
        B = r.shape[0]
        S = 3 * N + 2 if det_grad is not None else 1
        mk = lambda *s: torch.empty(*s, dtype=self.dtype, device=self.device)
        sign, log = mk(B), mk(B)
        grad, stats = (mk(B, 3 * N), mk(6, B)) if S > 1 else (None, None)
        ptr = lambda t: t.data_ptr() if t is not None else None
        dg = self._prep(det_grad) if det_grad is not None else None
        dl = self._prep(det_lap) if det_lap is not None else None
        R = self._nuclei()
        rc = self.lib.dqmc_debug_det_sum(self.h, r.data_ptr(), R.data_ptr(), det_sign.data_ptr(),
                                         det_log.data_ptr(), ptr(dg), ptr(dl), B, S, sign.data_ptr(), log.data_ptr(),
                                         ptr(grad), ptr(stats), self._stream())
        self._check(rc, 'dqmc_debug_det_sum')
        return sign, log, grad, stats

    def debug_attention_bwd(self, layer, QKV, dO):
        QKV, dO = self._prep(QKV), self._prep(dO)
        d = self.spec.embedding_dim
        assert QKV.dim() == 2 and QKV.shape[1] == 3 * d and dO.shape == (QKV.shape[0], d), (tuple(QKV.shape), tuple(dO.shape))
        dQKV = torch.empty_like(QKV)
        Mn = self.spec.n_nuc if self.spec.kind == 'transpsiformer' else 0
        dKn = torch.zeros(Mn, d, dtype=self.dtype, device=self.device) if Mn else None
        dVn = torch.zeros(Mn, d, dtype=self.dtype, device=self.device) if Mn else None
        ptr = lambda t: t.data_ptr() if t is not None else None
        rc = self.lib.dqmc_debug_attention_bwd(self.h, layer, QKV.data_ptr(), dO.data_ptr(), dQKV.data_ptr(), ptr(dKn), ptr(dVn),
                                               QKV.shape[0], self._stream())
        self._check(rc, 'dqmc_debug_attention_bwd')
        return dQKV, dKn, dVn

    def debug_wgrad(self, A, dY, lo=0, hi=-1):
        A, dY = self._prep(A), self._prep(dY)
        assert A.dim() == 2 and dY.dim() == 2 and A.shape[0] == dY.shape[0], (tuple(A.shape), tuple(dY.shape))
        dW = torch.zeros(A.shape[1], dY.shape[1], dtype=self.dtype, device=self.device)
        db = torch.zeros(dY.shape[1], dtype=self.dtype, device=self.device)
        rc = self.lib.dqmc_debug_wgrad(self.h, A.data_ptr(), dY.data_ptr(), A.shape[0], A.shape[1], dY.shape[1], lo, hi,
                                       dW.data_ptr(), db.data_ptr(), self._stream())
        self._check(rc, 'dqmc_debug_wgrad')
        return dW, db

    TRUNK_PHASES = ('tile_load', 'qkv_mainloop', 'qkv_epilogue', 'attention', 'wo_mainloop', 'wo_epilogue', 'w1_mainloop',
                    'w1_epilogue', 'w2_mainloop', 'w2_epilogue', 'weight_wait', 'mma_turn', 'tile_layer_pairs')

    def debug_trunk_phases(self):
        out = (C.c_uint64 * len(self.TRUNK_PHASES))()
        rc = self.lib.dqmc_debug_trunk_phases(self.h, out, len(out))
        self._check(rc, 'dqmc_debug_trunk_phases')
        return dict(zip(self.TRUNK_PHASES, out))

    def profile_begin(self):
        self.lib.dqmc_profile_begin(self.h)

    def profile_end(self):
        ms, fl, n = C.c_double(), C.c_double(), C.c_int64()
        self.lib.dqmc_profile_end(self.h, C.byref(ms), C.byref(fl), C.byref(n))
        return ms.value, fl.value, n.value

    PROFILE_CLASSES = ('row_gemm', 'mlp_block', 'trunk')

    def profile_end_classes(self):
        ms, fl, n = (C.c_double * 3)(), (C.c_double * 3)(), (C.c_int64 * 3)()
        self.lib.dqmc_profile_end_classes(self.h, ms, fl, n)
        return {k: (ms[i], fl[i], n[i]) for i, k in enumerate(self.PROFILE_CLASSES)}

    @property
    def launch_count(self):
        return self.lib.dqmc_launch_count(self.h)

    @property
    def ecp_forward_count(self):
        return self.lib.dqmc_ecp_forward_count(self.h)

    def close(self):
        if getattr(self, 'h', None):
            self.lib.dqmc_destroy(self.h)
            self.h = None

    def __del__(self):
        try:
            self.close()
        except Exception:
            pass
```

include/dqmc_b200.h:

```cpp
#ifndef DQMC_B200_H
#define DQMC_B200_H
#include <stdint.h>

#ifdef __cplusplus
extern "C" {
#endif

#define DQMC_MAX_NUC 32
#define DQMC_MAX_ECP_TERMS 4
#define DQMC_MAX_ECP_L 4

enum { DQMC_PSIFORMER = 0, DQMC_FERMINET = 1, DQMC_TRANSPSIFORMER = 2, DQMC_PAULINET = 3 };
enum { DQMC_F64 = 0, DQMC_F32 = 1 };
enum { DQMC_GEMM_SIMT = 0, DQMC_GEMM_TCGEN05 = 1 };
enum { DQMC_MODE_FORWARD = 0, DQMC_MODE_LOCAL_ENERGY = 1, DQMC_MODE_VJP = 2, DQMC_MODE_MCMC = 3, DQMC_MODE_LANGEVIN = 4,
       DQMC_MODE_SPIN = 5, DQMC_MODE_GRAD_POS = 6, DQMC_MODE_ECP_FORCE = 7,
       DQMC_MODE_ZV_FORCE = 8 };

typedef struct dqmc_config {
  int32_t kind;
  int32_t dtype;
  int32_t gemm_backend;
  int32_t n_up, n_down, n_nuc;
  int32_t embedding_dim, n_layers, n_heads, n_determinants, edge_dim;
  int32_t cusp_kind;
  double cusp_same_scale, cusp_anti_scale;
  double z_valence[DQMC_MAX_NUC];
  int32_t ecp_mask[DQMC_MAX_NUC];
  int32_t ecp_loc_terms;
  double ecp_loc[DQMC_MAX_NUC][3][2][DQMC_MAX_ECP_TERMS];
  int32_t ecp_nl_lmax_p1, ecp_nl_terms;
  double ecp_nl[DQMC_MAX_NUC][DQMC_MAX_ECP_L][2][DQMC_MAX_ECP_TERMS];
  int32_t n_env_per_nuc;
  int32_t n_nuc_tokens;
  int32_t factorized_det;
  int32_t conf_linear;
  int32_t mult_act;
  int32_t n_elec_types;
  int32_t jastrow_n;
  int32_t jastrow_dims[8];
  int32_t backflow_n;
  int32_t backflow_dims[8];
  int32_t gnn_features;
  int32_t gnn_concat;
  int32_t gnn_conv_ne;
  int32_t gnn_sub_n;
  int32_t gnn_deep_edges;
  int32_t gnn_res_norm;
  int32_t gnn_g_bias, gnn_w_bias;
  int32_t gnn_w_dims[8][4];
  int32_t gnn_h_dims[8][4];
  int32_t gnn_u_dims[8][4];
  int32_t nuc_cusp_kind;
  double z_nuclear[DQMC_MAX_NUC];
  int32_t backflow_add;
} dqmc_config;

typedef struct dqmc_engine* dqmc_handle;

int dqmc_create(const dqmc_config* cfg, int device, dqmc_handle* out);
int dqmc_destroy(dqmc_handle h);
const char* dqmc_last_error(dqmc_handle h);
const char* dqmc_version(void);

int dqmc_param_count(dqmc_handle h);
int dqmc_param_entry(dqmc_handle h, int idx, char* name, int name_len, int64_t* offset, int32_t* rows,
                     int32_t* cols);
int64_t dqmc_param_total(dqmc_handle h);
int dqmc_set_params(dqmc_handle h, const double* host_params, int64_t n, void* stream);

int64_t dqmc_workspace_bytes(dqmc_handle h, int32_t n_walkers, int32_t mode);
int64_t dqmc_workspace_bytes_min(dqmc_handle h, int32_t n_walkers, int32_t mode);

int dqmc_wf_forward(dqmc_handle h, const void* r, const void* R, int32_t R_batched, int32_t n_walkers,
                    void* out_sign, void* out_log, void* workspace, int64_t workspace_bytes, void* stream);

int dqmc_local_energy(dqmc_handle h, const void* r, const void* R, int32_t R_batched, int32_t n_walkers,
                      uint64_t seed, const void* ecp_twist, void* out_E, void* out_stats, void* out_sign,
                      void* out_log, void* out_grad, void* workspace, int64_t workspace_bytes, void* stream);

int dqmc_wf_orbitals(dqmc_handle h, const void* r, const void* R, int32_t R_batched, int32_t n_walkers, void* out_orbitals,
                     void* workspace, int64_t workspace_bytes, void* stream);

int dqmc_mcmc_sweep(dqmc_handle h, void* r, void* sign, void* log, int32_t* age, void* tau, const void* R,
                    int32_t R_batched, int32_t n_walkers, int32_t n_sub, double target_acceptance, int32_t max_age,
                    uint64_t seed, uint64_t step0, uint64_t walker_offset, const void* noise_normal,
                    const void* noise_uniform, void* out_stats, void* workspace, int64_t workspace_bytes,
                    void* stream);

int dqmc_mcmc_sweep_exchange(dqmc_handle h, void* r, void* sign, void* log, int32_t* age, void* tau, const void* R,
                             int32_t R_batched, int32_t n_walkers, int32_t n_sub, double target_acceptance, int32_t max_age,
                             uint64_t seed, uint64_t step0, uint64_t walker_offset, const void* noise_normal,
                             const void* noise_uniform, double exchange_step_probability, const int32_t* exchange_flags,
                             const int32_t* exchange_idx, void* out_stats, void* workspace, int64_t workspace_bytes,
                             void* stream);

int dqmc_langevin_sweep(dqmc_handle h, void* r, void* sign, void* log, void* force, int32_t* age, void* tau, const void* R,
                        int32_t R_batched, int32_t n_walkers, int32_t n_sub, double target_acceptance, int32_t max_age,
                        uint64_t seed, uint64_t step0, uint64_t walker_offset, const void* noise_normal,
                        const void* noise_uniform, void* out_stats, void* workspace, int64_t workspace_bytes, void* stream);

int dqmc_wf_vjp_params(dqmc_handle h, const void* r, const void* R, int32_t R_batched, int32_t n_walkers,
                       const void* weights, void* out_sign, void* out_log, void* out_grad_params, void* workspace,
                       int64_t workspace_bytes, void* stream);

int dqmc_spin(dqmc_handle h, const void* r, const void* R, int32_t R_batched, int32_t n_walkers, const void* sign,
              const void* log, int32_t down_idx, void* out_s2, void* out_ratio, void* workspace, int64_t workspace_bytes,
              void* stream);

int dqmc_wf_grad_positions(dqmc_handle h, const void* r, const void* R, int32_t R_batched, int32_t n_walkers,
                           void* out_sign, void* out_log, void* out_grad_r, void* out_grad_R,
                           void* workspace, int64_t workspace_bytes, void* stream);

int dqmc_force_terms(dqmc_handle h, const void* r, const void* R, int32_t R_batched, int32_t n_walkers,
                     const void* grad_r, void* out_bare, void* out_zvq, void* out_Q, void* stream);

int dqmc_ecp_force(dqmc_handle h, const void* r, const void* R, int32_t R_batched, int32_t n_walkers, uint64_t seed,
                   const void* ecp_twist, void* out_bare, void* out_nl, void* workspace, int64_t workspace_bytes, void* stream);

int dqmc_zv_force(dqmc_handle h, const void* r, const void* R, int32_t R_batched, int32_t n_walkers, void* out_zv,
                  void* out_grad_R, void* workspace, int64_t workspace_bytes, void* stream);

int dqmc_set_pseudo_hamiltonian(dqmc_handle h, int32_t n_tab, int32_t n_grid, double r_max, const double* tables,
                                const int32_t* tab_of_nuc);

int dqmc_stats_pack(dqmc_handle h, const void* E_loc, const void* stats, int32_t n_walkers, double* out11, void* stream);

int dqmc_debug_plan(dqmc_handle h, int32_t n_walkers, int32_t mode, int64_t workspace_bytes, int64_t* planned_bytes,
                    int64_t* carved_bytes);

int64_t dqmc_launch_count(dqmc_handle h);
int64_t dqmc_ecp_forward_count(dqmc_handle h);

int dqmc_debug_gemm(dqmc_handle h, const char* weight, const char* bias, const void* A, const void* Res, void* C,
                    int32_t rows, int32_t S, int32_t sliced, int32_t backend, void* stream);

int dqmc_debug_mlp_block(dqmc_handle h, int32_t layer, const void* O, const void* X, void* Out, int32_t rows, void* stream);

int dqmc_debug_trunk(dqmc_handle h, const void* X0, void* Out, int32_t rows, void* stream);

enum {
  DQMC_ATTN_KERNEL_MMA = 0,
  DQMC_ATTN_KERNEL_FL_F32 = 1,
  DQMC_ATTN_KERNEL_GENERIC = 2,
  DQMC_ATTN_KERNEL_FL_F32_MMA = 3,
  DQMC_ATTN_KERNEL_GENERIC_MMA = 4
};
int dqmc_debug_attention(dqmc_handle h, int32_t layer, const void* QKV, void* O, int32_t rows, int32_t S, int32_t* kernel,
                         void* stream);

enum {
  DQMC_MLP_PATH_BLOCK = 0,
  DQMC_MLP_PATH_GEMM_ACT = 1,
  DQMC_MLP_PATH_GEMM_TANH = 2,
  DQMC_MLP_PATH_SIMT_TANH = 3
};
int dqmc_debug_mlp(dqmc_handle h, int32_t layer, int32_t S, const void* O, const void* X, void* Out, void* scratch, int32_t rows,
                   int32_t* path, void* stream);

enum {
  DQMC_SLATER_KERNEL_SMALL = 0,
  DQMC_SLATER_KERNEL_FWD2 = 1,
  DQMC_SLATER_KERNEL_FWD_REG = 2,
  DQMC_SLATER_KERNEL_GENERIC = 3
};
int dqmc_debug_slater(dqmc_handle h, const void* r, const void* R, const void* BF, int32_t rows, int32_t S, void* det_sign,
                      void* det_log, void* det_grad, void* det_lap, int32_t* kernel, void* stream);

int dqmc_debug_det_sum(dqmc_handle h, const void* r, const void* R, const void* det_sign, const void* det_log,
                       const void* det_grad, const void* det_lap, int32_t B, int32_t S, void* sign, void* logp, void* grad,
                       void* stats, void* stream);

int dqmc_debug_attention_bwd(dqmc_handle h, int32_t layer, const void* QKV, const void* dO, void* dQKV, void* dKn, void* dVn,
                             int32_t rows, void* stream);

int dqmc_debug_wgrad(dqmc_handle h, const void* A, const void* dY, int32_t rows, int32_t K, int32_t Nc, int32_t lo, int32_t hi,
                     void* dW, void* db, void* stream);

int dqmc_debug_trunk_phases(dqmc_handle h, uint64_t* out, int32_t n);

int dqmc_profile_begin(dqmc_handle h);
int dqmc_profile_end(dqmc_handle h, double* gemm_ms, double* gemm_flops, int64_t* n_gemm);
int dqmc_profile_end_classes(dqmc_handle h, double* ms3, double* flops3, int64_t* n3);

#ifdef __cplusplus
}
#endif
#endif
```

Baseline: 932.4.

## Stream next GEMM's weights across GEMM boundaries and replace ping-pong token with lock

The weight-ring TMA loader now prefetches the first slots of the next GEMM (next group, layer or tile) while the current GEMM's tail runs, instead of refilling the ring at the start of each GEMM. The strict two-warpgroup ping-pong token handoff is replaced by a shared-memory CAS lock taken after the first weight slot arrives. Each GEMM now takes and releases the lock itself. This targets the pipeline bubble at GEMM boundaries and the serialization from fixed turn order. In exchange it adds spin-wait lock overhead and a timeout error flag exposed via a new debug query.

Result: faster. 964.9 (median of 6 runs) (+3.5%).

```diff
diff --git a/deepqmc_b200/_lib.py b/deepqmc_b200/_lib.py
--- a/deepqmc_b200/_lib.py
+++ b/deepqmc_b200/_lib.py
@@ -17,7 +17,7 @@
     'dqmc_profile_end_classes', 'dqmc_debug_trunk_phases', 'dqmc_debug_attention', 'dqmc_debug_mlp',
     'dqmc_debug_slater', 'dqmc_debug_det_sum', 'dqmc_spin', 'dqmc_ecp_forward_count', 'dqmc_wf_grad_positions',
     'dqmc_force_terms', 'dqmc_ecp_force', 'dqmc_debug_wgrad', 'dqmc_zv_force',
-    'dqmc_debug_attention_bwd',
+    'dqmc_debug_attention_bwd', 'dqmc_debug_tc_error',
 ]
 
 
@@ -79,6 +79,7 @@
     lib.dqmc_debug_mlp_block.argtypes = [vp, i32, vp, vp, vp, i32, vp]
     lib.dqmc_debug_trunk.argtypes = [vp, vp, vp, i32, vp]
     lib.dqmc_debug_trunk_phases.argtypes = [vp, C.POINTER(u64), i32]
+    lib.dqmc_debug_tc_error.argtypes = [vp, C.POINTER(i32)]
     lib.dqmc_debug_attention.argtypes = [vp, i32, vp, vp, i32, i32, C.POINTER(i32), vp]
     lib.dqmc_debug_mlp.argtypes = [vp, i32, i32, vp, vp, vp, vp, i32, C.POINTER(i32), vp]
     lib.dqmc_debug_slater.argtypes = [vp, vp, vp, vp, i32, i32, vp, vp, vp, vp, C.POINTER(i32), vp]
diff --git a/deepqmc_b200/csrc/engine.cu b/deepqmc_b200/csrc/engine.cu
--- a/deepqmc_b200/csrc/engine.cu
+++ b/deepqmc_b200/csrc/engine.cu
@@ -162,6 +162,7 @@
   virtual int debug_mlp(int layer, int S, const void* O, const void* X, void* Out, void* scratch, int rows, int32_t* path,
                         cudaStream_t st) = 0;
   virtual int debug_trunk_phases(uint64_t* out, int n) = 0;
+  virtual int debug_tc_error(int32_t* flag) = 0;
   virtual int debug_slater(const void* r, const void* R, const void* BF, int rows, int S, void* dsign, void* dlog, void* dgrad,
                            void* dlap, int32_t* kernel, cudaStream_t st) = 0;
   virtual int debug_det_sum(const void* r, const void* R, const void* dsign, const void* dlog, const void* dgrad,
@@ -492,6 +493,7 @@
   };
   CUtensorMap* d_trunk_maps = nullptr;
   unsigned char* d_trunk_scratch = nullptr;
+  int* d_tc_err = nullptr;
   unsigned long long* d_trunk_phase = nullptr;
   static constexpr float kActScale = 16.f;
   std::map<std::string, TcWeight> tcw;
@@ -684,6 +686,8 @@
       DQ_CHECK(raise_dyn_smem(tc::trunk_f16_kernel<8>, tc::TrSmem::total()));
       DQ_CHECK(raise_dyn_smem(tc::trunk_f16_kernel<16>, tc::TrSmem::total()));
       DQ_CHECK(raise_dyn_smem(tc::trunk_f16_kernel<32>, tc::TrSmem::total()));
+      DQ_CHECK(cudaMalloc((void**)&d_tc_err, sizeof(int)));
+      DQ_CHECK(cudaMemset(d_tc_err, 0, sizeof(int)));
       if (psif && !trans && d == 256 && H == 4 && N <= 32 && cfg.n_layers <= tc::kTrMaxLayers) {
         DQ_CHECK(cudaMalloc((void**)&d_trunk_maps, sizeof(CUtensorMap) * 8 * cfg.n_layers));
         DQ_CHECK(cudaMalloc((void**)&d_trunk_scratch, (size_t)n_sms * tc::kTrScratchPerCta));
@@ -717,6 +721,7 @@
     if (d_trunk_maps) cudaFree(d_trunk_maps);
     if (d_trunk_scratch) cudaFree(d_trunk_scratch);
     if (d_trunk_phase) cudaFree(d_trunk_phase);
+    if (d_tc_err) cudaFree(d_tc_err);
 #endif
   }
   const T* P(const std::string& n) const { return d_params + off(n); }
@@ -1124,7 +1129,7 @@
       p.O = O; p.ldo = d; p.X = X; p.ldx = d; p.Out = Out; p.ldout = d; p.b1 = P(pfx + "b1"); p.b2 = P(pfx + "b2");
       p.M = rows; p.d = d; p.a_scale = kActScale;
       p.us0 = 1.f / (kActScale * wo.wscale); p.us1 = 1.f / (kActScale * w1.wscale); p.us2 = 1.f / (kActScale * w2.wscale);
-      p.err_flag = nullptr;
+      p.err_flag = d_tc_err;
       const int MT = (rows + 127) / 128;
       const int grid = MT < n_sms ? MT : n_sms;
 #ifndef DQMC_EMU
@@ -1189,7 +1194,7 @@
       int np2 = 1;
       while (np2 < N) np2 *= 2;
       p.walkers = rows / N; p.N = N; p.L = cfg.n_layers; p.a_scale = kActScale;
-      p.attn_scale = (float)(1.0 / std::sqrt((double)dh)); p.err_flag = nullptr; p.phase = d_trunk_phase;
+      p.attn_scale = (float)(1.0 / std::sqrt((double)dh)); p.err_flag = d_tc_err; p.phase = d_trunk_phase;
       for (int l = 0; l < cfg.n_layers; ++l) {
         const std::string pfx = "L" + std::to_string(l) + ".";
         p.b1[l] = P(pfx + "b1"); p.b2[l] = P(pfx + "b2");
@@ -1229,6 +1234,18 @@
     if (n < tc::kPhases) { err = "dqmc_debug_trunk_phases: the output holds fewer than the kernel's counters"; return 2; }
     DQ_CHECK(cudaMemcpy(out, d_trunk_phase, sizeof(unsigned long long) * tc::kPhases, cudaMemcpyDeviceToHost));
     DQ_CHECK(cudaMemset(d_trunk_phase, 0, sizeof(unsigned long long) * tc::kPhases));
+    return 0;
+#else
+    err = "this build has no tensor-core backend"; return 2;
+#endif
+  }
+  int debug_tc_error(int32_t* flag) override {
+#if !defined(DQMC_NO_TCGEN05)
+    if (!d_tc_err) { err = "no tensor-core backend in this engine"; return 2; }
+    int v = 0;
+    DQ_CHECK(cudaMemcpy(&v, d_tc_err, sizeof(int), cudaMemcpyDeviceToHost));
+    DQ_CHECK(cudaMemset(d_tc_err, 0, sizeof(int)));
+    *flag = v;
     return 0;
 #else
     err = "this build has no tensor-core backend"; return 2;
@@ -3118,6 +3135,12 @@
   if (!out) { h->e->err = "dqmc_debug_trunk_phases: null output"; return 2; }
   return h->e->debug_trunk_phases(out, n);
 }
+int dqmc_debug_tc_error(dqmc_handle h, int32_t* flag) {
+  if (!h) return 2;
+  DQ_NEED_DEVICE(h);
+  if (!flag) { h->e->err = "dqmc_debug_tc_error: null output"; return 2; }
+  return h->e->debug_tc_error(flag);
+}
 
 int dqmc_profile_begin(dqmc_handle h) {
   if (!h) return 2;
diff --git a/deepqmc_b200/csrc/fused_tc.cuh b/deepqmc_b200/csrc/fused_tc.cuh
--- a/deepqmc_b200/csrc/fused_tc.cuh
+++ b/deepqmc_b200/csrc/fused_tc.cuh
@@ -30,15 +30,32 @@
 __device__ __forceinline__ uint64_t* ring_full(unsigned char* smem, int wg) {
   return (uint64_t*)(smem + MlpSmem::bars()) + wg * kMlpSlots;
 }
-__device__ __forceinline__ uint64_t* mma_token(unsigned char* smem, int wg) {
-  return (uint64_t*)(smem + MlpSmem::bars()) + 2 * kMlpSlots + wg;
-}
+__device__ __forceinline__ uint32_t* mma_lock(unsigned char* smem) {
+  return (uint32_t*)((uint64_t*)(smem + MlpSmem::bars()) + 2 * kMlpSlots);
+}
+static_assert(2 * kMlpSlots * 8 + 4 <= 64, "the ring barriers and the lock word fit below MlpSmem::phases()");
 __device__ __forceinline__ void init_rings(unsigned char* smem) {
-  for (int i = 0; i < 2 * kMlpSlots + 2; ++i) mbar_init((uint64_t*)(smem + MlpSmem::bars()) + i, 1);
+  for (int i = 0; i < 2 * kMlpSlots; ++i) mbar_init((uint64_t*)(smem + MlpSmem::bars()) + i, 1);
+  *mma_lock(smem) = 0u;
   fence_barrier_init();
 }
-__device__ __forceinline__ void start_pingpong(unsigned char* smem) {
-  if (threadIdx.x == 128) mbar_arrive(mma_token(smem, 0));
+
+constexpr unsigned kLockSleepNs = 64;
+__device__ __forceinline__ void lock_take(unsigned char* smem, int wg, int* err) {
+  const uint32_t a = smem_u32(mma_lock(smem)), me = 1u + (uint32_t)wg;
+  if (smem_cas_acquire(a, 0u, me) == 0u) return;
+  const long long t0 = clock64();
+  while (true) {
+    __nanosleep(kLockSleepNs);
+    if (smem_cas_acquire(a, 0u, me) == 0u) return;
+    if (clock64() - t0 > 4000000000LL) {
+      if (err) atomicExch(err, 1);
+      return;
+    }
+  }
+}
+__device__ __forceinline__ void lock_release(unsigned char* smem, int wg) {
+  smem_cas_release(smem_u32(mma_lock(smem)), 1u + (uint32_t)wg, 0u);
 }
 
 enum Phase {
@@ -101,35 +118,69 @@
 }
 
 struct Ring {
-  uint32_t nslot = 0, nturn = 0;
-};
-enum Turn { kTurnTake = 1, kTurnPass = 2, kTurnOwn = kTurnTake | kTurnPass, kTurnKeep = 0 };
+  uint32_t nslot = 0;
+};
+enum Turn { kTurnTake = 1, kTurnRelease = 2, kTurnOwn = kTurnTake | kTurnRelease, kTurnKeep = 0 };
+
+struct WTile {
+  const CUtensorMap* hi;
+  const CUtensorMap* lo;
+  int y0;
+};
+template <class Maps>
+struct WeightStream {
+  Maps maps;
+  int L, MT;
+  __device__ __forceinline__ WTile after(int tile, int l, int g) const {
+    if (++g == Maps::G) {
+      g = 0;
+      if (++l == L) {
+        l = 0;
+        tile += gridDim.x;
+      }
+    }
+    return tile < MT ? maps.at(l, g) : WTile{nullptr, nullptr, 0};
+  }
+};
 
 template <int D>
-__device__ __forceinline__ void gemm_abuf(float (&acc)[D / 2], unsigned char* smem, Ring& ring, const CUtensorMap* mh,
-                                          const CUtensorMap* ml, int y0, int turn, int* err, PhaseClock& pc) {
+__device__ __forceinline__ void load_slot(unsigned char* smem, int wg, int st, const WTile& w, int i) {
+  uint64_t* full = ring_full(smem, wg) + st;
+  mbar_expect_tx(full, D * 64u);
+  tma_load_2d(((i >> 1) & 1) ? w.lo : w.hi, full, smem + MlpSmem::wring(wg, st), (i >> 2) * 64 + (i & 1) * 32, w.y0);
+}
+template <int D, class Maps>
+__device__ __forceinline__ void stream_start(unsigned char* smem, const WeightStream<Maps>& ws) {
+  if ((threadIdx.x & 127) == 0 && (int)blockIdx.x < ws.MT) {
+    const WTile w = ws.maps.at(0, 0);
+    for (int i = 0; i < kMlpSlots; ++i) load_slot<D>(smem, threadIdx.x >> 7, i, w, i);
+  }
+}
+
+template <int D, class Maps>
+__device__ __forceinline__ void gemm_abuf(float (&acc)[D / 2], unsigned char* smem, Ring& ring, const WeightStream<Maps>& ws,
+                                          int tile, int l, int g, int turn, int* err, PhaseClock& pc) {
   uint32_t& nslot = ring.nslot;
   constexpr int KB = D / 64;
   constexpr int NS = 4 * KB;
-  static_assert(NS >= kMlpSlots, "the ring is filled at the start of a GEMM");
-  constexpr uint32_t kSlot = D * 64u;
+  static_assert(NS >= kMlpSlots, "a GEMM has at least as many slots as the ring has stages");
   const int wg = threadIdx.x >> 7;
   const bool leader = (threadIdx.x & 127) == 0;
   uint64_t* full = ring_full(smem, wg);
+  const WTile cur = ws.maps.at(l, g), nxt = ws.after(tile, l, g);
 #pragma unroll
   for (int i = 0; i < D / 2; ++i) acc[i] = 0.f;
   auto stage = [&](int i) { return (int)((nslot + (uint32_t)i) % (uint32_t)kMlpSlots); };
-  auto load = [&](int i) {
-    const int st = stage(i);
-    mbar_expect_tx(&full[st], kSlot);
-    tma_load_2d(((i >> 1) & 1) ? ml : mh, &full[st], smem + MlpSmem::wring(wg, st), (i >> 2) * 64 + (i & 1) * 32, y0);
-  };
-  if (leader)
-    for (int i = 0; i < kMlpSlots; ++i) load(i);
   if (turn & kTurnTake) {
-    const long long t0 = pc.acc ? clock64() : 0;
-    mbar_wait(mma_token(smem, wg), ring.nturn & 1u, err);
-    ++ring.nturn;
+    long long t0 = pc.acc ? clock64() : 0;
+    if (leader) mbar_wait(&full[stage(0)], (nslot / (uint32_t)kMlpSlots) & 1u, err);
+    if (pc.acc) {
+      const long long t1 = clock64();
+      pc.waited(t1 - t0, kPhWait);
+      t0 = t1;
+    }
+    if (leader) lock_take(smem, wg, err);
+    wg_sync(wg);
     if (pc.acc) pc.waited(clock64() - t0, kPhTurn);
   }
   auto acquire = [&](int i) {
@@ -139,11 +190,15 @@
     if (pc.acc) pc.waited(clock64() - t0, kPhWait);
     return smem_u32(smem + MlpSmem::wring(wg, st));
   };
-  auto retire = [&](int i) {
+  auto retire = [&](int i, bool cross) {
     wgmma_wait1();
     if (i == 0) return;
     wg_sync(wg);
-    if (leader && i + kMlpSlots - 1 < NS) load(i + kMlpSlots - 1);
+    const int s = i + kMlpSlots - 1;
+    const bool own = !cross || s < NS;
+    if (leader && (own || nxt.hi))
+      load_slot<D>(smem, wg, stage(s), WTile{own ? cur.hi : nxt.hi, own ? cur.lo : nxt.lo, own ? cur.y0 : nxt.y0},
+                   own ? s : s - NS);
   };
   auto mma = [&](float (&d)[D / 2], uint32_t a, uint32_t w, int accumulate) {
     if constexpr (D == 256) wgmma_f16_n256(d, make_desc(a), make_desc64(w), accumulate);
@@ -163,7 +218,7 @@
         mma(acc, ah + 32 * k, w + 32 * kk, 1);
       }
       wgmma_commit();
-      retire(4 * kb + q);
+      retire(4 * kb + q, false);
     }
 #pragma unroll
     for (int q = 0; q < 2; ++q) {
@@ -172,13 +227,14 @@
 #pragma unroll
       for (int kk = 0; kk < 2; ++kk) mma(acc, ah + 32 * (2 * q + kk), w + 32 * kk, 1);
       wgmma_commit();
-      retire(4 * kb + 2 + q);
-    }
-  }
-  if ((turn & kTurnPass) && leader) mbar_arrive(mma_token(smem, wg ^ 1));
+      retire(4 * kb + 2 + q, true);
+    }
+  }
+  if ((turn & kTurnRelease) && leader) lock_release(smem, wg);
   wgmma_wait0();
   fence_acc(acc);
   wg_sync(wg);
+  if (leader && nxt.hi) load_slot<D>(smem, wg, stage(NS + kMlpSlots - 1), nxt, kMlpSlots - 1);
   nslot += NS;
 }
 
@@ -243,17 +299,15 @@
   }
 }
 
-template <int D>
-__device__ __forceinline__ void mlp3(float (&acc)[D / 2], unsigned char* smem, Ring& ring, const CUtensorMap* const (&wmaps)[6],
-                                     float us0, float us1, float us2, float a_scale, const float* b1, const float* b2,
-                                     const float* const (&xin)[2], float* const (&aout)[2], float* const (&xout)[2],
-                                     bool operand_out, int* err, PhaseClock& pc) {
+template <int D, class Maps>
+__device__ __forceinline__ void mlp3(float (&acc)[D / 2], unsigned char* smem, Ring& ring, const WeightStream<Maps>& ws,
+                                     int tile, int l, float us0, float us1, float us2, float a_scale, const float* b1,
+                                     const float* b2, const float* const (&xin)[2], float* const (&aout)[2],
+                                     float* const (&xout)[2], bool operand_out, int* err, PhaseClock& pc) {
   const int wg = threadIdx.x >> 7;
 #pragma unroll 1
   for (int g = 0; g < 3; ++g) {
-    const CUtensorMap* mh = g == 0 ? wmaps[0] : (g == 1 ? wmaps[2] : wmaps[4]);
-    const CUtensorMap* ml = g == 0 ? wmaps[1] : (g == 1 ? wmaps[3] : wmaps[5]);
-    gemm_abuf<D>(acc, smem, ring, mh, ml, 0, kTurnOwn, err, pc);
+    gemm_abuf<D>(acc, smem, ring, ws, tile, l, Maps::G - 3 + g, kTurnOwn, err, pc);
     pc.mark(kPhWo + 2 * g);
     if (g == 0) {
       mlp_epilogue<D, kEpiWo>(acc, smem, us0, nullptr, a_scale, xin, aout, true);
@@ -273,6 +327,14 @@
   }
 }
 
+struct MlpMaps {
+  static constexpr int G = 3;
+  const CUtensorMap *wo_hi, *wo_lo, *w1_hi, *w1_lo, *w2_hi, *w2_lo;
+  __device__ __forceinline__ WTile at(int, int g) const {
+    return g == 0 ? WTile{wo_hi, wo_lo, 0} : (g == 1 ? WTile{w1_hi, w1_lo, 0} : WTile{w2_hi, w2_lo, 0});
+  }
+};
+
 template <int D>
 __global__ void __launch_bounds__(kMlpThreads, 1)
 mlp_block_f16_kernel(const __grid_constant__ CUtensorMap wo_hi, const __grid_constant__ CUtensorMap wo_lo,
@@ -282,6 +344,7 @@
   if ((smem_u32(smem) & 1023u) != 0u) tc_trap();
   const int tid = threadIdx.x, wg = tid >> 7;
   const int MT = (p.M + 127) / 128;
+  const WeightStream<MlpMaps> ws{MlpMaps{&wo_hi, &wo_lo, &w1_hi, &w1_lo, &w2_hi, &w2_lo}, 1, MT};
 
   if (tid == 0) {
     init_rings(smem);
@@ -289,7 +352,7 @@
     tma_prefetch_desc(&w1_lo); tma_prefetch_desc(&w2_hi); tma_prefetch_desc(&w2_lo);
   }
   __syncthreads();
-  start_pingpong(smem);
+  stream_start<D>(smem, ws);
   const Frag f;
   Ring ring;
   float acc[D / 2];
@@ -314,10 +377,9 @@
       xin[h] = valid ? p.X + (size_t)grow * p.ldx : nullptr;
       aout[h] = valid ? p.Out + (size_t)grow * p.ldout : nullptr;
     }
-    const CUtensorMap* const wmaps[6] = {&wo_hi, &wo_lo, &w1_hi, &w1_lo, &w2_hi, &w2_lo};
-    mlp3<D>(acc, smem, ring, wmaps, p.us0, p.us1, p.us2, p.a_scale, p.b1, p.b2, xin, aout, aout, false, p.err_flag, pc);
-  }
-}
-
-}
-}
+    mlp3<D>(acc, smem, ring, ws, tile, 0, p.us0, p.us1, p.us2, p.a_scale, p.b1, p.b2, xin, aout, aout, false, p.err_flag, pc);
+  }
+}
+
+}
+}
diff --git a/deepqmc_b200/csrc/tc_ptx.cuh b/deepqmc_b200/csrc/tc_ptx.cuh
--- a/deepqmc_b200/csrc/tc_ptx.cuh
+++ b/deepqmc_b200/csrc/tc_ptx.cuh
@@ -37,6 +37,16 @@
 }
 __device__ __forceinline__ void mbar_arrive(uint64_t* bar) {
   asm volatile("mbarrier.arrive.shared::cta.b64 _, [%0];" ::"r"(smem_u32(bar)) : "memory");
+}
+__device__ __forceinline__ uint32_t smem_cas_acquire(uint32_t saddr, uint32_t cmp, uint32_t val) {
+  uint32_t old;
+  asm volatile("atom.acquire.cta.shared::cta.cas.b32 %0, [%1], %2, %3;" : "=r"(old) : "r"(saddr), "r"(cmp), "r"(val) : "memory");
+  return old;
+}
+__device__ __forceinline__ uint32_t smem_cas_release(uint32_t saddr, uint32_t cmp, uint32_t val) {
+  uint32_t old;
+  asm volatile("atom.release.cta.shared::cta.cas.b32 %0, [%1], %2, %3;" : "=r"(old) : "r"(saddr), "r"(cmp), "r"(val) : "memory");
+  return old;
 }
 __device__ __forceinline__ void wg_sync(int wg) { asm volatile("bar.sync %0, 128;" ::"r"(1 + wg) : "memory"); }
 __device__ __forceinline__ void fence_proxy_async() { asm volatile("fence.proxy.async.shared::cta;" ::: "memory"); }
diff --git a/deepqmc_b200/csrc/trunk_tc.cuh b/deepqmc_b200/csrc/trunk_tc.cuh
--- a/deepqmc_b200/csrc/trunk_tc.cuh
+++ b/deepqmc_b200/csrc/trunk_tc.cuh
@@ -35,6 +35,15 @@
   unsigned long long* phase;
 };
 
+struct TrunkMaps {
+  static constexpr int G = 6;
+  const CUtensorMap* maps;
+  __device__ __forceinline__ WTile at(int l, int g) const {
+    const CUtensorMap* m = maps + 8 * l + 2 * (g < 3 ? 0 : g - 2);
+    return WTile{m, m + 1, g < 2 ? 256 * (g + 1) : 0};
+  }
+};
+
 template <int NP>
 __global__ void __launch_bounds__(kTrThreads, 1)
 trunk_f16_kernel(TrunkParams p) {
@@ -57,8 +66,9 @@
   }
   unsigned long long* ph = (unsigned long long*)(smem + TrSmem::phases());
   if (tid < 32) ph[tid] = 0ull;
+  const WeightStream<TrunkMaps> ws{TrunkMaps{p.maps}, L, MT};
   __syncthreads();
-  start_pingpong(smem);
+  stream_start<256>(smem, ws);
   PhaseClock pc(p.phase && (tid & 127) == 0 ? ph + 16 * wg : nullptr);
   const Frag f;
   Ring ring;
@@ -112,12 +122,10 @@
     pc.mark(kPhLoad);
     for (int l = 0; l < L; ++l) {
       const bool last = l == L - 1;
-      const CUtensorMap* lm = p.maps + 8 * l;
 #pragma unroll 1
       for (int j = 0; j < 3; ++j) {
         const int blk = j == 2 ? 0 : j + 1;
-        const int turn = j == 0 ? kTurnTake : (j == 2 ? kTurnPass : kTurnKeep);
-        gemm_abuf<256>(acc, smem, ring, lm, lm + 1, 256 * blk, turn, p.err_flag, pc);
+        gemm_abuf<256>(acc, smem, ring, ws, tile, l, j, kTurnOwn, p.err_flag, pc);
         pc.mark(kPhQkv);
         const float us = p.us[l][0];
         const int odd = ag & 1;
@@ -201,9 +209,8 @@
         const long long row = grow_of(r);
         xout[h] = !last ? resid + r * 256 : (row >= 0 ? p.Out + (size_t)row * p.ldout : nullptr);
       }
-      const CUtensorMap* const wmaps[6] = {lm + 2, lm + 3, lm + 4, lm + 5, lm + 6, lm + 7};
-      mlp3<256>(acc, smem, ring, wmaps, p.us[l][1], p.us[l][2], p.us[l][3], p.a_scale, p.b1[l], p.b2[l], xin, aout, xout,
-                !last, p.err_flag, pc);
+      mlp3<256>(acc, smem, ring, ws, tile, l, p.us[l][1], p.us[l][2], p.us[l][3], p.a_scale, p.b1[l], p.b2[l], xin, aout,
+                xout, !last, p.err_flag, pc);
       fence_proxy_async();
       wg_sync(wg);
       pc.mark(kPhW2Epi);
diff --git a/deepqmc_b200/engine.py b/deepqmc_b200/engine.py
--- a/deepqmc_b200/engine.py
+++ b/deepqmc_b200/engine.py
@@ -828,6 +828,11 @@
         self._check(rc, 'dqmc_debug_trunk_phases')
         return dict(zip(self.TRUNK_PHASES, out))
 
+    def debug_tc_error(self):
+        flag = C.c_int32()
+        self._check(self.lib.dqmc_debug_tc_error(self.h, C.byref(flag)), 'dqmc_debug_tc_error')
+        return flag.value
+
     def profile_begin(self):
         self.lib.dqmc_profile_begin(self.h)
 
diff --git a/include/dqmc_b200.h b/include/dqmc_b200.h
--- a/include/dqmc_b200.h
+++ b/include/dqmc_b200.h
@@ -179,6 +179,8 @@
 
 int dqmc_debug_trunk_phases(dqmc_handle h, uint64_t* out, int32_t n);
 
+int dqmc_debug_tc_error(dqmc_handle h, int32_t* flag);
+
 int dqmc_profile_begin(dqmc_handle h);
 int dqmc_profile_end(dqmc_handle h, double* gemm_ms, double* gemm_flops, int64_t* n_gemm);
 int dqmc_profile_end_classes(dqmc_handle h, double* ms3, double* flops3, int64_t* n3);
```
